# Gongzihang6/Pointcept-KeypointDetection

Measured on AMD Instinct MI355X. Metric: Mpoints/sec PTv3 fwd @100k pts/scene, 1024-pt window; keypoint offset L2 vs ref, higher is better.
Workload: dtype bf16; 1 GPU; OffsetKeypointPTv3 (PT-v3m1 fork config, 46.2M params) eval forward, 1 x 100000-point synthetic surface scene(s) per GPU, patch 1024, serialization + sparse conv + attention + head included; points_per_gpu=100000, parallelism=replicas x1 (scene-sharded, no collective), forwards_in_flight=1

## Files before the change

### include/ptv3_hip.h

```cpp
#ifndef PTV3_HIP_H
#define PTV3_HIP_H
#include <stddef.h>
#include <stdint.h>

#ifdef __cplusplus
extern "C" {
#endif

#define PTV3_F32 0
#define PTV3_BF16 1

#define PTV3_ORDER_Z 0
#define PTV3_ORDER_Z_TRANS 1
#define PTV3_ORDER_HILBERT 2
#define PTV3_ORDER_HILBERT_TRANS 3

#define PTV3_ACT_NONE 0
#define PTV3_ACT_GELU 1
#define PTV3_ACT_RELU 2

const char* ptv3_last_error(void);
int ptv3_version(void);

int ptv3_sfc_encode(const void* grid_coord, int coord_is_i64, const int64_t* batch, int64_t n,
                    int depth, const int* order_ids_host, int k, int64_t* code, void* stream);

size_t ptv3_argsort_workspace_bytes(int k, int64_t n);
int ptv3_argsort_i64(const int64_t* code, int k, int64_t n, int end_bit, int64_t* order,
                     int64_t* inverse, void* workspace, size_t workspace_bytes, void* stream);

int ptv3_argsort_i64_rows(const int64_t* code, int k, int64_t n, int end_bit, int64_t* order, int64_t* inverse,
                          int32_t* row_order, void* workspace, size_t workspace_bytes, void* stream);
int ptv3_argsort_scan_batch(void);

int ptv3_coord_max(const void* grid_coord, int coord_is_i64, int64_t n, int32_t* state, int32_t* out_max, void* stream);

int ptv3_pad_plan(const int64_t* offset, int b, int64_t n, int64_t n_pad, int patch, int64_t* pad,
                  int64_t* unpad, int32_t* cu_seqlens, void* stream);

int ptv3_window_maps(const int64_t* order, const int64_t* inverse, const int64_t* pad,
                     const int64_t* unpad, int64_t n, int64_t n_pad, int32_t* win_order,
                     int32_t* win_inverse, void* stream);

int ptv3_window_plan(const int64_t* order, const int64_t* inverse, const int64_t* offset, int b, int k,
                     int64_t n, int64_t n_pad, int patch, int32_t* win_order, int32_t* win_inverse,
                     int32_t* cu_seqlens, void* stream);

int ptv3_window_attn_fwd(const void* qkv, const int32_t* win_order, const int32_t* win_inverse,
                         void* out, int64_t n, int64_t n_pad, int c, int heads, int patch, float scale,
                         const float* rpe_bias, int dtype, void* stream);

int ptv3_window_attn_varlen_fwd(const void* qkv, const int32_t* win_order, const int32_t* win_inverse,
                                const int32_t* cu_seqlens, int num_windows, void* out, int64_t n, int64_t n_pad,
                                int c, int heads, int max_seqlen, float scale, double sum_len_sq, int dtype,
                                void* stream);

int ptv3_window_attn_rpe_fwd(const void* qkv, const int32_t* win_order, const int32_t* win_inverse, void* out,
                             int64_t n, int64_t n_pad, int c, int heads, int patch, float scale,
                             const int32_t* grid_coord, const float* rpe_table, int pos_bnd, int dtype,
                             void* stream);

int64_t ptv3_subm_table_slots(int64_t n);
int ptv3_subm_build_table(const int32_t* indices, int64_t n, void* table, int64_t slots, void* stream);
int ptv3_subm_neighbors(const int32_t* indices, int64_t n, const void* table, int64_t slots, int ksize,
                        int32_t* nbr, void* stream);

size_t ptv3_subm_block_table_bytes(int64_t n);
int ptv3_subm_build_block_table(const int32_t* indices, int64_t n, void* table, size_t bytes, void* stream);
int ptv3_subm_neighbors_blocks(const int32_t* indices, int64_t n, const void* table, size_t bytes, int ksize,
                               int32_t* nbr, void* stream);

int ptv3_subm_sites(const int64_t* batch, const void* grid_coord, int coord_is_i64, int64_t n, int32_t* indices,
                    int64_t* grid64, void* table, size_t bytes, void* stream);
int ptv3_subm_build_block_table_zeroed(const int32_t* indices, int64_t n, void* table, size_t bytes, void* stream);

size_t ptv3_gemm_workspace_bytes(int64_t m, int cin, int cout, int kvol, int dtype);
int ptv3_gemm_splits(int64_t m, int cin, int cout, int kvol, int dtype);
int ptv3_gemm(const void* x, const void* w, void* out, int64_t m, int cin, int cout, int kvol,
              const int32_t* nbr, const int32_t* row_order, const float* bias, const float* bn_scale,
              const float* bn_shift, int act, const void* res, const int32_t* res_index, void* out2,
              int dtype, void* workspace, size_t workspace_bytes, void* stream);

int ptv3_block_fusable(int c, int hidden, int dtype, int64_t m);
int ptv3_rows_linear_capable(int c, int cout, int dtype, int64_t m);
int ptv3_rows_linear(const void* x, const void* shortcut, const float* g0, const float* b0, const float* g1,
                     const float* b1, const void* w, const float* bias, int act, const void* res, void* f1, void* out,
                     int64_t m, int c, int cout, float eps, int dtype, void* stream);
int ptv3_block_head(const void* x, const float* slab, int splits, const float* conv_bias, const void* shortcut,
                    const float* g0, const float* b0, const float* g1, const float* b1, const void* wqkv,
                    const float* bqkv, void* f1, void* qkv, int64_t m, int c, float eps, int dtype, void* stream);
int ptv3_mlp2_fusable(int cin, int hidden, int cout, int dtype);
int ptv3_mlp2(const void* x, const void* w1, const float* b1, const float* s1, const float* t1, int act,
              const void* w2, const float* b2, void* out, int out_f32, int64_t m, int cin, int hidden, int cout,
              int dtype, void* stream);
int ptv3_block_tail(const void* attn, const void* f1, const void* wproj, const float* bproj, const float* g2,
                    const float* b2, const void* w1, const float* bias1, const void* w2, const float* bias2,
                    void* out, int64_t m, int c, int hidden, float eps, int dtype, void* stream);

int ptv3_rows_linear_ln_capable(int c, int cout, int dtype);
int ptv3_rows_linear_ln(const void* x, const void* w, const float* bias, const float* gamma, const float* beta,
                        void* out, int64_t m, int c, int cout, float eps, int act, int dtype, void* stream);
int ptv3_subm_conv_ln_capable(int c, int kvol, int dtype);
int ptv3_subm_conv_ln(const void* x, const void* w, const int32_t* nbr, const int32_t* row_order, const float* bias,
                      const float* gamma, const float* beta, void* out, int64_t m, int c, int kvol, float eps, int act,
                      int dtype, void* stream);

int ptv3_res_conv_capable(int64_t m, int ca, int cb, int cout, int kvol);
int ptv3_res_conv_row_tiles(int64_t m, int cout);
int ptv3_res_conv(const float* xa, const float* xb, const float* w, const int32_t* nbr, const int32_t* row_order,
                  const float* bn_scale, const float* bn_shift, const float* res, int act, float* out,
                  const float* w_proj, const float* proj_scale, const float* proj_shift, float* proj_out, int64_t m,
                  int ca, int cb, int cout, int kvol, void* stream);

int ptv3_layernorm(const void* x, const float* gamma, const float* beta, const void* res, void* y,
                   const float* gamma2, const float* beta2, void* y2, int64_t m, int c, float eps,
                   int dtype, void* stream);

int ptv3_layernorm_slabs(const float* slab, int splits, const float* slab_bias, const float* gamma, const float* beta,
                         const void* res, void* y, const float* gamma2, const float* beta2, void* y2, int64_t m, int c,
                         float eps, int dtype, void* stream);

int ptv3_affine_act(const void* x, const float* scale, const float* shift, int act, void* y, int64_t m,
                    int c, int dtype, void* stream);

int ptv3_cast(const void* x, int src_dtype, void* y, int dst_dtype, int64_t count, void* stream);

size_t ptv3_pool_workspace_bytes(int64_t n);
int ptv3_pool_segments(const int64_t* code0, const int64_t* order0, int64_t n, int shift_bits,
                       const int64_t* batch, int64_t* cluster, int32_t* seg_start, int32_t* n_out,
                       int64_t* pooled_offset, void* workspace, size_t workspace_bytes, void* stream);
int ptv3_pool_reduce(const void* feat, const float* coord, const int64_t* grid_coord,
                     const int64_t* batch, const int64_t* code, int k, const int64_t* order0,
                     const int32_t* seg_start, int64_t n, int64_t n_out, int c, int pooling_depth,
                     const float* bn_scale, const float* bn_shift, int act, const int* row_perm_host,
                     void* feat_out, float* coord_out, int64_t* grid_out, int64_t* batch_out,
                     int64_t* code_out, int dtype, void* stream);

typedef struct {
  int32_t dtype, in_channels , num_stages, num_orders;
  int32_t enc_depths[8], enc_channels[8], enc_heads[8], enc_patch[8];
  int32_t dec_depths[8], dec_channels[8], dec_heads[8], dec_patch[8];
  int32_t stride[8];
  int32_t enc_mode, enable_flash;
  int32_t head_hidden, head_out;
  float mlp_ratio, ln_eps, qk_scale ;
} ptv3_model_desc;

typedef struct {
  const void* grid_coord; int32_t coord_is_i64;
  const void* feat;
  const int64_t* batch;
  const int64_t* offset;
  const int64_t* offset_host;
  int32_t b; int64_t n;
  int32_t depth;
  const int32_t* order_ids_host;
  const int32_t* pool_perm_host;
  int64_t *code, *order, *inverse;
  void* out_feat;
  float* out_head;
  int64_t* stage_points_host;
  int32_t* depth_out;
  int64_t* batch_out;
  int32_t inputs_resident;
  int32_t overlap_calls;
  const void* raw_feat;
  int32_t raw_feat_channels;
  int32_t raw_feat_dtype;
  int64_t arena_n;
  int32_t arena_b;
  void* executor;
} ptv3_forward_io;

void* ptv3_executor_create(void);
int ptv3_executor_destroy(void* executor);

size_t ptv3_forward_workspace_bytes(const ptv3_model_desc* desc, int64_t n, int b);
int ptv3_forward(const ptv3_model_desc* desc, const void* const* params, int num_params,
                 const ptv3_forward_io* io, void* workspace, size_t workspace_bytes, void* stream);

size_t ptv3_gemm_tn_workspace_bytes(int64_t m, int cout, int cin, int kvol);
int ptv3_gemm_tn(const void* dy, const void* x, const int32_t* nbr, float* dw, float* dbias, int64_t m, int cout,
                 int cin, int kvol, int dtype, void* workspace, size_t workspace_bytes, void* stream);
size_t ptv3_col_reduce_workspace_bytes(int64_t m, int c);
int ptv3_col_reduce(const void* a, const void* b, const float* mu, const float* rs, float mu_scale, int mode, float* out,
                    int64_t m, int c, int dtype, void* workspace, size_t workspace_bytes, void* stream);
int ptv3_bn_finalize(const float* sum, const float* centred_sq, int64_t m, const float* weight, const float* bias,
                     float* running_mean, float* running_var, float momentum, float eps, float* mean, float* rstd,
                     float* scale, float* shift, int c, void* stream);
int ptv3_bn_bwd_coeffs(const float* sums, int64_t m, const float* weight, const float* rstd, const float* mean, float* ca,
                       float* cb, float* cc, int c, void* stream);
int ptv3_layernorm_bwd(const void* x, const void* dy, const void* add, const float* gamma, float eps, void* dx,
                       float* dgamma_dbeta, int64_t m, int c, int dtype, void* workspace,
                       size_t workspace_bytes, void* stream);
int ptv3_act_bwd(const void* dy, const void* x, const float* scale, const float* shift, int act, void* dx,
                 int64_t m, int c, int dtype, void* stream);
int ptv3_affine2(const void* dy, const void* x, const float* ca, const float* cb, const float* cc, void* dx,
                 int64_t m, int c, int dtype, void* stream);
int ptv3_pool_max_bwd(const void* feat, const void* dy, const int64_t* order0, const int32_t* seg_start,
                      int64_t n_out, int c, void* dfeat, int dtype, void* stream);
int ptv3_segment_sum(const void* dy, const int64_t* order0, const int32_t* seg_start, int64_t n_out, int c,
                     void* out, int dtype, void* stream);
size_t ptv3_window_attn_bwd_workspace_bytes(int64_t n, int64_t n_pad, int c, int heads, int dtype);
int ptv3_window_attn_bwd(const void* qkv, const void* out, const void* dout, const int32_t* win_order,
                         const int32_t* win_inverse, void* dqkv, int64_t n, int64_t n_pad, int c, int heads,
                         int patch, float scale, int dtype, void* workspace, size_t workspace_bytes,
                         void* stream);
int ptv3_window_attn_varlen_bwd(const void* qkv, const void* out, const void* dout, const int32_t* win_order,
                                const int32_t* win_inverse, const int32_t* cu_seqlens, int num_windows, void* dqkv,
                                int64_t n, int64_t n_pad, int c, int heads, int max_seqlen, float scale, int dtype,
                                void* workspace, size_t workspace_bytes, void* stream);
int ptv3_window_attn_train_fwd(const void* qkv, const int32_t* win_order, const int32_t* win_inverse,
                               const int32_t* cu_seqlens, int num_windows, void* out, float* lse, int64_t n,
                               int64_t n_pad, int c, int heads, int patch, float scale, double sum_len_sq, int dtype,
                               void* stream);
int ptv3_window_attn_train_bwd(const void* qkv, const void* out, const void* dout, const float* lse,
                               const int32_t* win_order, const int32_t* win_inverse, const int32_t* cu_seqlens,
                               int num_windows, void* dqkv, int64_t n, int64_t n_pad, int c, int heads, int patch,
                               float scale, int dtype, void* workspace, size_t workspace_bytes, void* stream);
int ptv3_window_attn_drop_fwd(const void* qkv, const int32_t* win_order, const int32_t* win_inverse,
                              const int32_t* cu_seqlens, int num_windows, void* out, int64_t n, int64_t n_pad, int c,
                              int heads, int patch, float scale, float p_drop, uint32_t seed, int dtype, void* stream);
int ptv3_window_attn_drop_bwd(const void* qkv, const void* out, const void* dout, const int32_t* win_order,
                              const int32_t* win_inverse, const int32_t* cu_seqlens, int num_windows, void* dqkv,
                              int64_t n, int64_t n_pad, int c, int heads, int patch, float scale, float p_drop,
                              uint32_t seed, int dtype, void* workspace, size_t workspace_bytes, void* stream);
size_t ptv3_window_attn_rpe_bwd_workspace_bytes(int64_t n, int64_t n_pad, int c, int heads, int patch, int pos_bnd,
                                                int dtype);
int ptv3_window_attn_rpe_bwd(const void* qkv, const void* out, const void* dout, const int32_t* win_order,
                             const int32_t* win_inverse, const int32_t* grid_coord, const float* rpe_table,
                             int pos_bnd, void* dqkv, float* dtable, int64_t n, int64_t n_pad, int c, int heads,
                             int patch, float scale, int dtype, void* workspace, size_t workspace_bytes, void* stream);
typedef struct ptv3_block_train {
  int64_t n, n_pad;
// ... 196 lines not shown
```

### pointcept-keypointdetection_amd/csrc/engine.hip

```cpp
#include <algorithm>
#include <chrono>
#include <mutex>
#include <stdio.h>
#include <stdlib.h>
#include <vector>
#include "common.h"
#include "window_attn.h"

namespace ptv3 {

struct Arena {
  char* base; size_t cap; size_t off; size_t peak; bool dry; bool failed;
  void* alloc(size_t bytes) {
    size_t a = (off + 255) / 256 * 256;
    off = a + bytes;
    if (off > peak) peak = off;
    if (dry) return (void*)(uintptr_t)256;
    if (off > cap) { failed = true; return nullptr; }
    return base + a;
  }
};

__global__ void make_indices_kernel(const int64_t* __restrict__ batch, const void* __restrict__ grid,
                                    int is_i64, int64_t n, int32_t* __restrict__ idx,
                                    int64_t* __restrict__ grid64, int32_t* __restrict__ row_order,
                                    const int64_t* __restrict__ order0) {
  int64_t i = (int64_t)blockIdx.x * blockDim.x + threadIdx.x;
  if (i >= n) return;
  int64_t x, y, z;
  if (is_i64) {
    const int64_t* g = (const int64_t*)grid;
    x = g[3 * i]; y = g[3 * i + 1]; z = g[3 * i + 2];
  } else {
    const int32_t* g = (const int32_t*)grid;
    x = g[3 * i]; y = g[3 * i + 1]; z = g[3 * i + 2];
  }
  idx[4 * i] = (int32_t)batch[i];
  idx[4 * i + 1] = (int32_t)x; idx[4 * i + 2] = (int32_t)y; idx[4 * i + 3] = (int32_t)z;
  if (grid64) { grid64[3 * i] = x; grid64[3 * i + 1] = y; grid64[3 * i + 2] = z; }
  if (row_order) row_order[i] = (int32_t)order0[i];
}

__global__ void i64_to_i32_kernel(const int64_t* __restrict__ src, int32_t* __restrict__ dst, int64_t n) {
  int64_t i = (int64_t)blockIdx.x * blockDim.x + threadIdx.x;
  if (i < n) dst[i] = (int32_t)src[i];
}

constexpr int CM_BATCH = 8;
template <typename CoordT>
__global__ void __launch_bounds__(256) coord_max_kernel(const CoordT* __restrict__ grid, int64_t n3, int* __restrict__ state,
                                                        int* __restrict__ out, const int64_t* __restrict__ offset, int b,
                                                        int64_t* __restrict__ offset_out) {
  __shared__ int s_wave[4];
  __shared__ int s_last;
  const int64_t base = (int64_t)blockIdx.x * (256 * CM_BATCH) + threadIdx.x;
  CoordT c[CM_BATCH];
#pragma unroll
  for (int u = 0; u < CM_BATCH; ++u) c[u] = grid[min(base + u * 256, n3 - 1)];
  int v = 0;
#pragma unroll
  for (int u = 0; u < CM_BATCH; ++u) v = max(v, (int)c[u]);
  for (int d = 32; d > 0; d >>= 1) v = max(v, __shfl_down(v, d, 64));
  if ((threadIdx.x & 63) == 0) s_wave[threadIdx.x >> 6] = v;
  __syncthreads();
  if (threadIdx.x == 0) {
    atomicMax(&state[0], max(max(s_wave[0], s_wave[1]), max(s_wave[2], s_wave[3])));
    __threadfence();
    const bool last = atomicAdd(&state[1], 1) == (int)gridDim.x - 1;
    if (last) {
      __threadfence();
      out[0] = atomicExch(&state[0], 0);
      atomicExch(&state[1], 0);
    }
    s_last = last;
  }
  __syncthreads();
  if (s_last)
    for (int i = threadIdx.x; i < b; i += 256) offset_out[i] = offset[i];
}
static void coord_max(const void* grid, int is_i64, int64_t n, int* state, int* out, const int64_t* offset, int b,
                      int64_t* offset_out, hipStream_t s) {
  const dim3 blocks((unsigned)cdiv(3 * n, 256 * CM_BATCH));
  if (is_i64)
    hipLaunchKernelGGL(coord_max_kernel<int64_t>, blocks, dim3(256), 0, s, (const int64_t*)grid, 3 * n, state, out, offset,
                       b, offset_out);
  else
    hipLaunchKernelGGL(coord_max_kernel<int32_t>, blocks, dim3(256), 0, s, (const int32_t*)grid, 3 * n, state, out, offset,
                       b, offset_out);
}

__global__ void batch_from_offset_kernel(const int64_t* __restrict__ offset, int b, int64_t n,
                                         int64_t* __restrict__ batch) {
  int64_t i = (int64_t)blockIdx.x * blockDim.x + threadIdx.x;
  if (i >= n) return;
  int lo = 0, hi = b;
  while (lo < hi) { int mid = (lo + hi) >> 1; if (offset[mid] > i) hi = mid; else lo = mid + 1; }
  batch[i] = lo;
}

struct Plan {
  int K = -1; int64_t n_pad = 0; int32_t* wo[8] = {nullptr}; int32_t* wi[8] = {nullptr};
  int32_t* cu = nullptr; int nwin = 0; double sum_len_sq = 0.0;
};

struct Level {
  int64_t n = 0; int depth = 0;
  std::vector<int64_t> off_host;
  const int64_t* offset = nullptr;
  const int64_t* grid = nullptr; const int64_t* batch = nullptr;
  int64_t *code = nullptr, *order = nullptr, *inverse = nullptr;
  int32_t* indices = nullptr; void* table = nullptr; size_t table_bytes = 0;
  int32_t* nbr3 = nullptr; int32_t* nbr5 = nullptr; int32_t* row_order = nullptr;
  Plan plan[2];
  int32_t* seg = nullptr;
  int64_t* cluster = nullptr;
  int32_t* cluster32 = nullptr;
  hipEvent_t ready = nullptr;
  void* feat = nullptr; void* conv_feat = nullptr; int channels = 0;
};

static inline double now_us() {
  return std::chrono::duration<double, std::micro>(std::chrono::steady_clock::now().time_since_epoch()).count();
}

struct DeviceStreams { hipStream_t geo = nullptr; hipStream_t feat[2] = {nullptr, nullptr}; };
static std::mutex g_pool_mutex;
static std::vector<DeviceStreams> g_device_streams;
static hipStream_t device_stream(int device, int which ) {
  std::lock_guard<std::mutex> guard(g_pool_mutex);
  if ((int)g_device_streams.size() <= device) g_device_streams.resize(device + 1);
  DeviceStreams& d = g_device_streams[device];
  hipStream_t& s = which == 0 ? d.geo : d.feat[which - 1];
  if (!s) {
    if (which == 0) {
      int least = 0, greatest = 0;
      (void)hipDeviceGetStreamPriorityRange(&least, &greatest);
      if (hipStreamCreateWithPriority(&s, hipStreamNonBlocking, greatest) != hipSuccess) s = nullptr;
    } else if (hipStreamCreateWithFlags(&s, hipStreamNonBlocking) != hipSuccess) {
      s = nullptr;
    }
  }
  return s;
}

struct Exec {
  int device = 0;
  hipStream_t geo = nullptr;
  hipStream_t feat[2] = {nullptr, nullptr};
  std::vector<hipEvent_t> events;
  unsigned call = 0;
  bool last_overlap = false;
  double sync_us = 0.0;
  std::mutex mu;
  void* pinned = nullptr; size_t pinned_cap = 0;
  int* cm_state = nullptr;
  int* coord_max_state() {
    if (!cm_state) {
      if (hipMalloc((void**)&cm_state, 256) != hipSuccess) { cm_state = nullptr; return nullptr; }
      if (hipMemset(cm_state, 0, 256) != hipSuccess) { (void)hipFree(cm_state); cm_state = nullptr; }
    }
    return cm_state;
  }
  void* pinned_at_least(size_t bytes) {
    if (pinned_cap < bytes) {
      if (pinned) (void)hipHostFree(pinned);
      pinned = nullptr; pinned_cap = 0;
      const size_t cap = std::max<size_t>(bytes, 4096);
      if (hipHostMalloc(&pinned, cap, hipHostMallocDefault) != hipSuccess) { pinned = nullptr; return nullptr; }
      pinned_cap = cap;
    }
    return pinned;
  }
  hipError_t timed_event_sync(hipEvent_t e) {
    double t = now_us();
    hipError_t r = hipEventSynchronize(e);
    sync_us += now_us() - t;
    return r;
  }
  hipError_t timed_sync(hipStream_t s) {
    double t = now_us();
    hipError_t e = hipStreamSynchronize(s);
    sync_us += now_us() - t;
    return e;
  }
  hipEvent_t event_at(size_t i) {
    while (events.size() <= i) {
      hipEvent_t e;
      (void)hipEventCreateWithFlags(&e, hipEventDisableTiming);
      events.push_back(e);
    }
    return events[i];
  }
  void release() {
    if (geo) { (void)hipStreamSynchronize(geo); geo = nullptr; }
    for (auto& f : feat) if (f) { (void)hipStreamSynchronize(f); f = nullptr; }
    for (hipEvent_t e : events) (void)hipEventDestroy(e);
    events.clear();
    if (pinned) { (void)hipHostFree(pinned); pinned = nullptr; pinned_cap = 0; }
    if (cm_state) { (void)hipFree(cm_state); cm_state = nullptr; }
  }
};
static std::mutex g_exec_mutex;
static std::vector<Exec*> g_default_exec;
static Exec* default_exec() {
  int dev = 0;
  (void)hipGetDevice(&dev);
  std::lock_guard<std::mutex> guard(g_exec_mutex);
  if ((int)g_default_exec.size() <= dev) g_default_exec.resize(dev + 1, nullptr);
  if (!g_default_exec[dev]) { g_default_exec[dev] = new Exec(); g_default_exec[dev]->device = dev; }
  return g_default_exec[dev];
}

template <typename S, typename D>
__global__ void pad_cast_kernel(const S* __restrict__ x, int cin, D* __restrict__ y, int cpad, int64_t n) {
  const int64_t i = (int64_t)blockIdx.x * blockDim.x + threadIdx.x;
  if (i >= n * cpad) return;
  const int c = (int)(i % cpad);
  y[i] = from_f32<D>(c < cin ? to_f32<S>(x[(i / cpad) * cin + c]) : 0.f);
}
static void pad_cast(const void* x, int sdt, int cin, void* y, int ddt, int cpad, int64_t n, hipStream_t s) {
  dim3 grid((unsigned)cdiv(n * cpad, 256)), block(256);
  if (sdt == PTV3_F32 && ddt == PTV3_F32)
    hipLaunchKernelGGL((pad_cast_kernel<float, float>), grid, block, 0, s, (const float*)x, cin, (float*)y, cpad, n);
  else if (sdt == PTV3_F32)
    hipLaunchKernelGGL((pad_cast_kernel<float, __bf16>), grid, block, 0, s, (const float*)x, cin, (__bf16*)y, cpad, n);
  else if (ddt == PTV3_F32)
    hipLaunchKernelGGL((pad_cast_kernel<__bf16, float>), grid, block, 0, s, (const __bf16*)x, cin, (float*)y, cpad, n);
  else
    hipLaunchKernelGGL((pad_cast_kernel<__bf16, __bf16>), grid, block, 0, s, (const __bf16*)x, cin, (__bf16*)y, cpad, n);
}

struct Run {
  Exec* X;
  const ptv3_model_desc* d; const void* const* params; int pi = 0;
  Arena* G; Arena* F;
  hipStream_t sg, sf;
  int es; bool dry; int rc = 0;
  const void* next() { return params ? params[pi++] : (pi++, nullptr); }
  bool ok() const { return rc == 0 && !G->failed && !F->failed; }
#define RUN(call) do { if (!dry && ok()) { int r__ = (call); if (r__) rc = r__; } } while (0)

  void gemm(const void* x, const void* w, void* out, int64_t m, int cin, int cout, int kvol, const int32_t* nbr,
            const int32_t* row_order, const float* bias, const float* bns, const float* bnt, int act,
            const void* res, const int32_t* res_index, void* out2) {
    size_t wsb = ptv3_gemm_workspace_bytes(m, cin, cout, kvol, d->dtype);
    size_t mark = F->off;
    void* ws = wsb ? F->alloc(wsb) : nullptr;
    RUN(ptv3_gemm(x, w, out, m, cin, cout, kvol, nbr, row_order, bias, bns, bnt, act, res, res_index, out2,
                  d->dtype, ws, wsb, sf));
    F->off = mark;
  }

  bool rows_path(int64_t n, int C, int hidden) const {
    static const int64_t min_rows = [] { const char* e = getenv("PTV3_ROWS_MIN"); return e ? atoll(e) : (int64_t)0; }();
    return n >= min_rows && ptv3_rows_linear_capable(C, 3 * C, d->dtype, n) && ptv3_rows_linear_capable(C, C, d->dtype, n) &&
           ptv3_rows_linear_capable(C, hidden, d->dtype, n);
  }

  int patch_K(const Level& L, int patch) const {
    if (d->enable_flash) return patch;
    int64_t mn = L.off_host[0];
    for (size_t i = 1; i < L.off_host.size(); ++i) mn = std::min(mn, L.off_host[i] - L.off_host[i - 1]);
    return (int)std::min<int64_t>(mn, patch);
  }

  void window_plan(Level& L, Plan& P, int K) {
    int64_t n_pad = 0, prev = 0;
    for (int64_t o : L.off_host) {
      int64_t cnt = o - prev;
      n_pad += cnt > K ? (cnt + K - 1) / K * K : cnt;
      prev = o;
    }
    P.K = K; P.n_pad = n_pad;
    bool ragged = false;
    P.nwin = 0; P.sum_len_sq = 0.0; prev = 0;
    for (int64_t o : L.off_host) {
      const int64_t cnt = o - prev;
      prev = o;
      P.nwin += (int)((cnt + K - 1) / K);
      if (cnt < K) { ragged = true; P.sum_len_sq += (double)cnt * cnt; }
      else P.sum_len_sq += (double)((cnt + K - 1) / K) * K * K;
    }
    const int k = d->num_orders;
    int32_t* wo = (int32_t*)G->alloc((size_t)k * n_pad * 4);
    int32_t* wi = (int32_t*)G->alloc((size_t)k * L.n * 4);
    P.cu = (ragged || (dry && d->enable_flash)) ? (int32_t*)G->alloc(((size_t)P.nwin + L.off_host.size() + 1) * 4) : nullptr;
    if (!ragged && !dry) P.cu = nullptr;
    RUN(ptv3_window_plan(L.order, L.inverse, L.offset, (int)L.off_host.size(), k, L.n, n_pad, K, wo, wi, P.cu, sg));
    for (int i = 0; i < k; ++i) { P.wo[i] = wo + (int64_t)i * n_pad; P.wi[i] = wi + (int64_t)i * L.n; }
  }

  hipEvent_t stem_ready = nullptr;
  void level0_sites(Level& L, const void* grid_in, int is_i64) {
    L.indices = (int32_t*)G->alloc((size_t)L.n * 16);
    L.row_order = (int32_t*)G->alloc((size_t)L.n * 4);
    int64_t* g64 = (int64_t*)G->alloc((size_t)L.n * 24);
    L.grid = g64;
    L.table_bytes = ptv3_subm_block_table_bytes(L.n);
    L.table = G->alloc(L.table_bytes);
    RUN(ptv3_subm_sites(L.batch, grid_in, is_i64, L.n, L.indices, g64, L.table, L.table_bytes, sg));
    RUN(ptv3_subm_build_block_table_zeroed(L.indices, L.n, L.table, L.table_bytes, sg));
    L.nbr5 = (int32_t*)G->alloc((size_t)L.n * 125 * 4);
    RUN(ptv3_subm_neighbors_blocks(L.indices, L.n, L.table, L.table_bytes, 5, L.nbr5, sg));
  }

  void level_tables(Level& L, int st) {
    L.nbr3 = (int32_t*)G->alloc((size_t)L.n * 27 * 4);
    RUN(ptv3_subm_neighbors_blocks(L.indices, L.n, L.table, L.table_bytes, 3, L.nbr3, sg));
    const int Ke = patch_K(L, d->enc_patch[st]);
    window_plan(L, L.plan[0], Ke);
    if (!d->enc_mode && st < d->num_stages - 1) {
      const int Kd = patch_K(L, d->dec_patch[st]);
      if (Kd == Ke) L.plan[1] = L.plan[0]; else window_plan(L, L.plan[1], Kd);
    }
  }

  void level_geometry(Level& L, int st, const void* grid_in, int is_i64) {
    L.indices = (int32_t*)G->alloc((size_t)L.n * 16);
    L.row_order = (int32_t*)G->alloc((size_t)L.n * 4);
    if (!dry && ok())
      hipLaunchKernelGGL(make_indices_kernel, dim3((unsigned)cdiv(L.n, 256)), dim3(256), 0, sg, L.batch, grid_in, is_i64,
                         L.n, L.indices, (int64_t*)nullptr, L.row_order, L.order);
    L.table_bytes = ptv3_subm_block_table_bytes(L.n);
    L.table = G->alloc(L.table_bytes);
    RUN(ptv3_subm_build_block_table(L.indices, L.n, L.table, L.table_bytes, sg));
    level_tables(L, st);
  }

  void attention(const Level& L, const Plan& P, const void* qkv, void* out, int C, int H, int oi, float scale) {
    WindowAttnCall a = window_attn_call(qkv, P.wo[oi], P.wi[oi], out, L.n, P.n_pad, C, H, P.K, scale, d->dtype, sf);
    a.cu_seqlens = P.cu; a.num_windows = P.nwin; a.sum_len_sq = P.sum_len_sq;
    RUN(window_attn_forward(a, {"window_attn", WA_RAGGED_OPTIONAL}));
  }

  void block(Level& L, const Plan& P, int C, int H, int oi) {
    const void* conv_w = next(); const float* conv_b = (const float*)next();
    const float* ln0_g = (const float*)next(); const float* ln0_b = (const float*)next();
    const float* n1_g = (const float*)next(); const float* n1_b = (const float*)next();
    const void* qkv_w = next(); const float* qkv_b = (const float*)next();
    const void* proj_w = next(); const float* proj_b = (const float*)next();
    const float* n2_g = (const float*)next(); const float* n2_b = (const float*)next();
    const void* fc1_w = next(); const float* fc1_b = (const float*)next();
    const void* fc2_w = next(); const float* fc2_b = (const float*)next();
    const int hidden = (int)(C * d->mlp_ratio);
    const size_t mark = F->off;
    const size_t row = (size_t)L.n * es;
    const float scale = d->qk_scale > 0.f ? d->qk_scale : 1.0f / sqrtf((float)(C / H));
    if (ptv3_block_fusable(C, hidden, d->dtype, L.n)) {
      void* f1 = F->alloc(row * C); void* qkv = F->alloc(row * 3 * C); void* t4 = F->alloc(row * C);
      const int splits = ptv3_gemm_splits(L.n, C, C, 27, d->dtype);
      if (splits > 1) {
        const size_t wsb = ptv3_gemm_workspace_bytes(L.n, C, C, 27, d->dtype);
        float* slab = (float*)F->alloc(wsb);
        RUN(ptv3_gemm(L.conv_feat, conv_w, nullptr, L.n, C, C, 27, L.nbr3, L.row_order, nullptr, nullptr, nullptr, 0,
                      nullptr, nullptr, nullptr, d->dtype, slab, wsb, sf));
        RUN(ptv3_block_head(nullptr, slab, splits, conv_b, L.feat, ln0_g, ln0_b, n1_g, n1_b, qkv_w, qkv_b, f1, qkv, L.n,
                            C, d->ln_eps, d->dtype, sf));
      } else {
        void* t2 = F->alloc(row * C);
        gemm(L.conv_feat, conv_w, t2, L.n, C, C, 27, L.nbr3, L.row_order, conv_b, nullptr, nullptr, 0, nullptr, nullptr, nullptr);
        RUN(ptv3_block_head(t2, nullptr, 0, nullptr, L.feat, ln0_g, ln0_b, n1_g, n1_b, qkv_w, qkv_b, f1, qkv, L.n, C,
                            d->ln_eps, d->dtype, sf));
      }
      attention(L, P, qkv, t4, C, H, oi, scale);
      RUN(ptv3_block_tail(t4, f1, proj_w, proj_b, n2_g, n2_b, fc1_w, fc1_b, fc2_w, fc2_b, L.feat, L.n, C, hidden,
                          d->ln_eps, d->dtype, sf));
    } else {
      void* t2 = F->alloc(row * C); void* f1 = F->alloc(row * C); void* t3 = F->alloc(row * C);
      void* qkv = F->alloc(row * 3 * C); void* t4 = F->alloc(row * C); void* f2 = F->alloc(row * C);
      void* t5 = F->alloc(row * C); void* t6 = F->alloc(row * hidden);
      const int splits = ptv3_gemm_splits(L.n, C, C, 27, d->dtype);
      const bool rows = rows_path(L.n, C, hidden);
      if (splits > 1) {
        const size_t wsb = ptv3_gemm_workspace_bytes(L.n, C, C, 27, d->dtype);
        float* slab = (float*)F->alloc(wsb);
        RUN(ptv3_gemm(L.conv_feat, conv_w, nullptr, L.n, C, C, 27, L.nbr3, L.row_order, nullptr, nullptr, nullptr, 0,
                      nullptr, nullptr, nullptr, d->dtype, slab, wsb, sf));
        RUN(ptv3_layernorm_slabs(slab, splits, conv_b, ln0_g, ln0_b, L.feat, f1, n1_g, n1_b, t3, L.n, C, d->ln_eps,
                                 d->dtype, sf));
        gemm(t3, qkv_w, qkv, L.n, C, 3 * C, 1, nullptr, nullptr, qkv_b, nullptr, nullptr, 0, nullptr, nullptr, nullptr);
      } else if (rows) {
        gemm(L.conv_feat, conv_w, t2, L.n, C, C, 27, L.nbr3, L.row_order, conv_b, nullptr, nullptr, 0, nullptr, nullptr, nullptr);
        RUN(ptv3_rows_linear(t2, L.feat, ln0_g, ln0_b, n1_g, n1_b, qkv_w, qkv_b, 0, nullptr, f1, qkv, L.n, C, 3 * C,
                             d->ln_eps, d->dtype, sf));
      } else {
        gemm(L.conv_feat, conv_w, t2, L.n, C, C, 27, L.nbr3, L.row_order, conv_b, nullptr, nullptr, 0, nullptr, nullptr, nullptr);
        RUN(ptv3_layernorm(t2, ln0_g, ln0_b, L.feat, f1, n1_g, n1_b, t3, L.n, C, d->ln_eps, d->dtype, sf));
        gemm(t3, qkv_w, qkv, L.n, C, 3 * C, 1, nullptr, nullptr, qkv_b, nullptr, nullptr, 0, nullptr, nullptr, nullptr);
      }
      attention(L, P, qkv, t4, C, H, oi, scale);
      if (rows) {
        RUN(ptv3_rows_linear(t4, nullptr, nullptr, nullptr, nullptr, nullptr, proj_w, proj_b, 0, f1, nullptr, f2, L.n, C, C,
                             d->ln_eps, d->dtype, sf));
        RUN(ptv3_rows_linear(f2, nullptr, nullptr, nullptr, n2_g, n2_b, fc1_w, fc1_b, PTV3_ACT_GELU, nullptr, nullptr, t6,
                             L.n, C, hidden, d->ln_eps, d->dtype, sf));
      } else {
        gemm(t4, proj_w, f2, L.n, C, C, 1, nullptr, nullptr, proj_b, nullptr, nullptr, 0, f1, nullptr, nullptr);
        RUN(ptv3_layernorm(f2, n2_g, n2_b, nullptr, t5, nullptr, nullptr, nullptr, L.n, C, d->ln_eps, d->dtype, sf));
        gemm(t5, fc1_w, t6, L.n, C, hidden, 1, nullptr, nullptr, fc1_b, nullptr, nullptr, PTV3_ACT_GELU, nullptr, nullptr, nullptr);
      }
      gemm(t6, fc2_w, L.feat, L.n, hidden, C, 1, nullptr, nullptr, fc2_b, nullptr, nullptr, 0, f2, nullptr, nullptr);
    }
    L.conv_feat = L.feat;
    F->off = mark;
  }
};

#define RUNR(call) do { if (!dry && R.ok()) { int r__ = (call); if (r__) R.rc = r__; } } while (0)

static int run_forward(Exec* X, const ptv3_model_desc* d, const void* const* params, const ptv3_forward_io* io, Arena& G,
                       Arena& F, hipStream_t sf, bool dry, int* param_count = nullptr) {
  Run R; R.X = X; R.d = d; R.params = params; R.G = &G; R.F = &F; R.sf = sf; R.dry = dry;
  R.es = d->dtype == PTV3_F32 ? 4 : 2;
  const int S = d->num_stages, k = d->num_orders, es = R.es;
  if (!dry) {
    if (!X->geo) {
      X->geo = device_stream(X->device, 0);
      if (!X->geo) {
        set_error("forward: cannot create the geometry stream");
        return PTV3_ERR_LAUNCH;
      }
    }
    if (!io->inputs_resident) {
      hipEvent_t e = X->event_at(0);
      (void)hipEventRecord(e, sf);
      (void)hipStreamWaitEvent(X->geo, e, 0);
    } else {
      (void)hipStreamWaitEvent(X->geo, X->event_at(20 + (X->call & 1)), 0);
    }
  }
  R.sg = dry ? nullptr : X->geo;
  hipStream_t sg = R.sg;
  std::vector<Level> lv(S);
  const int nbits = io->b > 1 ? 32 - __builtin_clz((unsigned)(io->b - 1)) : 0;

  Level& L0 = lv[0];
  L0.n = io->n; L0.batch = io->batch; L0.offset = io->offset;
  L0.code = io->code; L0.order = io->order; L0.inverse = io->inverse;
  L0.off_host.resize(io->b);
  int depth = io->depth;
  const int* hmax = nullptr; const int64_t* hoff = nullptr;
  hipEvent_t read_back = nullptr;
  if (dry) {
    for (int i = 0; i < io->b; ++i) L0.off_host[i] = io->offset_host ? io->offset_host[i] : io->n * (i + 1) / io->b;
    if (depth <= 0) depth = 16;
  } else {
    if (io->offset_host) std::copy(io->offset_host, io->offset_host + io->b, L0.off_host.begin());
    if (depth <= 0 || !io->offset_host) {
      char* pin = (char*)X->pinned_at_least(8 + (size_t)io->b * 8);
      if (!pin) { set_error("forward: cannot allocate the pinned read-back buffer"); return PTV3_ERR_LAUNCH; }
      if (!io->offset_host) hoff = (const int64_t*)(pin + 8);
      if (depth <= 0) {
        int* state = X->coord_max_state();
        if (!state) { set_error("forward: cannot allocate the coordinate-maximum state"); return PTV3_ERR_LAUNCH; }
        hmax = (const int*)pin;
        coord_max(io->grid_coord, io->coord_is_i64, io->n, state, (int*)pin, io->offset, hoff ? io->b : 0,
                  (int64_t*)(pin + 8), sg);
      } else {
        (void)hipMemcpyAsync(pin + 8, io->offset, (size_t)io->b * 8, hipMemcpyDeviceToHost, sg);
      }
      read_back = X->event_at(18);
      (void)hipEventRecord(read_back, sg);
    }
  }
  if (io->batch == nullptr) {
    int64_t* bt = io->batch_out ? io->batch_out : (int64_t*)G.alloc((size_t)io->n * 8);
    if (!dry && R.ok())
      hipLaunchKernelGGL(batch_from_offset_kernel, dim3((unsigned)cdiv(io->n, 256)), dim3(256), 0, sg, io->offset, io->b,
                         io->n, bt);
    L0.batch = bt;
  }
  R.level0_sites(L0, io->grid_coord, io->coord_is_i64);
  if (!dry) {
    if (read_back && X->timed_event_sync(read_back) != hipSuccess) {
      set_error("forward: input read-back failed");
      return PTV3_ERR_LAUNCH;
    }
    if (hoff) std::copy(hoff, hoff + io->b, L0.off_host.begin());
    if (hmax) { depth = 0; for (unsigned v = (unsigned)*hmax + 1; v; v >>= 1) ++depth; }
    PTV3_REQUIRE(depth >= 1 && depth <= 16, "forward: serialization depth %d outside [1,16] (structure.py:81)", depth);
    for (int i = 0; i < io->b; ++i)
      PTV3_REQUIRE(L0.off_host[i] > (i ? L0.off_host[i - 1] : 0), "forward: empty scene %d", i);
    PTV3_REQUIRE(L0.off_host[io->b - 1] == io->n, "forward: offset does not end at n");
  }
  L0.depth = depth;
  if (io->depth_out) *io->depth_out = depth;
  {
    RUNR(ptv3_sfc_encode(io->grid_coord, io->coord_is_i64, L0.batch, io->n, depth, io->order_ids_host, k, L0.code, sg));
    size_t wsb = ptv3_argsort_workspace_bytes(k, io->n);
    void* ws = G.alloc(wsb);
    RUNR(ptv3_argsort_i64_rows(L0.code, k, io->n, std::max(1, 3 * depth + nbits), L0.order, L0.inverse, L0.row_order, ws, wsb,
                               sg));
  }
  if (!dry && R.ok()) { R.stem_ready = X->event_at(19); (void)hipEventRecord(R.stem_ready, sg); }
  R.level_tables(L0, 0);
  if (io->stage_points_host) io->stage_points_host[0] = L0.n;
  if (!dry && R.ok()) { L0.ready = X->event_at(1); (void)hipEventRecord(L0.ready, sg); }

  auto wait_level = [&](Level& L) { if (!dry && R.ok()) (void)hipStreamWaitEvent(sf, L.ready, 0); };
  struct PoolParams { const void* w; const float *b, *bns, *bnt; };
  const void* stem_w = R.next(); const float* stem_s = (const float*)R.next(); const float* stem_t = (const float*)R.next();
  {
    if (!dry && R.ok()) (void)hipStreamWaitEvent(sf, R.stem_ready, 0);
    const int C0 = d->enc_channels[0];
    L0.feat = F.alloc((size_t)L0.n * C0 * es); L0.channels = C0;
    const void* feat_in = io->feat;
    if (io->raw_feat) {
      void* padded = F.alloc((size_t)L0.n * d->in_channels * es);
      if (!dry && R.ok())
        pad_cast(io->raw_feat, io->raw_feat_dtype, io->raw_feat_channels, padded, d->dtype, d->in_channels, L0.n, sf);
      feat_in = padded;
    }
    R.gemm(feat_in, stem_w, L0.feat, L0.n, d->in_channels, C0, 125, L0.nbr5, L0.row_order, nullptr, stem_s, stem_t,
           PTV3_ACT_GELU, nullptr, nullptr, nullptr);
    L0.conv_feat = L0.feat;
    wait_level(L0);
  }
  for (int st = 0; st < S; ++st) {
    Level& L = lv[st];
    if (st > 0) {
      Level& P = lv[st - 1];
      PoolParams pp;
      pp.w = R.next(); pp.b = (const float*)R.next(); pp.bns = (const float*)R.next(); pp.bnt = (const float*)R.next();
      const int C = d->enc_channels[st], Cp = d->enc_channels[st - 1];
      int pd = 0; { int v = d->stride[st - 1] - 1; while (v > 0) { ++pd; v >>= 1; } }
      if (pd > P.depth) pd = 0;
      P.cluster = (int64_t*)G.alloc((size_t)P.n * 8);
      P.seg = (int32_t*)G.alloc((size_t)(P.n + 1) * 4);
      int64_t* poff = (int64_t*)G.alloc((size_t)io->b * 8);
      int32_t* nout_dev = (int32_t*)G.alloc(256);
      size_t pwsb = ptv3_pool_workspace_bytes(P.n);
      void* pws = G.alloc(pwsb);
      RUNR(ptv3_pool_segments(P.code, P.order, P.n, 3 * pd, P.batch, P.cluster, P.seg, nout_dev, poff, pws, pwsb, sg));
      L.off_host.resize(io->b);
      if (dry) {
        L.off_host = P.off_host;
      } else if (R.ok()) {
        if (hipMemcpyAsync(L.off_host.data(), poff, (size_t)io->b * 8, hipMemcpyDeviceToHost, sg) != hipSuccess ||
            X->timed_sync(sg) != hipSuccess) { set_error("forward: offset read-back failed"); return PTV3_ERR_LAUNCH; }
      }
      if (!R.ok()) break;
      L.n = L.off_host[io->b - 1]; L.depth = P.depth - pd; L.offset = poff; L.channels = C;
      if (io->stage_points_host) io->stage_points_host[st] = L.n;
      const int* perm = io->pool_perm_host + (size_t)(st - 1) * k;
      int64_t* g = (int64_t*)G.alloc((size_t)L.n * 24);
      int64_t* bt = (int64_t*)G.alloc((size_t)L.n * 8);
      L.code = (int64_t*)G.alloc((size_t)k * L.n * 8);
      L.order = (int64_t*)G.alloc((size_t)k * L.n * 8);
      L.inverse = (int64_t*)G.alloc((size_t)k * L.n * 8);
      RUNR(ptv3_pool_reduce(nullptr, nullptr, P.grid, P.batch, P.code, k, P.order, P.seg, P.n, L.n, C, pd, nullptr,
                           nullptr, 0, perm, nullptr, nullptr, g, bt, L.code, d->dtype, sg));
      L.grid = g; L.batch = bt;
      {
        size_t wsb = ptv3_argsort_workspace_bytes(k, L.n);
        void* ws = G.alloc(wsb);
        RUNR(ptv3_argsort_i64(L.code, k, L.n, std::max(1, 3 * L.depth + nbits), L.order, L.inverse, ws, wsb, sg));
      }
      R.level_geometry(L, st, L.grid, 1);
      if (!d->enc_mode) {
        P.cluster32 = (int32_t*)G.alloc((size_t)P.n * 4);
        if (!dry && R.ok())
          hipLaunchKernelGGL(i64_to_i32_kernel, dim3((unsigned)cdiv(P.n, 256)), dim3(256), 0, sg, P.cluster, P.cluster32, P.n);
      }
      if (!dry && R.ok()) { L.ready = X->event_at(1 + st); (void)hipEventRecord(L.ready, sg); }
      wait_level(L);
      L.feat = F.alloc((size_t)L.n * C * es);
      const size_t mark = F.off;
      void* proj = F.alloc((size_t)P.n * C * es);
      R.gemm(P.feat, pp.w, proj, P.n, Cp, C, 1, nullptr, nullptr, pp.b, nullptr, nullptr, 0, nullptr, nullptr, nullptr);
      RUNR(ptv3_pool_reduce(proj, nullptr, nullptr, nullptr, nullptr, k, P.order, P.seg, P.n, L.n, C, pd, pp.bns, pp.bnt,
                           PTV3_ACT_GELU, nullptr, L.feat, nullptr, nullptr, nullptr, nullptr, d->dtype, sf));
      F.off = mark;
      L.conv_feat = L.feat;
    }
    for (int i = 0; i < d->enc_depths[st]; ++i)
      R.block(L, L.plan[0], d->enc_channels[st], d->enc_heads[st], i % k);
    if (!R.ok()) break;
  }
  if (!d->enc_mode && R.ok()) {
    for (int st = S - 2; st >= 0; --st) {
      Level& P = lv[st];
      Level& Ch = lv[st + 1];
      const int Cd = d->dec_channels[st];
      const int Cin = Ch.channels, Cskip = d->enc_channels[st];
      const void* w = R.next(); const float* b = (const float*)R.next();
      const float* bns = (const float*)R.next(); const float* bnt = (const float*)R.next();
      const void* ws_ = R.next(); const float* bs = (const float*)R.next();
      const float* bnss = (const float*)R.next(); const float* bnst = (const float*)R.next();
      void* skip = F.alloc((size_t)P.n * Cd * es);
      void* fused = (st == 0 && io->out_feat) ? io->out_feat : F.alloc((size_t)P.n * Cd * es);
      const size_t mark = F.off;
      void* up = F.alloc((size_t)Ch.n * Cd * es);
      R.gemm(Ch.feat, w, up, Ch.n, Cin, Cd, 1, nullptr, nullptr, b, bns, bnt, PTV3_ACT_GELU, nullptr, nullptr, nullptr);
      R.gemm(P.feat, ws_, skip, P.n, Cskip, Cd, 1, nullptr, nullptr, bs, bnss, bnst, PTV3_ACT_GELU, up, P.cluster32, fused);
      F.off = mark;
      P.feat = fused; P.conv_feat = skip; P.channels = Cd;
      for (int i = 0; i < d->dec_depths[st]; ++i)
        R.block(P, P.plan[1], Cd, d->dec_heads[st], i % k);
      if (!R.ok()) break;
    }
  }
  if (R.ok() && d->head_out > 0 && !d->enc_mode) {
    Level& L = lv[0];
    const void* w0 = R.next(); const float* b0 = (const float*)R.next();
    const float* bns = (const float*)R.next(); const float* bnt = (const float*)R.next();
    const void* w1 = R.next(); const float* b1 = (const float*)R.next();
    const size_t mark = F.off;
    if (ptv3_mlp2_fusable(L.channels, d->head_hidden, d->head_out, d->dtype)) {
      if (!dry && R.ok()) {
        int r = ptv3_mlp2(L.feat, w0, b0, bns, bnt, PTV3_ACT_RELU, w1, b1, io->out_head, 1, L.n, L.channels,
                          d->head_hidden, d->head_out, d->dtype, sf);
        if (r) R.rc = r;
      }
    } else {
    void* hid = F.alloc((size_t)L.n * d->head_hidden * es);
    R.gemm(L.feat, w0, hid, L.n, L.channels, d->head_hidden, 1, nullptr, nullptr, b0, bns, bnt, PTV3_ACT_RELU, nullptr,
           nullptr, nullptr);
    if (d->dtype == PTV3_F32) {
      R.gemm(hid, w1, io->out_head, L.n, d->head_hidden, d->head_out, 1, nullptr, nullptr, b1, nullptr, nullptr, 0,
             nullptr, nullptr, nullptr);
    } else {
      void* o = F.alloc((size_t)L.n * d->head_out * es);
      R.gemm(hid, w1, o, L.n, d->head_hidden, d->head_out, 1, nullptr, nullptr, b1, nullptr, nullptr, 0, nullptr,
             nullptr, nullptr);
      if (!dry && R.ok()) { int r = ptv3_cast(o, PTV3_BF16, io->out_head, PTV3_F32, L.n * d->head_out, sf); if (r) R.rc = r; }
    }
    }
    F.off = mark;
  }
  if (!dry && R.ok() && !d->enc_mode && io->out_feat && lv[0].feat != io->out_feat)
    (void)hipMemcpyAsync(io->out_feat, lv[0].feat, (size_t)lv[0].n * lv[0].channels * es, hipMemcpyDeviceToDevice, sf);
  if (!dry) (void)hipEventRecord(X->event_at(20 + (X->call & 1)), sf);
  if (param_count) *param_count = R.pi;
  if (G.failed || F.failed) { set_error("forward: workspace arena too small"); return PTV3_ERR_ARG; }
  if (R.rc) return R.rc;
  if (!dry) PTV3_LAUNCH_CHECK();
  return PTV3_OK;
}

static int check_desc(const ptv3_model_desc* d) {
  PTV3_REQUIRE(d->num_stages >= 1 && d->num_stages <= 8, "forward: num_stages %d", d->num_stages);
  PTV3_REQUIRE(d->num_orders >= 1 && d->num_orders <= 8, "forward: num_orders %d", d->num_orders);
  PTV3_REQUIRE(d->dtype == PTV3_F32 || d->dtype == PTV3_BF16, "forward: dtype");
  PTV3_REQUIRE(d->mlp_ratio > 0.f, "forward: mlp_ratio");
  return PTV3_OK;
}

static void plan_bytes(const ptv3_model_desc* desc, int64_t n, int b, size_t* geo, size_t* feat, int* count) {
  std::vector<int> ids(desc->num_orders, 0), perm((size_t)desc->num_stages * desc->num_orders, 0);
  ptv3_forward_io io{};
  io.n = n; io.b = b; io.depth = 0; io.order_ids_host = ids.data(); io.pool_perm_host = perm.data();
  io.coord_is_i64 = 1;
  Arena G{nullptr, 0, 0, 0, true, false}, F{nullptr, 0, 0, 0, true, false};
  run_forward(nullptr, desc, nullptr, &io, G, F, nullptr, true, count);
  *geo = (G.peak + (size_t)b * 16384 * 64 + (1 << 20) + 255) / 256 * 256;
  *feat = (F.peak + (1 << 20) + 255) / 256 * 256;
}

}

using namespace ptv3;

extern "C" int ptv3_coord_max(const void* grid_coord, int coord_is_i64, int64_t n, int32_t* state, int32_t* out_max,
                              void* stream) {
  PTV3_REQUIRE(n >= 1 && n < ((int64_t)1 << 31) && grid_coord && state && out_max, "coord_max: n=%lld or a null pointer",
               (long long)n);
  coord_max(grid_coord, coord_is_i64, n, state, out_max, nullptr, 0, nullptr, (hipStream_t)stream);
  PTV3_LAUNCH_CHECK();
  return PTV3_OK;
}

extern "C" size_t ptv3_forward_workspace_bytes(const ptv3_model_desc* desc, int64_t n, int b) {
  if (check_desc(desc)) return 0;
  size_t g, f;
  plan_bytes(desc, n, b, &g, &f, nullptr);
  return 2 * g + 2 * f + 512;
}

extern "C" void* ptv3_executor_create(void) {
  Exec* X = new Exec();
  (void)hipGetDevice(&X->device);
  return X;
}

extern "C" int ptv3_executor_destroy(void* executor) {
  Exec* X = (Exec*)executor;
  if (!X) return PTV3_OK;
  {
    std::lock_guard<std::mutex> guard(X->mu);
    X->release();
  }
  delete X;
  return PTV3_OK;
}

extern "C" int ptv3_forward(const ptv3_model_desc* desc, const void* const* params, int num_params,
                            const ptv3_forward_io* io, void* workspace, size_t workspace_bytes, void* stream) {
  Exec* X = io->executor ? (Exec*)io->executor : default_exec();
  std::lock_guard<std::mutex> guard(X->mu);
  int cur_dev = 0;
  (void)hipGetDevice(&cur_dev);
  PTV3_REQUIRE(cur_dev == X->device, "forward: executor belongs to device %d, the current device is %d", X->device, cur_dev);
  if (int r = check_desc(desc)) return r;
  PTV3_REQUIRE(io->n >= 1 && io->b >= 1, "forward: empty batch");
  PTV3_REQUIRE(io->depth <= 16, "forward: depth %d > 16", io->depth);
  PTV3_REQUIRE(io->code && io->order && io->inverse, "forward: level-0 serialization outputs are required");
  size_t g, f;
  int count = 0;
  plan_bytes(desc, io->n, io->b, &g, &f, &count);
  PTV3_REQUIRE(count == num_params, "forward: %d parameter pointers given, the model description needs %d",
               num_params, count);
  const bool overlap = io->overlap_calls != 0;
  PTV3_REQUIRE(!overlap || io->inputs_resident, "forward: overlap_calls needs inputs_resident");
  PTV3_REQUIRE(io->raw_feat == nullptr || (io->raw_feat_channels >= 1 && io->raw_feat_channels <= desc->in_channels &&
                                           (io->raw_feat_dtype == PTV3_F32 || io->raw_feat_dtype == PTV3_BF16)),
               "forward: bad raw_feat description");
  if (io->arena_n > 0) {
    PTV3_REQUIRE(io->arena_n >= io->n && io->arena_b >= io->b, "forward: arena capacity (%lld, %d) below this call (%lld, %d)",
                 (long long)io->arena_n, io->arena_b, (long long)io->n, io->b);
    size_t gc, fc;
    plan_bytes(desc, io->arena_n, io->arena_b, &gc, &fc, nullptr);
    PTV3_REQUIRE(gc >= g && fc >= f, "forward: arena capacity plan smaller than this call's plan");
    g = gc; f = fc;
  } else {
    PTV3_REQUIRE(!io->inputs_resident || !overlap, "forward: overlap_calls needs a fixed arena layout (arena_n / arena_b)");
  }
  const size_t need = 2 * g + (overlap ? 2 : 1) * f + 256;
  PTV3_REQUIRE(workspace_bytes >= need, "forward: workspace %zu bytes < %zu (ptv3_forward_workspace_bytes)",
               workspace_bytes, need);
// ... 38 lines not shown
```

### pointcept-keypointdetection_amd/csrc/gemm.hip

```cpp
#include <stdlib.h>
#include <algorithm>
#include <type_traits>
#include "common.h"
#include "profile.h"
#include "block_args.h"
#include "../../include/ptv3_hip.h"

namespace ptv3 {

constexpr int GM_THREADS = 256;
constexpr int GM_BM = 64;

struct GemmArgs {
  const void* x; const void* w; void* out; void* out2; const void* res;
  const int32_t* nbr; const int32_t* row_order; const int32_t* res_index;
  const float* bias; const float* bn_scale; const float* bn_shift;
  float* slab;
  int64_t m; int cin; int cout; int kvol; int act; int cin_shift; int steps_per_split;
  int64_t x_bytes;
  int ablate;
};

__device__ __forceinline__ float apply_act(float v, int act) {
  if (act == PTV3_ACT_GELU) return gelu_erf(v);
  if (act == PTV3_ACT_RELU) return fmaxf(v, 0.f);
  return v;
}

template <typename T>
__device__ __forceinline__ void epilogue_store(const GemmArgs& a, int64_t orow, int ch0, const float* accv) {
  typedef typename Vec4<T>::type V4;
  T* out = reinterpret_cast<T*>(a.out);
  T* out2 = reinterpret_cast<T*>(a.out2);
  const T* res = reinterpret_cast<const T*>(a.res);
  const bool vec_ok = (a.cout & 3) == 0;
  float v[4], v2[4];
#pragma unroll
  for (int r = 0; r < 4; ++r) {
    const int ch = ch0 + r;
    float t = accv[r];
    if (ch < a.cout) {
      if (a.bias) t += a.bias[ch];
      if (a.bn_scale) t = t * a.bn_scale[ch] + a.bn_shift[ch];
      t = apply_act(t, a.act);
    }
    v[r] = t;
    v2[r] = t;
  }
  if (a.res) {
    const int64_t rrow = a.res_index ? (int64_t)a.res_index[orow] : orow;
    if (vec_ok) {
      float rr[4];
      unpack4<T>(*reinterpret_cast<const V4*>(res + rrow * a.cout + ch0), rr);
#pragma unroll
      for (int r = 0; r < 4; ++r) v2[r] = v[r] + rr[r];
    } else {
#pragma unroll
      for (int r = 0; r < 4; ++r)
        if (ch0 + r < a.cout) v2[r] = v[r] + to_f32<T>(res[rrow * a.cout + ch0 + r]);
    }
  }
  if (vec_ok) {
    if (out2) {
      *reinterpret_cast<V4*>(out + orow * a.cout + ch0) = pack4<T>(v[0], v[1], v[2], v[3]);
      *reinterpret_cast<V4*>(out2 + orow * a.cout + ch0) = pack4<T>(v2[0], v2[1], v2[2], v2[3]);
    } else {
      *reinterpret_cast<V4*>(out + orow * a.cout + ch0) = pack4<T>(v2[0], v2[1], v2[2], v2[3]);
    }
  } else {
#pragma unroll
    for (int r = 0; r < 4; ++r)
      if (ch0 + r < a.cout) {
        if (out2) {
          out[orow * a.cout + ch0 + r] = from_f32<T>(v[r]);
          out2[orow * a.cout + ch0 + r] = from_f32<T>(v2[r]);
        } else {
          out[orow * a.cout + ch0 + r] = from_f32<T>(v2[r]);
        }
      }
  }
}

template <typename T> struct Chunk16;
template <> struct Chunk16<float> {
  static constexpr int N = 4;
  static __device__ __forceinline__ void load(const float* p, float* o) { f32x4 v = *reinterpret_cast<const f32x4*>(p); o[0] = v[0]; o[1] = v[1]; o[2] = v[2]; o[3] = v[3]; }
  static __device__ __forceinline__ void store(float* p, const float* o) { *reinterpret_cast<f32x4*>(p) = f32x4{o[0], o[1], o[2], o[3]}; }
};
template <> struct Chunk16<__bf16> {
  static constexpr int N = 8;
  static __device__ __forceinline__ void load(const __bf16* p, float* o) {
    const s16x8 v = *reinterpret_cast<const s16x8*>(p);
#pragma unroll
    for (int i = 0; i < 8; ++i) o[i] = bf16_to_f32(v[i]);
  }
  static __device__ __forceinline__ void store(__bf16* p, const float* o) {
    const s16x4 lo = pack4<__bf16>(o[0], o[1], o[2], o[3]), hi = pack4<__bf16>(o[4], o[5], o[6], o[7]);
    *reinterpret_cast<s16x8*>(p) = __builtin_shufflevector(lo, hi, 0, 1, 2, 3, 4, 5, 6, 7);
  }
};

struct EpiVec { f32x4 bias, scale, shift; };
__device__ __forceinline__ void park_epi(const GemmArgs& a, float* sEpi, int bn, int n0, int tid, int nthreads) {
  for (int t = tid; t < bn; t += nthreads) {
    const int ch = n0 + t;
    const bool in = ch < a.cout;
    sEpi[t] = (in && a.bias) ? a.bias[ch] : 0.f;
    sEpi[bn + t] = (in && a.bn_scale) ? a.bn_scale[ch] : 1.f;
    sEpi[2 * bn + t] = (in && a.bn_scale) ? a.bn_shift[ch] : 0.f;
  }
}
__device__ __forceinline__ EpiVec load_epi(const float* sEpi, int bn, int cl) {
  return EpiVec{*reinterpret_cast<const f32x4*>(sEpi + cl), *reinterpret_cast<const f32x4*>(sEpi + bn + cl),
                *reinterpret_cast<const f32x4*>(sEpi + 2 * bn + cl)};
}

template <typename T>
__device__ __forceinline__ void stage_values(const GemmArgs& a, T* sOut, int os, int rl, int cl, const EpiVec& e,
                                             f32x4 acc) {
  float v[4];
#pragma unroll
  for (int r = 0; r < 4; ++r) v[r] = apply_act((acc[r] + e.bias[r]) * e.scale[r] + e.shift[r], a.act);
  *reinterpret_cast<typename Vec4<T>::type*>(sOut + (size_t)rl * os + cl) = pack4<T>(v[0], v[1], v[2], v[3]);
}

template <typename T, int UB>
__device__ __forceinline__ void store_tile(const GemmArgs& a, const T* sOut, int os, int rows, int bn, int64_t row0,
                                           int n0, int tid, int nthreads) {
  constexpr int N = Chunk16<T>::N;
  typedef typename Frag<T>::type FR;
  const int cpr = bn / N;
  const int total = rows * cpr;
  T* out = reinterpret_cast<T*>(a.out);
  T* out2 = reinterpret_cast<T*>(a.out2);
  const T* res = reinterpret_cast<const T*>(a.res);
  for (int e0 = tid; e0 < total; e0 += nthreads * UB) {
    int64_t orow[UB];
    int col[UB], rl[UB];
    bool ok[UB];
#pragma unroll
    for (int u = 0; u < UB; ++u) {
      const int e = e0 + u * nthreads;
      rl[u] = e / cpr;
      col[u] = n0 + (e - rl[u] * cpr) * N;
      const int64_t prow = row0 + rl[u];
      ok[u] = e < total && prow < a.m && col[u] < a.cout;
      orow[u] = ok[u] ? (a.row_order ? (int64_t)a.row_order[prow] : prow) : 0;
    }
    FR rraw[UB];
    if (res) {
      int64_t rrow[UB];
#pragma unroll
      for (int u = 0; u < UB; ++u) rrow[u] = (ok[u] && a.res_index) ? (int64_t)a.res_index[orow[u]] : orow[u];
#pragma unroll
      for (int u = 0; u < UB; ++u)
        if (ok[u]) rraw[u] = *reinterpret_cast<const FR*>(res + rrow[u] * a.cout + col[u]);
    }
#pragma unroll
// ... 465 lines not shown
  const int wr = wave / WN, wc = wave % WN;
  const unsigned ntn = (a.cout + BN - 1) / BN;
  const unsigned logical = xcd_remap(blockIdx.x, gridDim.x);
  const int64_t row0 = (int64_t)(logical / ntn) * GC_BM;
  const int n0 = (int)(logical % ntn) * BN;
  const int ktot = a.kvol * a.cin;
  const int step_lo = a.slab ? (int)blockIdx.y * a.steps_per_split : 0;
  const int nsteps = a.slab ? min(ktot / BK - step_lo, a.steps_per_split) : ktot / BK;

  {
#pragma unroll
    for (int half = tid; half < 2 * GC_BM; half += NTH) {
      const int pr = half >> 1, d0 = (half & 1) * 14;
      const int64_t r = row0 + pr;
      const bool in = r < a.m;
      const int64_t orow = in ? (a.row_order ? (int64_t)a.row_order[r] : r) : 0;
      int32_t v[14];
#pragma unroll
      for (int u = 0; u < 14; ++u) {
        const int d = d0 + u;
        v[u] = a.nbr[orow * a.kvol + (d < a.kvol ? d : 0)];
      }
#pragma unroll
      for (int u = 0; u < 14; ++u)
        if (d0 + u < a.kvol) sNbr[pr * a.kvol + d0 + u] = in ? v[u] : -1;
    }
  }
  if (!a.slab) park_epi(a, sEpi, BN, n0, tid, NTH);

  const __amdgpu_buffer_rsrc_t xrs =
      __builtin_amdgcn_make_buffer_rsrc(const_cast<void*>(a.x), 0, (int)a.x_bytes, 0x00020000);
  const __amdgpu_buffer_rsrc_t wrs = __builtin_amdgcn_make_buffer_rsrc(
      const_cast<void*>(a.w), 0, (int)((int64_t)a.cout * ktot * (int)sizeof(T)), 0x00020000);
  auto swz = [](int r) { return KB == 128 ? ((r >> 1) & 7) : ((0 - (r >> 2)) & 3); };
  constexpr int LPR = KB / 16;
  const int rr = lane / LPR, cch = lane % LPR;
  int xnb[XQ];
  unsigned xcol[XQ];
  unsigned woff[WQ];
#pragma unroll
  for (int i = 0; i < XQ; ++i) {
    const int r = RPI * (wave + NW * i) + rr;
    xnb[i] = r * a.kvol;
    xcol[i] = (unsigned)((cch ^ swz(r)) * 16);
  }
#pragma unroll
  for (int i = 0; i < WQ; ++i) {
    const int r = RPI * (wave + NW * i) + rr;
    const int o = n0 + r;
    woff[i] = o < a.cout ? (unsigned)(((int64_t)o * ktot) * (int)sizeof(T)) + (unsigned)((cch ^ swz(r)) * 16) : 0xFFFFFFF0u;
  }
  const unsigned row_bytes = (unsigned)(a.cin * (int)sizeof(T));
  auto issue = [&](int step) {
    char* buf = stg + (step % NSTG) * STG;
    const int k0 = (step_lo + step) * BK;
    const int d = a.cin_shift >= 0 ? (k0 >> a.cin_shift) : (k0 / a.cin);
    const unsigned kb = (unsigned)((k0 - d * a.cin) * (int)sizeof(T));
#pragma unroll
    for (int i = 0; i < XQ; ++i) {
      const int src = sNbr[xnb[i] + d];
      const unsigned off = src >= 0 ? (unsigned)src * row_bytes + kb + xcol[i] : 0xFFFFFFF0u;
      __builtin_amdgcn_raw_ptr_buffer_load_lds(xrs, PTV3_LDS_PTR(buf + (wave + NW * i) * 1024), 16, off, 0, 0, 0);
    }
    const unsigned kw = (unsigned)(k0 * (int)sizeof(T));
#pragma unroll
    for (int i = 0; i < WQ; ++i) {
      const unsigned off = woff[i] == 0xFFFFFFF0u ? woff[i] : woff[i] + kw;
      __builtin_amdgcn_raw_ptr_buffer_load_lds(wrs, PTV3_LDS_PTR(buf + GC_BM * KB + (wave + NW * i) * 1024), 16, off, 0, 0, 0);
    }
  };

  f32x4 acc[MI][NJ];
#pragma unroll
  for (int m = 0; m < MI; ++m)
#pragma unroll
    for (int j = 0; j < NJ; ++j) acc[m][j] = f32x4{0.f, 0.f, 0.f, 0.f};

  auto frag = [&](const char* img, int r, int ks) -> FR {
    return *reinterpret_cast<const FR*>(img + r * KB + 16 * ((4 * ks + g) ^ swz(r)));
  };
  asm volatile("s_waitcnt lgkmcnt(0)" ::: "memory");
  __builtin_amdgcn_s_barrier();
  asm volatile("" ::: "memory");
#pragma unroll
  for (int i = 0; i < AH; ++i)
    if (i < nsteps) issue(i);
  for (int step = 0; step < nsteps; ++step) {
    const int rem = nsteps - 1 - step;
    if (!(a.ablate & 4)) {
      if (rem >= AH - 1) gc_wait_vm<(AH - 1) * DPS>();
      else if (AH >= 3 && rem == 1) gc_wait_vm<DPS>();
      else gc_wait_vm<0>();
      asm volatile("s_waitcnt lgkmcnt(0)" ::: "memory");
      __builtin_amdgcn_s_barrier();
      asm volatile("" ::: "memory");
    }
    if (step + AH < nsteps && !(a.ablate & 2)) issue(step + AH);
    if (a.ablate & 1) continue;
    const char* bx = stg + (step % NSTG) * STG;
    const char* bw = bx + GC_BM * KB;
    FR xf[2][4], wf[2][NJ];
    auto load_group = [&](int n, FR (&x4)[4], FR (&w4)[NJ]) {
      const int ks = n / (MI / 4), h = n % (MI / 4);
      if (h == 0) {
#pragma unroll
        for (int j = 0; j < NJ; ++j) w4[j] = frag(bw, (NJ * wc + j) * 16 + li, ks);
      }
#pragma unroll
      for (int m = 0; m < 4; ++m) x4[m] = frag(bx, (MI * wr + 4 * h + m) * 16 + li, ks);
    };
    load_group(0, xf[0], wf[0]);
    __builtin_amdgcn_sched_group_barrier(0x100, 4 + NJ, 0);
    static_for<0, NGRP>([&](auto nc) {
      constexpr int n = decltype(nc)::value;
      constexpr int ks = n / (MI / 4), h = n % (MI / 4);
      if constexpr (n + 1 < NGRP) load_group(n + 1, xf[(n + 1) & 1], wf[((n + 1) / (MI / 4)) & 1]);
#pragma unroll
      for (int m = 0; m < 4; ++m)
#pragma unroll
        for (int j = 0; j < NJ; ++j) acc[4 * h + m][j] = F::mma(wf[ks & 1][j], xf[n & 1][m], acc[4 * h + m][j]);
      constexpr int MPG = 4 * NJ * (F::E == 8 ? 1 : 4);
      __builtin_amdgcn_sched_group_barrier(0x008, 1, 0);
      if constexpr (n + 1 < NGRP) __builtin_amdgcn_sched_group_barrier(0x100, ((n + 1) % (MI / 4) == 0) ? 4 + NJ : 4, 0);
      __builtin_amdgcn_sched_group_barrier(0x008, MPG - 1, 0);
    });
  }
  if (a.slab) {
#pragma unroll
    for (int m = 0; m < MI; ++m) {
      const int64_t prow = row0 + (MI * wr + m) * 16 + li;
      if (prow >= a.m) continue;
      const int64_t orow = a.row_order ? (int64_t)a.row_order[prow] : prow;
      float* dst = a.slab + ((int64_t)blockIdx.y * a.m + orow) * a.cout + n0 + 4 * g;
#pragma unroll
      for (int j = 0; j < NJ; ++j) {
        const int ch = (NJ * wc + j) * 16;
        if (n0 + ch + 4 * g < a.cout) *reinterpret_cast<f32x4*>(dst + ch) = acc[m][j];
      }
    }
    return;
  }
  __syncthreads();
  constexpr int OS = BN + 16 / (int)sizeof(T);
  T* sOut = reinterpret_cast<T*>(gc_smem);
#pragma unroll
  for (int j = 0; j < NJ; ++j) {
    const EpiVec ev = load_epi(sEpi, BN, (NJ * wc + j) * 16 + 4 * g);
#pragma unroll
    for (int m = 0; m < MI; ++m)
      stage_values<T>(a, sOut, OS, (MI * wr + m) * 16 + li, (NJ * wc + j) * 16 + 4 * g, ev, acc[m][j]);
  }
  __syncthreads();
  store_tile<T, 8>(a, sOut, OS, GC_BM, BN, row0, n0, tid, NTH);
}

static bool use_conv_tile(int64_t m, int cin, int cout, int kvol, int dtype, int64_t x_bytes, int* bn_out, int splits) {
  const char* env = getenv("PTV3_CONV_TILE");
  const int mode = env ? atoi(env) : 1;
  const int bk = dtype == PTV3_F32 ? 32 : 64, gran = dtype == PTV3_F32 ? 4 : 8;
  const char* e64 = getenv("PTV3_CONV_TILE_64");
  const bool narrow = cout == 64 && dtype == PTV3_BF16 && e64 && atoi(e64) != 0;
  if (mode == 0 || x_bytes <= 0 || kvol > GB_MAX_KVOL || kvol < 2 || cin % bk != 0 || cout % gran != 0 || (cout < 128 && !narrow))
    return false;
  if (narrow) {
    *bn_out = 64;
    return splits > 1 || mode == 2 || cdiv(m, GC_BM) >= 160;
  }
  if (splits > 1) {
    const char* se = getenv("PTV3_CONV_TILE_SPLIT");
    *bn_out = 128;
    return cout % 8 == 0 && (se ? atoi(se) != 0 : dtype == PTV3_BF16);
  }
  const int bn = (dtype == PTV3_BF16 && cout >= 256) ? 256 : 128;
  *bn_out = bn;
  if (mode == 2) return true;
  const int64_t tiles = cdiv(m, GC_BM) * cdiv(cout, bn);
  const int64_t rounds = cdiv(tiles, 256);
  return tiles >= 160 && 4 * tiles >= 3 * rounds * 256 && (int64_t)kvol * cin >= 1024;
}

static bool use_big_tile(int64_t m, int cin, int cout, int kvol, int dtype, int* bn_out) {
  const char* env = getenv("PTV3_GEMM_BIG");
  const int mode = env ? atoi(env) : 1;
  if (mode == 0 || kvol > GB_MAX_KVOL || cout < (mode == 2 ? 64 : 128)) return false;
  const int bn = cout >= 128 ? 128 : 64;
  *bn_out = bn;
  const int64_t tiles = cdiv(m, GB_BM) * cdiv(cout, bn);
  const int64_t ktot = (int64_t)kvol * cin;
  if (mode == 2) return true;
  return tiles >= 256 && ktot >= 1024;
}

template <typename T>
__global__ void __launch_bounds__(256) splitk_reduce_kernel(GemmArgs a, int splits) {
  const int c4 = (a.cout + 3) / 4;
  int64_t t = (int64_t)blockIdx.x * blockDim.x + threadIdx.x;
  if (t >= a.m * c4) return;
  const int64_t row = t / c4;
  const int ch0 = (int)(t - row * c4) * 4;
  float v[4] = {0.f, 0.f, 0.f, 0.f};
  const bool vec_ok = (a.cout & 3) == 0;
  for (int z = 0; z < splits; ++z) {
    const float* src = a.slab + ((int64_t)z * a.m + row) * a.cout + ch0;
    if (vec_ok) {
      f32x4 p = *reinterpret_cast<const f32x4*>(src);
      v[0] += p[0]; v[1] += p[1]; v[2] += p[2]; v[3] += p[3];
    } else {
#pragma unroll
      for (int r = 0; r < 4; ++r)
        if (ch0 + r < a.cout) v[r] += src[r];
    }
  }
  epilogue_store<T>(a, row, ch0, v);
}

static int bk_of(int dtype) { return dtype == PTV3_F32 ? 32 : 64; }

static int choose_nt(int cout) {
  static const int opts[] = {2, 4, 6, 8, 12, 16};
  static const bool tuning = getenv("PTV3_GEMM_TUNE") != nullptr;
  if (tuning) {
    if (const char* e = getenv("PTV3_GEMM_NT")) {
      int v = atoi(e);
      for (int nt : opts) if (nt == v) return v;
    }
  }
  return cout <= 32 ? 2 : 4;
}

static int choose_splits(int64_t m, int cin, int cout, int kvol, int dtype, int* steps_per_split) {
  const int bk = bk_of(dtype);
  const int64_t ktot = (int64_t)kvol * cin;
  const int nsteps = (int)((ktot + bk - 1) / bk);
  const int bn = 16 * choose_nt(cout);
  const int64_t base = cdiv(m, GM_BM) * cdiv(cout, bn);
  int splits = 1;
  if (nsteps >= 16 && base < 512) {
    int64_t want = 1536 / base;
    if (want > nsteps / 4) want = nsteps / 4;
    if (want >= 4) splits = (int)want;
  }
  int sps = (nsteps + splits - 1) / splits;
  splits = (nsteps + sps - 1) / sps;
  *steps_per_split = sps;
  return splits;
}

}

using namespace ptv3;

extern "C" int ptv3_gemm_splits(int64_t m, int cin, int cout, int kvol, int dtype) {
  int sps;
  return choose_splits(m, cin, cout, kvol, dtype, &sps);
}

extern "C" size_t ptv3_gemm_workspace_bytes(int64_t m, int cin, int cout, int kvol, int dtype) {
  int sps;
  int splits = choose_splits(m, cin, cout, kvol, dtype, &sps);
  return splits > 1 ? (size_t)splits * m * cout * sizeof(float) : 0;
}

extern "C" int ptv3_gemm(const void* x, const void* w, void* out, int64_t m, int cin, int cout, int kvol,
                         const int32_t* nbr, const int32_t* row_order, const float* bias,
                         const float* bn_scale, const float* bn_shift, int act, const void* res,
                         const int32_t* res_index, void* out2, int dtype, void* workspace,
                         size_t workspace_bytes, void* stream) {
  PTV3_REQUIRE(dtype == PTV3_F32 || dtype == PTV3_BF16, "gemm: bad dtype %d", dtype);
  const int gran = dtype == PTV3_F32 ? 4 : 8;
  PTV3_REQUIRE(cin > 0 && cin % gran == 0, "gemm: cin=%d must be a positive multiple of %d for this dtype", cin, gran);
  PTV3_REQUIRE(cout > 0, "gemm: cout=%d", cout);
  PTV3_REQUIRE(kvol >= 1 && (kvol == 1 || nbr != nullptr), "gemm: kvol=%d needs a neighbour table", kvol);
  PTV3_REQUIRE((bn_scale == nullptr) == (bn_shift == nullptr), "gemm: bn_scale/bn_shift must come together");
  PTV3_REQUIRE(out2 == nullptr || res != nullptr, "gemm: out2 without res");
  if (m == 0) return PTV3_OK;
  int sps;
  int splits = choose_splits(m, cin, cout, kvol, dtype, &sps);
  {
    const char* ct = getenv("PTV3_CONV_TILE");
    const char* bg = getenv("PTV3_GEMM_BIG");
    const char* sk = getenv("PTV3_GEMM_SPLITK");
    if (out != nullptr && ((ct && atoi(ct) == 2 && nbr) || (bg && atoi(bg) == 2) || (sk && atoi(sk) == 0))) { splits = 1; sps = 0; }
  }
  int big_bn = 0;
  const bool big = splits <= 1 && out != nullptr && use_big_tile(m, cin, cout, kvol, dtype, &big_bn);
  if (splits > 1 && (workspace == nullptr || workspace_bytes < (size_t)splits * m * cout * sizeof(float))) {
    splits = 1;
    sps = 0;
  }
  PTV3_REQUIRE(out != nullptr || splits > 1, "gemm: out == NULL needs a split-K shape and its workspace");
  int cin_shift = -1;
  if ((cin & (cin - 1)) == 0) { cin_shift = 0; while ((1 << cin_shift) < cin) ++cin_shift; }
  const int esz0 = dtype == PTV3_F32 ? 4 : 2;
  const char* buf_env = getenv("PTV3_GEMM_BUF");
  const bool buf_on = !(buf_env && atoi(buf_env) == 0);
  const int64_t xb = m * cin * esz0, wb = (int64_t)cout * kvol * cin * esz0, lim = ((int64_t)1 << 31) - 4096;
  const int64_t x_bytes = (nbr && buf_on && xb < lim && wb < lim) ? xb : 0;
  GemmArgs a{x, w, out, out2, res, nbr, row_order, res_index, bias, bn_scale, bn_shift,
             splits > 1 ? (float*)workspace : nullptr, m, cin, cout, kvol, act, cin_shift, sps, x_bytes, 0};
  if (const char* e = getenv("PTV3_CONV_ABLATE")) a.ablate = atoi(e);
  hipStream_t s = (hipStream_t)stream;
  int nt = choose_nt(cout);
  if (nbr && nt != 2) nt = 4;
  const int bn = 16 * nt;
  const int esz = dtype == PTV3_F32 ? 4 : 2;
  const int prof = prof_begin(s, nbr ? PROF_SUBM_CONV : PROF_LINEAR, 2.0 * m * kvol * cin * cout,
                              ((double)m * cin * (nbr ? 1 : kvol) + (double)cout * kvol * cin +
                               (double)m * cout * (1 + (res != nullptr) + (out2 != nullptr))) * esz,
                              nbr, m * kvol, 2.0 * cin * cout);
  auto reduce_slabs = [&]() {
    GemmArgs r = a;
    r.row_order = nullptr;
    const int64_t work = m * ((cout + 3) / 4);
    if (dtype == PTV3_F32)
      hipLaunchKernelGGL(splitk_reduce_kernel<float>, dim3((unsigned)cdiv(work, 256)), dim3(256), 0, s, r, splits);
    else
      hipLaunchKernelGGL(splitk_reduce_kernel<__bf16>, dim3((unsigned)cdiv(work, 256)), dim3(256), 0, s, r, splits);
  };
  int ct_bn = 0;
  const bool ctile = nbr != nullptr && (out != nullptr || splits > 1) && use_conv_tile(m, cin, cout, kvol, dtype, x_bytes, &ct_bn, splits);
  if (ctile) {
    prof_kernel(prof, PK_CONV_TILE);
    const char* st_env = getenv("PTV3_CONV_STAGES");
    const bool four = st_env && atoi(st_env) == 4 && splits <= 1;
    const size_t lds_ops = (size_t)(GC_BM + ct_bn) * 256 + (size_t)GC_BM * GB_MAX_KVOL * 4;
    const size_t lds_out = (size_t)GC_BM * (ct_bn * esz + 16);
    const size_t lds = std::max(lds_ops, lds_out) + (size_t)3 * ct_bn * sizeof(float);
    PTV3_REQUIRE(lds <= 160 * 1024, "conv tile: %zu bytes of LDS", lds);
    dim3 cgrid((unsigned)(cdiv(m, GC_BM) * cdiv(cout, ct_bn)), (unsigned)std::max(splits, 1));
#define GC_LAUNCH(T, BN_, KB_, NS_)                                                                              \
    do {                                                                                                         \
      ensure_dynamic_lds(reinterpret_cast<const void*>(&conv_tile_kernel<T, BN_, KB_, NS_>), 160 * 1024);        \
      hipLaunchKernelGGL((conv_tile_kernel<T, BN_, KB_, NS_>), cgrid, gc_threads, lds, s, a);              \
    } while (0)
#define GC_PICK(T, BN_) do { if (four) GC_LAUNCH(T, BN_, 64, 4); else GC_LAUNCH(T, BN_, 128, 2); } while (0)
    const dim3 gc_threads(ct_bn == 64 ? GC_THREADS / 2 : GC_THREADS);
    if (dtype == PTV3_F32) GC_PICK(float, 128);
    else if (ct_bn == 256) GC_PICK(__bf16, 256);
    else if (ct_bn == 64) GC_PICK(__bf16, 64);
    else GC_PICK(__bf16, 128);
#undef GC_PICK
#undef GC_LAUNCH
    prof_end(prof, s);
    if (splits > 1 && out != nullptr) reduce_slabs();
    PTV3_LAUNCH_CHECK();
    return PTV3_OK;
  }
  prof_kernel(prof, big ? (nbr ? PK_GEMM_BIG_CONV : PK_GEMM_BIG_DENSE)
                        : nt == 2 ? (nbr ? PK_GEMM32_CONV : PK_GEMM32_DENSE) : (nbr ? PK_GEMM64_CONV : PK_GEMM64_DENSE));
  if (big) {
    const size_t lds_out = (size_t)GB_BM * (big_bn * esz + 16);
    const size_t lds = std::max((size_t)2 * (GB_BM + big_bn) * 128 + (nbr ? (size_t)GB_BM * kvol * 4 : 0), lds_out);
    static_assert(2 * (GB_BM + 128) * 128 + GB_BM * GB_MAX_KVOL * 4 + GB_MAX_STEPS + 32 + 3 * 128 * 4 <= 80 * 1024,
                  "gemm_big_kernel: two workgroups per CU need <= 80 KB of LDS each");
    dim3 bgrid((unsigned)(cdiv(m, GB_BM) * cdiv(cout, big_bn)));
#define GB_LAUNCH(T, WM_, WN_, BN_, G_, B_)                                                                      \
    do {                                                                                                         \
      ensure_dynamic_lds(reinterpret_cast<const void*>(&gemm_big_kernel<T, WM_, WN_, BN_, G_, B_>), 96 * 1024);  \
      hipLaunchKernelGGL((gemm_big_kernel<T, WM_, WN_, BN_, G_, B_>), bgrid, dim3(GB_THREADS), lds, s, a);       \
    } while (0)
#define GB_PICK(T)                                                                                               \
    do {                                                                                                         \
      if (nbr && x_bytes) { if (big_bn == 128) GB_LAUNCH(T, 2, 2, 128, true, true); else GB_LAUNCH(T, 4, 1, 64, true, true); } \
      else if (nbr) { if (big_bn == 128) GB_LAUNCH(T, 2, 2, 128, true, false); else GB_LAUNCH(T, 4, 1, 64, true, false); }     \
      else { if (big_bn == 128) GB_LAUNCH(T, 2, 2, 128, false, false); else GB_LAUNCH(T, 4, 1, 64, false, false); }            \
    } while (0)
    if (dtype == PTV3_F32) GB_PICK(float); else GB_PICK(__bf16);
#undef GB_PICK
#undef GB_LAUNCH
    prof_end(prof, s);
    PTV3_LAUNCH_CHECK();
    return PTV3_OK;
  }
  dim3 grid((unsigned)cdiv(m, GM_BM), (unsigned)cdiv(cout, bn), (unsigned)splits);
#define GM_LAUNCH(T, G)                                                                                \
  switch (nt) {                                                                                        \
    case 2: hipLaunchKernelGGL((gemm_kernel<T, 2, G>), grid, dim3(GM_THREADS), 0, s, a); break;        \
    case 4: hipLaunchKernelGGL((gemm_kernel<T, 4, G>), grid, dim3(GM_THREADS), 0, s, a); break;        \
    case 6: hipLaunchKernelGGL((gemm_kernel<T, 6, G>), grid, dim3(GM_THREADS), 0, s, a); break;        \
    case 8: hipLaunchKernelGGL((gemm_kernel<T, 8, G>), grid, dim3(GM_THREADS), 0, s, a); break;        \
    case 12: hipLaunchKernelGGL((gemm_kernel<T, 12, G>), grid, dim3(GM_THREADS), 0, s, a); break;      \
    default: hipLaunchKernelGGL((gemm_kernel<T, 16, G>), grid, dim3(GM_THREADS), 0, s, a); break;      \
  }
  const char* pd_env = getenv("PTV3_GEMM_PD");
  const char* pdl_env = getenv("PTV3_GEMM_PD_LARGE");
  int pd = 1;
  if (nt == 4) {
    const bool small = (int64_t)grid.x * grid.y * grid.z <= 1024;
    pd = pd_env ? atoi(pd_env) : (small ? 4 : (pdl_env ? atoi(pdl_env) : 1));
    if (pd != 2 && pd != 4) pd = 1;
  }
#define GM_PD(T, G)                                                                                            \
  do {                                                                                                         \
    if (pd == 4) hipLaunchKernelGGL((gemm_kernel<T, 4, G, 4>), grid, dim3(GM_THREADS), 0, s, a);               \
    else if (pd == 2) hipLaunchKernelGGL((gemm_kernel<T, 4, G, 2>), grid, dim3(GM_THREADS), 0, s, a);          \
    else hipLaunchKernelGGL((gemm_kernel<T, 4, G, 1>), grid, dim3(GM_THREADS), 0, s, a);                       \
  } while (0)
  if (nbr) {
    if (dtype == PTV3_F32) {
      if (nt == 2) hipLaunchKernelGGL((gemm_kernel<float, 2, true>), grid, dim3(GM_THREADS), 0, s, a);
      else GM_PD(float, true);
    } else {
      if (nt == 2) hipLaunchKernelGGL((gemm_kernel<__bf16, 2, true>), grid, dim3(GM_THREADS), 0, s, a);
      else GM_PD(__bf16, true);
    }
  } else if (nt == 4) {
    if (dtype == PTV3_F32) GM_PD(float, false); else GM_PD(__bf16, false);
  } else if (dtype == PTV3_F32) { GM_LAUNCH(float, false) } else { GM_LAUNCH(__bf16, false) }
#undef GM_PD
#undef GM_LAUNCH
  prof_end(prof, s);
  if (splits > 1 && out != nullptr) reduce_slabs();
  PTV3_LAUNCH_CHECK();
  return PTV3_OK;
}
```

### pointcept-keypointdetection_amd/csrc/profile.h

```cpp
#pragma once
#include <hip/hip_runtime.h>
#include <stdint.h>

namespace ptv3 {
enum { PROF_LINEAR = 0, PROF_SUBM_CONV = 1, PROF_WINDOW_ATTN = 2, PROF_BACKWARD = 3, PROF_FAMILIES = 4 };
enum {
  PK_GEMM64_DENSE = 0, PK_GEMM64_CONV, PK_GEMM32_DENSE, PK_GEMM32_CONV, PK_GEMM_BIG_DENSE, PK_GEMM_BIG_CONV,
  PK_BLOCK_HEAD, PK_BLOCK_TAIL, PK_BLOCK_HEAD_COOP, PK_BLOCK_TAIL_COOP, PK_MLP2, PK_ATTN_FULL, PK_ATTN_TILED,
  PK_BLOCK_HEAD_WIDE, PK_BLOCK_TAIL_WIDE, PK_CONV_TILE, PK_GEMM_TN, PK_ATTN_BWD_DQ, PK_ATTN_BWD_DKV, PK_SWIN_ATTN, PK_ROWS_LINEAR, PK_SWIN_ATTN_MFMA, PK_KERNELS
};
void prof_kernel(int rec, int kernel);
bool prof_on();
int prof_begin(hipStream_t s, int family, double flops, double bytes, const int32_t* nbr, int64_t nbr_count,
               double flops_per_valid);
void prof_end(int rec, hipStream_t s);
}
```

### pointcept-keypointdetection_amd/csrc/profile.hip

```cpp
#include <vector>
#include "common.h"
#include "profile.h"
#include "../../include/ptv3_hip.h"

namespace ptv3 {

struct ProfRec { int family; double flops, bytes, per_valid; hipEvent_t e0, e1; int slot; int kernel; };
static const char* const g_kernel_names[PK_KERNELS] = {
    "gemm_kernel<64ch> dense", "gemm_kernel<64ch> gather (sparse conv)", "gemm_kernel<32ch> dense",
    "gemm_kernel<32ch> gather (sparse conv)", "gemm_big_kernel dense", "gemm_big_kernel gather (sparse conv)",
    "block_head_kernel", "block_tail_kernel", "block_head_coop_kernel", "block_tail_coop_kernel", "mlp2_kernel",
    "window_attn_full_kernel", "window_attn_kernel", "block_head_wide_kernel", "block_tail_wide_kernel",
    "conv_tile_kernel (sparse conv)", "gemm_tn_kernel", "attn_bwd_dq_kernel", "attn_bwd_dkv_kernel",
    "swin_attn_kernel", "rows_linear_kernel", "swin_attn_mfma_kernel"};
static bool g_on = false;
static double g_hint_flops = -1.0;
static std::vector<ProfRec> g_recs;
static std::vector<hipEvent_t> g_pool;
static unsigned long long* g_slots = nullptr;
static int g_nslots = 0;
constexpr int MAX_SLOTS = 1 << 16;

__global__ void count_valid_kernel(const int32_t* __restrict__ nbr, int64_t n, unsigned long long* out) {
  int64_t i = (int64_t)blockIdx.x * blockDim.x + threadIdx.x;
  unsigned long long c = 0;
  for (; i < n; i += (int64_t)gridDim.x * blockDim.x) c += nbr[i] >= 0;
  for (int d = 32; d > 0; d >>= 1) c += __shfl_down(c, d, 64);
  if ((threadIdx.x & 63) == 0 && c) atomicAdd(out, c);
}

bool prof_on() { return g_on; }

static hipEvent_t get_event() {
  if (!g_pool.empty()) { hipEvent_t e = g_pool.back(); g_pool.pop_back(); return e; }
  hipEvent_t e;
  (void)hipEventCreate(&e);
  return e;
}

int prof_begin(hipStream_t s, int family, double flops, double bytes, const int32_t* nbr, int64_t nbr_count,
               double flops_per_valid) {
  if (!g_on) return -1;
  static const int default_kernel[PROF_FAMILIES] = {PK_GEMM64_DENSE, PK_GEMM64_CONV, PK_ATTN_FULL, PK_GEMM_TN};
  if (g_hint_flops >= 0.0) { flops = g_hint_flops; g_hint_flops = -1.0; }
  ProfRec r{family, flops, bytes, flops_per_valid, get_event(), get_event(), -1, default_kernel[family]};
  if (nbr && g_slots && g_nslots < MAX_SLOTS) {
    r.slot = g_nslots++;
    hipLaunchKernelGGL(count_valid_kernel, dim3(512), dim3(256), 0, s, nbr, nbr_count, g_slots + r.slot);
  }
  (void)hipEventRecord(r.e0, s);
  g_recs.push_back(r);
  return (int)g_recs.size() - 1;
}

void prof_end(int rec, hipStream_t s) {
  if (rec >= 0) (void)hipEventRecord(g_recs[rec].e1, s);
}

void prof_kernel(int rec, int kernel) {
  if (rec >= 0 && kernel >= 0 && kernel < PK_KERNELS) g_recs[rec].kernel = kernel;
}

}

using namespace ptv3;

extern "C" int ptv3_profile_enable(int on) {
  if (on && !g_slots) {
    if (hipMalloc(&g_slots, (size_t)MAX_SLOTS * 8) != hipSuccess) { set_error("profile: hipMalloc failed"); return PTV3_ERR_LAUNCH; }
  }
  if (on) {
    (void)hipMemset(g_slots, 0, (size_t)MAX_SLOTS * 8);
    g_nslots = 0;
    for (auto& r : g_recs) { g_pool.push_back(r.e0); g_pool.push_back(r.e1); }
    g_recs.clear();
  }
  g_on = on != 0;
  return PTV3_OK;
}

extern "C" int ptv3_profile_hint_flops(double flops) {
  g_hint_flops = flops;
  return PTV3_OK;
}

extern "C" int ptv3_profile_kernel_count(void) { return PK_KERNELS; }
extern "C" const char* ptv3_profile_kernel_name(int kernel) {
  return kernel >= 0 && kernel < PK_KERNELS ? g_kernel_names[kernel] : "";
}

static int collect(int by_kernel, int n, double* ms, double* flops, double* bytes, int64_t* launches) {
  if (hipDeviceSynchronize() != hipSuccess) { set_error("profile: synchronize failed"); return PTV3_ERR_LAUNCH; }
  std::vector<unsigned long long> slots(g_nslots > 0 ? g_nslots : 1);
  if (g_nslots > 0) (void)hipMemcpy(slots.data(), g_slots, (size_t)g_nslots * 8, hipMemcpyDeviceToHost);
  for (int f = 0; f < n; ++f) { ms[f] = flops[f] = bytes[f] = 0.0; launches[f] = 0; }
  for (auto& r : g_recs) {
    float t = 0.f;
    (void)hipEventElapsedTime(&t, r.e0, r.e1);
    const int k = by_kernel ? r.kernel : r.family;
    ms[k] += t;
    flops[k] += r.slot >= 0 ? r.per_valid * (double)slots[r.slot] : r.flops;
    bytes[k] += r.bytes;
    launches[k] += 1;
  }
  return PTV3_OK;
}

extern "C" int ptv3_profile_collect_kernels(double* ms, double* flops, double* bytes, int64_t* launches) {
  return collect(1, PK_KERNELS, ms, flops, bytes, launches);
}

extern "C" int ptv3_profile_collect(double* ms, double* flops, double* bytes, int64_t* launches) {
  if (int rc = collect(0, PROF_FAMILIES, ms, flops, bytes, launches)) return rc;
  for (auto& r : g_recs) { g_pool.push_back(r.e0); g_pool.push_back(r.e1); }
  g_recs.clear();
  if (g_slots) (void)hipMemset(g_slots, 0, (size_t)MAX_SLOTS * 8);
  g_nslots = 0;
  return PTV3_OK;
}
```

### pointcept-keypointdetection_amd/csrc/sparse.hip

```cpp
#include <stdlib.h>
#include "common.h"
#include "hashtable.h"
#include "../../include/ptv3_hip.h"

namespace ptv3 {

__global__ void ht_insert_kernel(const int32_t* __restrict__ idx, int64_t n, unsigned long long* keys,
                                 int32_t* vals, uint64_t mask) {
  int64_t i = (int64_t)blockIdx.x * blockDim.x + threadIdx.x;
  if (i >= n) return;
  uint64_t key = site_key(idx[4 * i], idx[4 * i + 1], idx[4 * i + 2], idx[4 * i + 3]);
  uint64_t slot = mix64(key) & mask;
  for (uint64_t probe = 0; probe <= mask; ++probe) {
    unsigned long long prev = atomicCAS(&keys[slot], (unsigned long long)HT_EMPTY, (unsigned long long)key);
    if (prev == HT_EMPTY || prev == key) {
      atomicMin(&vals[slot], (int32_t)i);
      return;
    }
    slot = (slot + 1) & mask;
  }
}

__global__ void ht_neighbors_kernel(const int32_t* __restrict__ idx, int64_t n,
                                    const unsigned long long* __restrict__ keys,
                                    const int32_t* __restrict__ vals, uint64_t mask, int ksize, int kvol,
                                    int32_t* __restrict__ nbr) {
  int64_t t = (int64_t)blockIdx.x * blockDim.x + threadIdx.x;
  if (t >= n * kvol) return;
  int64_t i = t / kvol;
  int d = (int)(t - i * kvol);
  int c = d % ksize, b_ = (d / ksize) % ksize, a = d / (ksize * ksize);
  int half = ksize / 2;
  int x = idx[4 * i + 1] + a - half, y = idx[4 * i + 2] + b_ - half, z = idx[4 * i + 3] + c - half;
  int32_t found = -1;
  if (d == kvol / 2) {
    found = (int32_t)i;
  } else if (x >= 0 && y >= 0 && z >= 0 && x < 65536 && y < 65536 && z < 65536) {
    uint64_t key = site_key(idx[4 * i], x, y, z);
    uint64_t slot = mix64(key) & mask;
    for (uint64_t probe = 0; probe <= mask; ++probe) {
      unsigned long long kq = keys[slot];
      if (kq == key) { found = vals[slot]; break; }
      if (kq == HT_EMPTY) break;
      slot = (slot + 1) & mask;
    }
  }
  nbr[t] = found;
}

__global__ void ht_neighbors_half_kernel(const int32_t* __restrict__ idx, int64_t n,
                                         const unsigned long long* __restrict__ keys, const int32_t* __restrict__ vals,
                                         uint64_t mask, int ksize, int kvol, int slots_log2,
                                         int32_t* __restrict__ nbr) {
  const int hv = kvol / 2 + 1;
  const int64_t i = (int64_t)blockIdx.x * (256 >> slots_log2) + (threadIdx.x >> slots_log2);
  const int d = threadIdx.x & ((1 << slots_log2) - 1);
  if (i >= n || d >= hv) return;
  if (d == kvol / 2) { nbr[i * kvol + d] = (int32_t)i; return; }
  int c = d % ksize, b_ = (d / ksize) % ksize, a = d / (ksize * ksize);
  int half = ksize / 2;
  int x = idx[4 * i + 1] + a - half, y = idx[4 * i + 2] + b_ - half, z = idx[4 * i + 3] + c - half;
  if (!(x >= 0 && y >= 0 && z >= 0 && x < 65536 && y < 65536 && z < 65536)) return;
  uint64_t key = site_key(idx[4 * i], x, y, z);
  uint64_t slot = mix64(key) & mask;
  for (uint64_t probe = 0; probe <= mask; ++probe) {
    unsigned long long kq = keys[slot];
    if (kq == key) {
      const int32_t j = vals[slot];
      nbr[i * kvol + d] = j;
      nbr[(int64_t)j * kvol + (kvol - 1 - d)] = (int32_t)i;
      return;
    }
    if (kq == HT_EMPTY) return;
    slot = (slot + 1) & mask;
  }
}

struct BlockTable {
  BlockSlot* slots; uint32_t* payload; int32_t* counter; int32_t* site_slot; uint64_t smask; size_t zero_bytes;
};
static inline size_t bt_payload_bytes(int64_t n) { return ((size_t)n * 4 + 15) & ~(size_t)15; }
static inline BlockTable bt_layout(void* table, int64_t n) {
  const int64_t S = ptv3_subm_table_slots(n);
  char* p = (char*)table;
  BlockTable t;
  t.slots = (BlockSlot*)p;
  t.payload = (uint32_t*)(p + (size_t)S * sizeof(BlockSlot));
  t.counter = (int32_t*)((char*)t.payload + bt_payload_bytes(n));
  t.site_slot = (int32_t*)((char*)t.counter + 16);
  t.smask = (uint64_t)(S - 1);
  t.zero_bytes = (size_t)S * sizeof(BlockSlot) + bt_payload_bytes(n) + 16;
  return t;
}

__global__ void bt_sites_kernel(const int64_t* __restrict__ batch, const void* __restrict__ grid, int is_i64, int64_t n,
                                int32_t* __restrict__ idx, int64_t* __restrict__ grid64, uint4* __restrict__ zero,
                                int64_t zero16) {
  const int64_t i = (int64_t)blockIdx.x * blockDim.x + threadIdx.x;
  for (int64_t j = i; j < zero16; j += (int64_t)gridDim.x * blockDim.x) zero[j] = uint4{0u, 0u, 0u, 0u};
  if (i >= n) return;
  int64_t x, y, z;
  if (is_i64) {
    const int64_t* g = (const int64_t*)grid;
    x = g[3 * i]; y = g[3 * i + 1]; z = g[3 * i + 2];
  } else {
    const int32_t* g = (const int32_t*)grid;
    x = g[3 * i]; y = g[3 * i + 1]; z = g[3 * i + 2];
  }
  reinterpret_cast<int4*>(idx)[i] = int4{(int32_t)batch[i], (int32_t)x, (int32_t)y, (int32_t)z};
  if (grid64) { grid64[3 * i] = x; grid64[3 * i + 1] = y; grid64[3 * i + 2] = z; }
}

__global__ void bt_claim_kernel(const int32_t* __restrict__ idx, int64_t n, BlockSlot* slots, uint64_t smask,
                                int32_t* __restrict__ site_slot) {
  const int64_t i = (int64_t)blockIdx.x * blockDim.x + threadIdx.x;
  if (i >= n) return;
  const int4 s = reinterpret_cast<const int4*>(idx)[i];
  const uint64_t key = block_key(s.x, s.y >> 2, s.z >> 2, s.w >> 2);
  uint64_t slot = mix64(key) & smask;
  int32_t mine = -1;
  for (uint64_t probe = 0; probe <= smask; ++probe) {
    const unsigned long long prev = atomicCAS(&slots[slot].key, 0ull, (unsigned long long)key);
    if (prev == 0 || prev == key) {
      atomicOr(&slots[slot].mask, 1ull << block_bit(s.y, s.z, s.w));
      mine = (int32_t)slot;
      break;
    }
    slot = (slot + 1) & smask;
  }
  site_slot[i] = mine;
}

__global__ __launch_bounds__(256) void bt_base_kernel(BlockSlot* slots, int32_t* counter) {
  __shared__ int s_wave[4];
  __shared__ int s_start;
  const int64_t s0 = (int64_t)blockIdx.x * 1024 + threadIdx.x;
  const int lane = threadIdx.x & 63, wave = threadIdx.x >> 6;
  int cnt[4], mine = 0;
#pragma unroll
  for (int j = 0; j < 4; ++j) { cnt[j] = __popcll(slots[s0 + j * 256].mask); mine += cnt[j]; }
  int incl = mine;
#pragma unroll
  for (int o = 1; o < 64; o <<= 1) {
    const int up = __shfl_up(incl, o, 64);
    if (lane >= o) incl += up;
  }
  if (lane == 63) s_wave[wave] = incl;
  __syncthreads();
  if (threadIdx.x == 0) {
    const int total = s_wave[0] + s_wave[1] + s_wave[2] + s_wave[3];
    s_start = total ? atomicAdd(counter, total) : 0;
  }
  __syncthreads();
  int at = s_start + incl - mine;
  for (int w = 0; w < wave; ++w) at += s_wave[w];
#pragma unroll
  for (int j = 0; j < 4; ++j) {
    if (cnt[j]) slots[s0 + j * 256].base = at;
    at += cnt[j];
  }
}

__global__ void bt_payload_kernel(const int32_t* __restrict__ idx, int64_t n, const BlockSlot* __restrict__ slots,
                                  const int32_t* __restrict__ site_slot, uint32_t* payload) {
  const int64_t i = (int64_t)blockIdx.x * blockDim.x + threadIdx.x;
  if (i >= n) return;
  const int32_t slot = site_slot[i];
  if (slot < 0) return;
  const int4 s = reinterpret_cast<const int4*>(idx)[i];
  const unsigned long long m = slots[slot].mask;
  const int bit = block_bit(s.y, s.z, s.w);
  const int at = slots[slot].base + __popcll(m & ((1ull << bit) - 1));
  atomicMax(&payload[at], ~(uint32_t)i);
}

template <int K, int SITES>
__global__ __launch_bounds__(256) void bt_neighbors_kernel(const int32_t* __restrict__ idx, int64_t n,
                                                           const BlockSlot* __restrict__ slots, uint64_t smask,
                                                           const uint32_t* __restrict__ payload,
                                                           int32_t* __restrict__ nbr) {
  constexpr int KVOL = K * K * K, H = K / 2, NB = K <= 5 ? 2 : 3, NC = NB * NB * NB;
  constexpr int ITER = (SITES * KVOL + 255) / 256;
  __shared__ int4 s_site[SITES];
  __shared__ unsigned long long s_mask[SITES * NC];
  __shared__ int32_t s_base[SITES * NC];
  const int64_t i0 = (int64_t)blockIdx.x * SITES;
  for (int c = threadIdx.x; c < SITES * NC; c += 256) {
    const int s = c / NC, cc = c - s * NC;
    unsigned long long m = 0;
    int32_t base = 0;
    if (i0 + s < n) {
      const int4 p = reinterpret_cast<const int4*>(idx)[i0 + s];
      if (cc == 0) s_site[s] = p;
      const int cx = cc / (NB * NB), cy = (cc / NB) % NB, cz = cc % NB;
      const int bx0 = (p.y - H) >> 2, by0 = (p.z - H) >> 2, bz0 = (p.w - H) >> 2;
      const int bx = bx0 + cx, by = by0 + cy, bz = bz0 + cz;
      if (bx >= 0 && by >= 0 && bz >= 0 && bx <= ((p.y + H) >> 2) && by <= ((p.z + H) >> 2) &&
          bz <= ((p.w + H) >> 2) && bx < 16384 && by < 16384 && bz < 16384) {
        const int64_t slot = bt_find(slots, smask, p.x, bx, by, bz);
        if (slot >= 0) { m = slots[slot].mask; base = slots[slot].base; }
      }
    }
    s_mask[c] = m;
    s_base[c] = base;
  }
  __syncthreads();
  int32_t v[ITER];
#pragma unroll
  for (int it = 0; it < ITER; ++it) {
    const int t = threadIdx.x + it * 256;
    const int s = t / KVOL, d = t - s * KVOL;
    v[it] = -1;
    if (t < SITES * KVOL && i0 + s < n) {
      const int4 p = s_site[s];
      const int x = p.y + d / (K * K) - H, y = p.z + (d / K) % K - H, z = p.w + d % K - H;
      if (d == KVOL / 2) {
        v[it] = (int32_t)(i0 + s);
      } else if (x >= 0 && y >= 0 && z >= 0 && x < 65536 && y < 65536 && z < 65536) {
        const int c = s * NC + (((x >> 2) - ((p.y - H) >> 2)) * NB + ((y >> 2) - ((p.z - H) >> 2))) * NB +
                      ((z >> 2) - ((p.w - H) >> 2));
        const unsigned long long m = s_mask[c];
        const int bit = block_bit(x, y, z);
        if ((m >> bit) & 1) v[it] = (int32_t)~payload[s_base[c] + __popcll(m & ((1ull << bit) - 1))];
      }
    }
  }
#pragma unroll
  for (int it = 0; it < ITER; ++it) {
    const int t = threadIdx.x + it * 256;
    if (t < SITES * KVOL && i0 + t / KVOL < n) nbr[i0 * KVOL + t] = v[it];
  }
}

}

using namespace ptv3;

extern "C" int64_t ptv3_subm_table_slots(int64_t n) {
  int64_t s = 1024;
  while (s < 2 * n) s <<= 1;
  return s;
}

extern "C" int ptv3_subm_build_table(const int32_t* indices, int64_t n, void* table, int64_t slots,
                                     void* stream) {
  PTV3_REQUIRE(slots >= 2 * n && (slots & (slots - 1)) == 0, "subm_build_table: slots must be a power of two >= 2n");
  hipStream_t s = (hipStream_t)stream;
  unsigned long long* keys = (unsigned long long*)table;
  int32_t* vals = (int32_t*)((char*)table + slots * 8);
  if (hipMemsetAsync(keys, 0xFF, (size_t)slots * 8, s) != hipSuccess) {
    set_error("subm_build_table: memset failed");
    return PTV3_ERR_LAUNCH;
  }
  if (hipMemsetAsync(vals, 0x7F, (size_t)slots * 4, s) != hipSuccess) {
    set_error("subm_build_table: memset failed");
    return PTV3_ERR_LAUNCH;
  }
  if (n == 0) return PTV3_OK;
  hipLaunchKernelGGL(ht_insert_kernel, dim3((unsigned)cdiv(n, 256)), dim3(256), 0, s, indices, n, keys, vals,
                     (uint64_t)(slots - 1));
  PTV3_LAUNCH_CHECK();
  return PTV3_OK;
}

extern "C" int ptv3_subm_neighbors(const int32_t* indices, int64_t n, const void* table, int64_t slots,
                                   int ksize, int32_t* nbr, void* stream) {
  PTV3_REQUIRE(ksize >= 1 && ksize <= 7 && (ksize & 1), "subm_neighbors: ksize %d must be odd and <= 7", ksize);
  if (n == 0) return PTV3_OK;
  const int kvol = ksize * ksize * ksize;
  const unsigned long long* keys = (const unsigned long long*)table;
  const int32_t* vals = (const int32_t*)((const char*)table + slots * 8);
  const char* sym = getenv("PTV3_NBR_SYMMETRIC");
  if (sym && atoi(sym) == 0) {
    hipLaunchKernelGGL(ht_neighbors_kernel, dim3((unsigned)cdiv(n * kvol, 256)), dim3(256), 0,
                       (hipStream_t)stream, indices, n, keys, vals, (uint64_t)(slots - 1), ksize, kvol, nbr);
  } else {
    if (hipMemsetAsync(nbr, 0xFF, (size_t)n * kvol * sizeof(int32_t), (hipStream_t)stream) != hipSuccess) {
      set_error("subm_neighbors: memset failed");
      return PTV3_ERR_LAUNCH;
    }
    int sl = 0;
    while ((1 << sl) < kvol / 2 + 1) ++sl;
    hipLaunchKernelGGL(ht_neighbors_half_kernel, dim3((unsigned)cdiv(n, 256 >> sl)), dim3(256), 0,
                       (hipStream_t)stream, indices, n, keys, vals, (uint64_t)(slots - 1), ksize, kvol, sl, nbr);
  }
  PTV3_LAUNCH_CHECK();
  return PTV3_OK;
}

extern "C" size_t ptv3_subm_block_table_bytes(int64_t n) {
  if (n < 0) n = 0;
  return (size_t)ptv3_subm_table_slots(n) * sizeof(BlockSlot) + 2 * bt_payload_bytes(n) + 16;
}

extern "C" int ptv3_subm_sites(const int64_t* batch, const void* grid_coord, int coord_is_i64, int64_t n,
                               int32_t* indices, int64_t* grid64, void* table, size_t bytes, void* stream) {
  PTV3_REQUIRE(n >= 0 && n < ((int64_t)1 << 31), "subm_sites: n=%lld out of range", (long long)n);
  PTV3_REQUIRE(table && bytes >= ptv3_subm_block_table_bytes(n) && ((uintptr_t)table & 15) == 0,
               "subm_sites: table must be 16-byte aligned and hold ptv3_subm_block_table_bytes(n) bytes");
  PTV3_REQUIRE(n == 0 || (batch && grid_coord && indices), "subm_sites: batch, grid_coord and indices are required");
  PTV3_REQUIRE(((uintptr_t)indices & 15) == 0, "subm_sites: indices must be 16-byte aligned");
  const BlockTable t = bt_layout(table, n);
  hipLaunchKernelGGL(bt_sites_kernel, dim3((unsigned)cdiv(n > 0 ? n : 1, 256)), dim3(256), 0, (hipStream_t)stream, batch,
                     grid_coord, coord_is_i64, n, indices, grid64, (uint4*)table, (int64_t)(t.zero_bytes / 16));
  PTV3_LAUNCH_CHECK();
  return PTV3_OK;
}

static int build_block_table(const int32_t* indices, int64_t n, void* table, size_t bytes, bool zeroed, void* stream) {
  PTV3_REQUIRE(n >= 0 && n < ((int64_t)1 << 31), "subm_build_block_table: n=%lld out of range", (long long)n);
  PTV3_REQUIRE(table && bytes >= ptv3_subm_block_table_bytes(n) && ((uintptr_t)table & 15) == 0,
               "subm_build_block_table: table must be 16-byte aligned and hold ptv3_subm_block_table_bytes(n) bytes");
  PTV3_REQUIRE(n == 0 || indices, "subm_build_block_table: indices are required");
  hipStream_t s = (hipStream_t)stream;
  const BlockTable t = bt_layout(table, n);
  if (!zeroed && hipMemsetAsync(table, 0, t.zero_bytes, s) != hipSuccess) {
    set_error("subm_build_block_table: memset failed");
    return PTV3_ERR_LAUNCH;
  }
  if (n == 0) return PTV3_OK;
  const dim3 sites((unsigned)cdiv(n, 256)), block(256);
  hipLaunchKernelGGL(bt_claim_kernel, sites, block, 0, s, indices, n, t.slots, t.smask, t.site_slot);
  hipLaunchKernelGGL(bt_base_kernel, dim3((unsigned)((t.smask + 1) / 1024)), block, 0, s, t.slots, t.counter);
  hipLaunchKernelGGL(bt_payload_kernel, sites, block, 0, s, indices, n, t.slots, t.site_slot, t.payload);
  PTV3_LAUNCH_CHECK();
  return PTV3_OK;
}

extern "C" int ptv3_subm_build_block_table(const int32_t* indices, int64_t n, void* table, size_t bytes,
                                           void* stream) {
  return build_block_table(indices, n, table, bytes, false, stream);
}

extern "C" int ptv3_subm_build_block_table_zeroed(const int32_t* indices, int64_t n, void* table, size_t bytes,
                                                  void* stream) {
  return build_block_table(indices, n, table, bytes, true, stream);
}

template <int K, int SITES>
static void bt_neighbors_launch(const int32_t* indices, int64_t n, const BlockTable& t, int32_t* nbr, hipStream_t s) {
  hipLaunchKernelGGL((bt_neighbors_kernel<K, SITES>), dim3((unsigned)cdiv(n, SITES)), dim3(256), 0, s, indices, n,
                     t.slots, t.smask, t.payload, nbr);
}

extern "C" int ptv3_subm_neighbors_blocks(const int32_t* indices, int64_t n, const void* table, size_t bytes,
                                          int ksize, int32_t* nbr, void* stream) {
  PTV3_REQUIRE(ksize >= 1 && ksize <= 7 && (ksize & 1), "subm_neighbors_blocks: ksize %d must be odd and <= 7", ksize);
  PTV3_REQUIRE(n >= 0 && n < ((int64_t)1 << 31), "subm_neighbors_blocks: n=%lld out of range", (long long)n);
  PTV3_REQUIRE(table && bytes >= ptv3_subm_block_table_bytes(n) && ((uintptr_t)table & 15) == 0,
               "subm_neighbors_blocks: table must be the one ptv3_subm_build_block_table built for these n sites");
  if (n == 0) return PTV3_OK;
  PTV3_REQUIRE(indices && nbr, "subm_neighbors_blocks: indices and nbr are required");
  const BlockTable t = bt_layout(const_cast<void*>(table), n);
  hipStream_t s = (hipStream_t)stream;
  switch (ksize) {
    case 1: bt_neighbors_launch<1, 256>(indices, n, t, nbr, s); break;
    case 3: bt_neighbors_launch<3, 16>(indices, n, t, nbr, s); break;
    case 5: bt_neighbors_launch<5, 16>(indices, n, t, nbr, s); break;
    default: bt_neighbors_launch<7, 4>(indices, n, t, nbr, s); break;
  }
  PTV3_LAUNCH_CHECK();
  return PTV3_OK;
}
```

### pointcept-keypointdetection_amd/ptv3_hip/lib.py

```python
import ctypes
import os
from ctypes import c_char_p, c_double, c_float, c_int, c_int64, c_size_t, c_uint32, c_void_p

PTV3_F32, PTV3_BF16 = 0, 1
ACT_NONE, ACT_GELU, ACT_RELU = 0, 1, 2
ORDER_IDS = {"z": 0, "z-trans": 1, "hilbert": 2, "hilbert-trans": 3}

_HERE = os.path.dirname(os.path.abspath(__file__))


def library_path():
    return os.environ.get("PTV3_HIP_LIB", os.path.join(os.path.dirname(_HERE), "lib", "libptv3_hip.so"))


P = c_void_p


class BlockTrain(ctypes.Structure):
    _fields_ = ([("n", c_int64), ("n_pad", c_int64)] +
                [(k, ctypes.c_int32) for k in ("c", "hidden", "heads", "patch", "kvol", "num_windows", "dtype", "reserved")] +
                [("scale", c_float), ("eps", c_float), ("keep1", c_float), ("keep2", c_float), ("sum_len_sq", c_double)] +
                [(k, P) for k in ("nbr", "row_order", "win_order", "win_inverse", "cu_seqlens", "feat", "conv_feat",
                                  "w_conv", "w_lin", "w_qkv", "w_proj", "w_fc1", "w_fc2",
                                  "wt_conv", "wt_lin", "wt_qkv", "wt_proj", "wt_fc1", "wt_fc2",
                                  "b_conv", "b_lin", "b_qkv", "b_proj", "b_fc1", "b_fc2", "g0", "b0", "g1", "b1", "g2", "b2",
                                  "mask1", "mask2",
                                  "c1", "c2", "f1", "t3", "qkv", "a", "f2", "t5", "h0", "h", "out",
                                  "dout", "dfeat", "dconv_feat",
                                  "dw_conv", "dw_lin", "dw_qkv", "dw_proj", "dw_fc1", "dw_fc2",
                                  "db_conv", "db_lin", "db_qkv", "db_proj", "db_fc1", "db_fc2",
                                  "dln0", "dln1", "dln2", "workspace")] +
                [("workspace_bytes", c_size_t), ("attn_lse", P)])


SIGNATURES = {
    "ptv3_last_error": (c_char_p, []),
    "ptv3_version": (c_int, []),
    "ptv3_sfc_encode": (c_int, [P, c_int, P, c_int64, c_int, P, c_int, P, P]),
    "ptv3_argsort_workspace_bytes": (c_size_t, [c_int, c_int64]),
    "ptv3_argsort_i64": (c_int, [P, c_int, c_int64, c_int, P, P, P, c_size_t, P]),
    "ptv3_argsort_i64_rows": (c_int, [P, c_int, c_int64, c_int, P, P, P, P, c_size_t, P]),
    "ptv3_argsort_scan_batch": (c_int, []),
    "ptv3_coord_max": (c_int, [P, c_int, c_int64, P, P, P]),
    "ptv3_subm_sites": (c_int, [P, P, c_int, c_int64, P, P, P, c_size_t, P]),
    "ptv3_subm_build_block_table_zeroed": (c_int, [P, c_int64, P, c_size_t, P]),
    "ptv3_pad_plan": (c_int, [P, c_int, c_int64, c_int64, c_int, P, P, P, P]),
    "ptv3_window_maps": (c_int, [P, P, P, P, c_int64, c_int64, P, P, P]),
    "ptv3_window_plan": (c_int, [P, P, P, c_int, c_int, c_int64, c_int64, c_int, P, P, P, P]),
    "ptv3_window_attn_fwd": (c_int, [P, P, P, P, c_int64, c_int64, c_int, c_int, c_int, c_float, P, c_int, P]),
    "ptv3_window_attn_varlen_fwd": (c_int, [P, P, P, P, c_int, P, c_int64, c_int64, c_int, c_int, c_int, c_float,
                                            c_double, c_int, P]),
    "ptv3_window_attn_rpe_fwd": (c_int, [P, P, P, P, c_int64, c_int64, c_int, c_int, c_int, c_float, P, P, c_int,
                                         c_int, P]),
    "ptv3_subm_table_slots": (c_int64, [c_int64]),
    "ptv3_subm_build_table": (c_int, [P, c_int64, P, c_int64, P]),
    "ptv3_subm_neighbors": (c_int, [P, c_int64, P, c_int64, c_int, P, P]),
    "ptv3_subm_block_table_bytes": (c_size_t, [c_int64]),
    "ptv3_subm_build_block_table": (c_int, [P, c_int64, P, c_size_t, P]),
    "ptv3_subm_neighbors_blocks": (c_int, [P, c_int64, P, c_size_t, c_int, P, P]),
    "ptv3_gemm_workspace_bytes": (c_size_t, [c_int64, c_int, c_int, c_int, c_int]),
    "ptv3_gemm": (c_int, [P, P, P, c_int64, c_int, c_int, c_int, P, P, P, P, P, c_int, P, P, P, c_int, P, c_size_t,
                          P]),
    "ptv3_gemm_splits": (c_int, [c_int64, c_int, c_int, c_int, c_int]),
    "ptv3_block_fusable": (c_int, [c_int, c_int, c_int, c_int64]),
    "ptv3_rows_linear_capable": (c_int, [c_int, c_int, c_int, c_int64]),
    "ptv3_rows_linear": (c_int, [P, P, P, P, P, P, P, P, c_int, P, P, P, c_int64, c_int, c_int, c_float, c_int, P]),
    "ptv3_block_head": (c_int, [P, P, c_int, P, P, P, P, P, P, P, P, P, P, c_int64, c_int, c_float, c_int, P]),
    "ptv3_block_tail": (c_int, [P, P, P, P, P, P, P, P, P, P, P, c_int64, c_int, c_int, c_float, c_int, P]),
    "ptv3_rows_linear_ln_capable": (c_int, [c_int, c_int, c_int]),
    "ptv3_rows_linear_ln": (c_int, [P, P, P, P, P, P, c_int64, c_int, c_int, c_float, c_int, c_int, P]),
    "ptv3_subm_conv_ln_capable": (c_int, [c_int, c_int, c_int]),
    "ptv3_subm_conv_ln": (c_int, [P, P, P, P, P, P, P, P, c_int64, c_int, c_int, c_float, c_int, c_int, P]),
    "ptv3_res_conv_capable": (c_int, [c_int64, c_int, c_int, c_int, c_int]),
    "ptv3_res_conv_row_tiles": (c_int, [c_int64, c_int]),
    "ptv3_res_conv": (c_int, [P, P, P, P, P, P, P, P, c_int, P, P, P, P, P, c_int64, c_int, c_int, c_int, c_int, P]),
    "ptv3_mlp2_fusable": (c_int, [c_int, c_int, c_int, c_int]),
    "ptv3_mlp2": (c_int, [P, P, P, P, P, c_int, P, P, P, c_int, c_int64, c_int, c_int, c_int, c_int, P]),
    "ptv3_layernorm": (c_int, [P, P, P, P, P, P, P, P, c_int64, c_int, c_float, c_int, P]),
    "ptv3_layernorm_slabs": (c_int, [P, c_int, P, P, P, P, P, P, P, P, c_int64, c_int, c_float, c_int, P]),
    "ptv3_affine_act": (c_int, [P, P, P, c_int, P, c_int64, c_int, c_int, P]),
    "ptv3_cast": (c_int, [P, c_int, P, c_int, c_int64, P]),
    "ptv3_pool_workspace_bytes": (c_size_t, [c_int64]),
    "ptv3_pool_segments": (c_int, [P, P, c_int64, c_int, P, P, P, P, P, P, c_size_t, P]),
    "ptv3_pool_reduce": (c_int, [P, P, P, P, P, c_int, P, P, c_int64, c_int64, c_int, c_int, P, P, c_int, P, P, P,
                                 P, P, P, c_int, P]),
    "ptv3_forward_workspace_bytes": (c_size_t, [P, c_int64, c_int]),
    "ptv3_forward": (c_int, [P, P, c_int, P, P, c_size_t, P]),
    "ptv3_executor_create": (c_void_p, []),
    "ptv3_executor_destroy": (c_int, [P]),
    "ptv3_block_train_workspace_bytes": (c_size_t, [P, c_int]),
    "ptv3_block_train_fwd": (c_int, [P, P]),
    "ptv3_block_train_bwd": (c_int, [P, P]),
    "ptv3_gemm_tn_workspace_bytes": (c_size_t, [c_int64, c_int, c_int, c_int]),
    "ptv3_gemm_tn": (c_int, [P, P, P, P, P, c_int64, c_int, c_int, c_int, c_int, P, c_size_t, P]),
    "ptv3_col_reduce_workspace_bytes": (c_size_t, [c_int64, c_int]),
    "ptv3_col_reduce": (c_int, [P, P, P, P, c_float, c_int, P, c_int64, c_int, c_int, P, c_size_t, P]),
    "ptv3_bn_finalize": (c_int, [P, P, c_int64, P, P, P, P, c_float, c_float, P, P, P, P, c_int, P]),
    "ptv3_bn_bwd_coeffs": (c_int, [P, c_int64, P, P, P, P, P, P, c_int, P]),
    "ptv3_layernorm_bwd": (c_int, [P, P, P, P, c_float, P, P, c_int64, c_int, c_int, P, c_size_t, P]),
    "ptv3_act_bwd": (c_int, [P, P, P, P, c_int, P, c_int64, c_int, c_int, P]),
    "ptv3_affine2": (c_int, [P, P, P, P, P, P, c_int64, c_int, c_int, P]),
    "ptv3_pool_max_bwd": (c_int, [P, P, P, P, c_int64, c_int, P, c_int, P]),
    "ptv3_segment_sum": (c_int, [P, P, P, c_int64, c_int, P, c_int, P]),
    "ptv3_window_attn_bwd_workspace_bytes": (c_size_t, [c_int64, c_int64, c_int, c_int, c_int]),
    "ptv3_window_attn_bwd": (c_int, [P, P, P, P, P, P, c_int64, c_int64, c_int, c_int, c_int, c_float, c_int, P,
                                     c_size_t, P]),
    "ptv3_window_attn_varlen_bwd": (c_int, [P, P, P, P, P, P, c_int, P, c_int64, c_int64, c_int, c_int, c_int, c_float,
                                            c_int, P, c_size_t, P]),
    "ptv3_window_attn_train_fwd": (c_int, [P, P, P, P, c_int, P, P, c_int64, c_int64, c_int, c_int, c_int, c_float,
                                           c_double, c_int, P]),
    "ptv3_window_attn_train_bwd": (c_int, [P, P, P, P, P, P, P, c_int, P, c_int64, c_int64, c_int, c_int, c_int, c_float,
                                           c_int, P, c_size_t, P]),
    "ptv3_window_attn_drop_fwd": (c_int, [P, P, P, P, c_int, P, c_int64, c_int64, c_int, c_int, c_int, c_float, c_float,
                                          c_uint32, c_int, P]),
    "ptv3_window_attn_drop_bwd": (c_int, [P, P, P, P, P, P, c_int, P, c_int64, c_int64, c_int, c_int, c_int, c_float,
                                          c_float, c_uint32, c_int, P, c_size_t, P]),
    "ptv3_window_attn_rpe_bwd_workspace_bytes": (c_size_t, [c_int64, c_int64, c_int, c_int, c_int, c_int, c_int]),
    "ptv3_window_attn_rpe_bwd": (c_int, [P, P, P, P, P, P, P, c_int, P, P, c_int64, c_int64, c_int, c_int, c_int,
                                         c_float, c_int, P, c_size_t, P]),
    "ptv3_adamw_entry_bytes": (c_size_t, []),
    "ptv3_adamw_chunk": (c_int, []),
    "ptv3_adamw_fill_entry": (c_int, [P, P, P, P, P, c_int64, c_int, c_int]),
    "ptv3_adamw_fill_shadow": (c_int, [P, P, P, c_int, c_int, c_int, c_int]),
    "ptv3_adamw_fill_step_lag": (c_int, [P, c_int64]),
    "ptv3_adamw_step": (c_int, [P, c_int, c_int, P, P, c_int, c_float, c_float, c_float, c_int64, c_float, P, P, c_int,
                                c_int, P]),
    "ptv3_adamw_shadow_tiles": (c_int, [c_int, c_int, c_int]),
    "ptv3_adamw_fill_first_tile": (c_int, [P, c_int]),
    "ptv3_grad_sqnorm": (c_int, [P, c_int, c_int, P, P, P, P, P]),
    "ptv3_grid_hash": (c_int, [P, c_int64, c_double, c_int, P, P, P, P]),
    "ptv3_keypoint_aggregate": (c_int, [P, P, P, c_int, c_int, P, P, c_int, c_float, P, P, P]),
    "ptv3_scene_mean_workspace_bytes": (c_size_t, [c_int64, c_int, c_int]),
    "ptv3_scene_mean": (c_int, [P, P, c_int64, c_int, c_int, c_int, P, P, c_size_t, P]),
    "ptv3_scene_mean_head": (c_int, [P, P, c_int64, c_int, c_int, c_int, P, P, P, P, c_int, P, P, P, P, c_int, P, P,
                                     c_size_t, P]),
    "ptv3_scene_mean_bwd": (c_int, [P, P, c_int64, c_int, c_int, P, c_int, P]),
    "ptv3_scene_median_workspace_bytes": (c_size_t, [c_int, c_int]),
    "ptv3_scene_median": (c_int, [P, P, P, c_int64, c_int, c_int, P, P, c_size_t, P]),
    "ptv3_vote_loss_workspace_bytes": (c_size_t, [c_int64, c_int, c_int]),
    "ptv3_vote_loss": (c_int, [P, P, P, c_int, P, P, c_int, c_int64, c_int, c_int, c_float, P, P, P, c_size_t, P]),
    "ptv3_vote_loss_bwd": (c_int, [P, P, P, P, c_int, P, P, c_int64, c_int, c_int, c_float, P, P]),
    "ptv3_profile_enable": (c_int, [c_int]),
    "ptv3_profile_collect": (c_int, [P, P, P, P]),
    "ptv3_profile_hint_flops": (c_int, [ctypes.c_double]),
    "ptv3_profile_kernel_count": (c_int, []),
    "ptv3_profile_kernel_name": (c_char_p, [c_int]),
    "ptv3_profile_collect_kernels": (c_int, [P, P, P, P]),
    "ptv3_swin_window_keys": (c_int, [P, c_int64, c_int, c_int, c_int, P, P, P]),
    "ptv3_swin_attn_fwd": (c_int, [P, P, P, P, P, P, P, c_int, P, P, c_int, P, P, c_int64, c_int, c_int, c_int, c_int, P]),
    "ptv3_swin_attn_bwd": (c_int, [P, P, P, P, P, P, P, P, c_int, P, P, c_int, P, P, P, P, P, P, P, c_int64, c_int, c_int,
                                   c_int, c_int, P]),
    "ptv3_knn_query": (c_int, [c_int, c_int, P, P, P, P, c_int, P, P, P]),
    "ptv3_knn_query_cells": (c_int, [c_int, c_int, P, P, P, P, c_int64, P, P, P, c_float, P, P, P]),
    "ptv3_grouping_forward": (c_int, [c_int, c_int, c_int, P, P, P, P]),
    "ptv3_grouping_backward": (c_int, [c_int, c_int, c_int, P, P, P, P]),
    "ptv3_interpolation_forward": (c_int, [c_int, c_int, c_int, P, P, P, P, P]),
    "ptv3_interpolation_backward": (c_int, [c_int, c_int, c_int, P, P, P, P, P]),
    "ptv3_farthest_point_sampling": (c_int, [c_int, c_int, P, P, P, P, P, P]),
    "ptv3_vector_attn_fwd": (c_int, [P, P, P, P, P, c_int64, c_int, c_int, P, P, P, P, P, P, P, P, P, P, P, P, P, P]),
    "ptv3_down2_keys": (c_int, [P, c_int64, c_int, c_int, c_int, c_int64, P, P, P]),
    "ptv3_down2_children": (c_int, [P, P, P, P, P, P, P, c_int64, c_int64, P, P, P, P, P, P]),
    "ptv3_down2_conv": (c_int, [P, P, P, c_int64, c_int64, c_int, c_int, P, P, c_int, P, P]),
    "ptv3_up2_conv": (c_int, [P, P, P, P, P, c_int64, c_int64, c_int, c_int, P, P, c_int, P, P]),
    "ptv3_cluster_keys": (c_int, [P, c_int64, P, c_int, P, P]),
    "ptv3_cluster_center": (c_int, [P, c_int64, P, P, P, c_int64, c_int, P, P]),
    "ptv3_cluster_softmax_sum": (c_int, [P, c_int64, P, c_int64, P, P, P, P, c_int64, c_int, P, P]),
    "ptv3_cluster_mix": (c_int, [P, c_int64, P, P, c_int, P, c_int64, c_int64, c_int, P, c_int64, c_int, P]),
    "ptv3_add_act": (c_int, [P, P, c_int, P, c_int64, P]),
    "ptv3_gva_fwd": (c_int, [P, P, P, P, P, c_int64, c_int, c_int, c_int, P, P, P, P, P, P, P, P, P, P, P, P]),
    "ptv3_grid_keys": (c_int, [P, c_int64, P, c_int, c_float, P, P, P, P, P]),
    "ptv3_segment_mean3": (c_int, [P, P, P, c_int64, P, P]),
    "ptv3_strat_cell_keys": (c_int, [P, c_int64, P, c_int, P, c_float, c_int, P, P, P, P]),
    "ptv3_strat_key_count": (c_int, [P, P, P, P, P, P, P, P, P, P, c_int64, P, P]),
    "ptv3_strat_key_fill": (c_int, [P, P, P, P, P, P, P, P, P, P, P, c_int64, c_int64, P, P, P, P]),
    "ptv3_strat_rel_index": (c_int, [P, P, P, c_int64, c_float, c_float, c_int, P, P]),
    "ptv3_strat_attn_capable": (c_int, [c_int, c_int, c_int]),
    "ptv3_strat_attn_fwd": (c_int, [P, P, P, c_int64, P, P, P, P, P, P, P, P, c_int64, c_int, c_int, c_int, c_float,
                                    c_float, c_float, P, P]),
    "ptv3_ball_query": (c_int, [P, P, c_int, c_int64, c_float, c_int, P, P]),
    "ptv3_octree_keys": (c_int, [P, P, c_int, c_int64, c_float, c_int, P, P, P]),
    "ptv3_octree_attn_capable": (c_int, [c_int, c_int, c_int, c_int]),
    "ptv3_octree_attn_fwd": (c_int, [P, P, P, P, P, c_int64, c_int, c_int, c_int, c_int, c_int, c_float, P]),
    "ptv3_octree_dwconv": (c_int, [P, P, P, P, P, P, c_int64, c_int, P]),
    "ptv3_lovasz_scan_tile": (c_int, []),
    "ptv3_lovasz_workspace_bytes": (c_size_t, [c_int64, c_int]),
    "ptv3_lovasz_fwd": (c_int, [P, P, c_int64, c_int, c_int64, c_float, P, P, P, P, P, c_size_t, P]),
    "ptv3_lovasz_bwd": (c_int, [P, P, P, P, P, c_int64, c_int, c_int64, c_float, P, P]),
    "ptv3_focal_workspace_bytes": (c_size_t, [c_int64, c_int]),
    "ptv3_focal_fwd": (c_int, [P, P, P, c_int64, c_int, c_int64, c_float, c_float, c_int, P, P, P, c_size_t, P]),
    "ptv3_focal_bwd": (c_int, [P, P, P, P, P, c_int64, c_int, c_int64, c_float, c_float, c_int, P, P]),
}


class _Lib:

    def __init__(self):
        self._dll = None

    def load(self):
        if self._dll is None:
            path = library_path()
            if not os.path.exists(path):
                raise ImportError(
                    f"libptv3_hip.so not found at {path}: build it with `make -C pointcept-keypointdetection_amd` "
                    "(or __graft_entry__.build()); there is no CPU fallback for the PTv3 HIP path")
            dll = ctypes.CDLL(path)
            for name, (res, args) in SIGNATURES.items():
                fn = getattr(dll, name)
                fn.restype, fn.argtypes = res, args
            self._dll = dll
        return self._dll

    def __getattr__(self, name):
        return getattr(self.load(), name)

    def check(self, rc, what):
# ... 6 lines not shown
```

### pointcept-keypointdetection_amd/ptv3_hip/ops.py

```python
import ctypes
from types import SimpleNamespace

import torch

from .lib import lib, PTV3_F32, PTV3_BF16, ACT_NONE, ACT_GELU, ACT_RELU, ORDER_IDS

_DT = {torch.float32: PTV3_F32, torch.bfloat16: PTV3_BF16}

_raw_stream = torch._C._cuda_getCurrentRawStream if hasattr(torch._C, "_cuda_getCurrentRawStream") else None


def _stream():
    if _raw_stream is not None:
        return _raw_stream(torch.cuda.current_device())
    return torch.cuda.current_stream().cuda_stream


def _p(t):
    return None if t is None else t.data_ptr()


def _chk(t, name, dtype=None, dim=None):
    if t is None:
        return
# ... 172 lines not shown
    return window_attention_varlen(qkv, win_order, win_inverse, cu_seqlens, heads, patch, scale, sum_len_sq)


def window_attention_train(qkv, win_order, win_inverse, heads, patch, scale, cu_seqlens=None, sum_len_sq=0.0):
    n, c, n_pad, nwin = _attn_check("window_attention_train", qkv, win_order, win_inverse, heads, patch, cu_seqlens)
    out = torch.empty((n, c), dtype=qkv.dtype, device=qkv.device)
    lse = torch.empty((n_pad, int(heads)), dtype=torch.float32, device=qkv.device)
    lib.check(lib.ptv3_window_attn_train_fwd(_p(qkv), _p(win_order), _p(win_inverse), _p(cu_seqlens), nwin, _p(out),
                                             _p(lse), n, n_pad, c, int(heads), int(patch), float(scale),
                                             float(sum_len_sq), _dt(qkv), _stream()), "ptv3_window_attn_train_fwd")
    return out, lse


def window_attention_train_bwd(qkv, out, dout, lse, win_order, win_inverse, heads, patch, scale, cu_seqlens=None):
    n, c, n_pad, nwin = _attn_check("window_attention_train_bwd", qkv, win_order, win_inverse, heads, patch, cu_seqlens,
                                    out, dout, lse)
    dqkv = torch.empty_like(qkv)
    nb = lib.ptv3_window_attn_bwd_workspace_bytes(n, n_pad, c, int(heads), _dt(qkv))
    ws = _ws(nb, qkv.device)
    lib.check(lib.ptv3_window_attn_train_bwd(_p(qkv), _p(out), _p(dout), _p(lse), _p(win_order), _p(win_inverse),
                                             _p(cu_seqlens), nwin, _p(dqkv), n, n_pad, c, int(heads), int(patch),
                                             float(scale), _dt(qkv), _p(ws), nb, _stream()), "ptv3_window_attn_train_bwd")
    return dqkv


def window_attention_drop(qkv, win_order, win_inverse, heads, patch, scale, p_drop, seed, cu_seqlens=None):
    n, c, n_pad, nwin = _attn_check("window_attention_drop", qkv, win_order, win_inverse, heads, patch, cu_seqlens)
    out = torch.empty((n, c), dtype=qkv.dtype, device=qkv.device)
    lib.check(lib.ptv3_window_attn_drop_fwd(_p(qkv), _p(win_order), _p(win_inverse), _p(cu_seqlens), nwin, _p(out), n,
                                            n_pad, c, int(heads), int(patch), float(scale), float(p_drop),
                                            int(seed) & 0xFFFFFFFF, _dt(qkv), _stream()), "ptv3_window_attn_drop_fwd")
    return out


def window_attention_drop_bwd(qkv, out, dout, win_order, win_inverse, heads, patch, scale, p_drop, seed, cu_seqlens=None):
    n, c, n_pad, nwin = _attn_check("window_attention_drop_bwd", qkv, win_order, win_inverse, heads, patch, cu_seqlens,
                                    out, dout)
    dqkv = torch.empty_like(qkv)
    nb = lib.ptv3_window_attn_bwd_workspace_bytes(n, n_pad, c, int(heads), _dt(qkv))
    ws = _ws(nb, qkv.device)
    lib.check(lib.ptv3_window_attn_drop_bwd(_p(qkv), _p(out), _p(dout), _p(win_order), _p(win_inverse), _p(cu_seqlens),
                                            nwin, _p(dqkv), n, n_pad, c, int(heads), int(patch), float(scale),
                                            float(p_drop), int(seed) & 0xFFFFFFFF, _dt(qkv), _p(ws), nb, _stream()),
              "ptv3_window_attn_drop_bwd")
    return dqkv


def drop_keep_mask(slot, head, key, heads, seed, p_drop):
    import numpy as np
    idv = ((np.asarray(slot, np.uint64) * np.uint64(heads) + np.asarray(head, np.uint64)) << np.uint64(14)) | np.asarray(key, np.uint64)
    lo = (idv & np.uint64(0xFFFFFFFF)).astype(np.uint64)
    hi = (idv >> np.uint64(32)).astype(np.uint64)
    m32 = np.uint64(0xFFFFFFFF)
    x = ((lo * np.uint64(0x9E3779B1)) & m32) ^ ((hi * np.uint64(0x85EBCA77)) & m32) ^ np.uint64(int(seed) & 0xFFFFFFFF)
    x ^= x >> np.uint64(16)
    x = (x * np.uint64(0x7FEB352D)) & m32
    x ^= x >> np.uint64(15)
    x = (x * np.uint64(0x846CA68B)) & m32
    x ^= x >> np.uint64(16)
    thr = np.uint64(min(4294967295, int(float(np.float32(p_drop)) * 4294967296.0)))
    return x >= thr


def window_attention_rpe(qkv, win_order, win_inverse, heads, patch, scale, grid_coord, rpe_table, pos_bnd):
    n, c, n_pad, _ = _attn_check("window_attention_rpe", qkv, win_order, win_inverse, heads, patch,
                                 grid_coord=grid_coord, rpe_table=rpe_table, pos_bnd=pos_bnd)
    out = torch.empty((n, c), dtype=qkv.dtype, device=qkv.device)
    rc = lib.ptv3_window_attn_rpe_fwd(_p(qkv), _p(win_order), _p(win_inverse), _p(out), n, n_pad, c, int(heads),
                                      int(patch), float(scale), _p(grid_coord), _p(rpe_table), int(pos_bnd), _dt(qkv),
                                      _stream())
    if rc == 3:
        return None
    lib.check(rc, "ptv3_window_attn_rpe_fwd")
    return out


def subm_neighbors(indices, ksize, table=None):
    _chk(indices, "indices", torch.int32, 2)
    n = indices.shape[0]
    if table is None:
        slots = lib.ptv3_subm_table_slots(n)
        table = torch.empty(slots * 12, dtype=torch.uint8, device=indices.device)
        lib.check(lib.ptv3_subm_build_table(_p(indices), n, _p(table), slots, _stream()), "ptv3_subm_build_table")
    slots = table.numel() // 12
    nbr = torch.empty((n, ksize ** 3), dtype=torch.int32, device=indices.device)
    lib.check(lib.ptv3_subm_neighbors(_p(indices), n, _p(table), slots, int(ksize), _p(nbr), _stream()),
              "ptv3_subm_neighbors")
    return nbr, table


def subm_neighbors_blocks(indices, ksize, table=None):
    _chk(indices, "indices", torch.int32, 2)
    n = indices.shape[0]
    if table is None:
        table = torch.empty(lib.ptv3_subm_block_table_bytes(n), dtype=torch.uint8, device=indices.device)
        lib.check(lib.ptv3_subm_build_block_table(_p(indices), n, _p(table), table.numel(), _stream()),
                  "ptv3_subm_build_block_table")
    nbr = torch.empty((n, ksize ** 3), dtype=torch.int32, device=indices.device)
    lib.check(lib.ptv3_subm_neighbors_blocks(_p(indices), n, _p(table), table.numel(), int(ksize), _p(nbr), _stream()),
              "ptv3_subm_neighbors_blocks")
    return nbr, table


def subm_sites_table(batch, grid_coord):
    _chk(batch, "batch", torch.int64, 1)
    _chk(grid_coord, "grid_coord", (torch.int32, torch.int64), 2)
    n = grid_coord.shape[0]
    indices = torch.empty((n, 4), dtype=torch.int32, device=batch.device)
    grid64 = torch.empty((n, 3), dtype=torch.int64, device=batch.device)
    table = torch.empty(lib.ptv3_subm_block_table_bytes(n), dtype=torch.uint8, device=batch.device)
    lib.check(lib.ptv3_subm_sites(_p(batch), _p(grid_coord), int(grid_coord.dtype == torch.int64), n, _p(indices),
                                  _p(grid64), _p(table), table.numel(), _stream()), "ptv3_subm_sites")
    lib.check(lib.ptv3_subm_build_block_table_zeroed(_p(indices), n, _p(table), table.numel(), _stream()),
              "ptv3_subm_build_block_table_zeroed")
    return indices, grid64, table


def gemm(x, w, bias=None, nbr=None, kvol=1, row_order=None, bn_scale=None, bn_shift=None, act=ACT_NONE,
         res=None, res_index=None, dual=False, m=None):
    _chk(x, "x", (torch.float32, torch.bfloat16), 2)
    _chk(w, "w", x.dtype)
    for t, nm in ((bias, "bias"), (bn_scale, "bn_scale"), (bn_shift, "bn_shift")):
        _chk(t, nm, torch.float32, 1)
    _chk(nbr, "nbr", torch.int32, 2)
    _chk(row_order, "row_order", torch.int32, 1)
    _chk(res, "res", x.dtype, 2)
    _chk(res_index, "res_index", torch.int32, 1)
    cin = x.shape[1]
    cout = w.shape[0]
    if w.numel() != cout * kvol * cin:
        raise RuntimeError(f"gemm: weight has {w.numel()} elements, expected {cout}x{kvol}x{cin}")
    if m is None:
        m = nbr.shape[0] if nbr is not None else x.shape[0]
    if nbr is not None and (nbr.shape[0] != m or nbr.shape[1] != kvol):
        raise RuntimeError("gemm: neighbour table shape mismatch")
    for t in (bias, bn_scale, bn_shift):
        if t is not None and t.numel() != cout:
            raise RuntimeError("gemm: epilogue vector length != cout")
    if res is not None:
        if res.shape[1] != cout or (res_index is None and res.shape[0] != m):
            raise RuntimeError("gemm: residual shape mismatch")
        if res_index is not None and res_index.shape[0] != m:
            raise RuntimeError("gemm: res_index length != m")
    if row_order is not None and row_order.shape[0] != m:
        raise RuntimeError("gemm: row_order length != m")
    out = torch.empty((m, cout), dtype=x.dtype, device=x.device)
    out2 = torch.empty_like(out) if dual else None
    dt = _dt(x)
    ws_bytes = lib.ptv3_gemm_workspace_bytes(m, cin, cout, int(kvol), dt)
    ws = torch.empty(ws_bytes, dtype=torch.uint8, device=x.device) if ws_bytes else None
    lib.check(lib.ptv3_gemm(_p(x), _p(w), _p(out), m, cin, cout, int(kvol), _p(nbr), _p(row_order), _p(bias),
                            _p(bn_scale), _p(bn_shift), int(act), _p(res), _p(res_index), _p(out2), dt, _p(ws),
                            ws_bytes, _stream()), "ptv3_gemm")
    return (out, out2) if dual else out


def gemm_splits(m, cin, cout, kvol, dtype):
    return int(lib.ptv3_gemm_splits(int(m), int(cin), int(cout), int(kvol), _DT[dtype]))


def block_fusable(c, hidden, dtype, m=0):
    return int(lib.ptv3_block_fusable(int(c), int(hidden), _DT[dtype], int(m)))


def chain_permute(w, dtype):
    if dtype == torch.float32:
        return w
    k = w.shape[1]
    assert k % 32 == 0
    base = [(4 * g + e) if e < 4 else (16 + 4 * g + e - 4) for g in range(4) for e in range(8)]
    perm = torch.tensor([32 * q + b for q in range(k // 32) for b in base], device=w.device)
    return w.index_select(1, perm).contiguous()


def conv_slabs(x, w, nbr, kvol, row_order=None):
    m, cin, cout = nbr.shape[0], x.shape[1], w.shape[0]
    dt = _dt(x)
    splits = lib.ptv3_gemm_splits(m, cin, cout, int(kvol), dt)
    if splits <= 1:
        return None
    ws_bytes = lib.ptv3_gemm_workspace_bytes(m, cin, cout, int(kvol), dt)
    ws = torch.empty(ws_bytes, dtype=torch.uint8, device=x.device)
    lib.check(lib.ptv3_gemm(_p(x), _p(w), None, m, cin, cout, int(kvol), _p(nbr), _p(row_order), None, None, None, 0,
                            None, None, None, dt, _p(ws), ws_bytes, _stream()), "ptv3_gemm(slabs)")
    return ws, splits


def rows_linear_rows():
    import os
    return int(os.environ.get("PTV3_ROWS_MIN", "0"))


def rows_linear_capable(c, cout, dtype, m):
    return bool(lib.ptv3_rows_linear_capable(int(c), int(cout), _DT[dtype], int(m)))


def rows_linear(x, w, bias, act=ACT_NONE, res=None, ln=None, ln0=None, shortcut=None, eps=1e-5):
    _chk(x, "x", (torch.float32, torch.bfloat16), 2)
    _chk(w, "w", x.dtype, 2)
    m, c = x.shape
    cout = w.shape[0]
    out = torch.empty((m, cout), dtype=x.dtype, device=x.device)
    f1 = torch.empty_like(x) if ln0 is not None else None
    g0, b0 = ln0 if ln0 is not None else (None, None)
    g1, b1 = ln if ln is not None else (None, None)
    lib.check(lib.ptv3_rows_linear(_p(x), _p(shortcut), _p(g0), _p(b0), _p(g1), _p(b1), _p(w), _p(bias), int(act), _p(res),
                                   _p(f1), _p(out), m, c, cout, float(eps), _dt(x), _stream()), "ptv3_rows_linear")
    return (f1, out) if ln0 is not None else out


def rows_linear_ln_capable(c, cout, dtype):
    return dtype in _DT and bool(lib.ptv3_rows_linear_ln_capable(int(c), int(cout), _DT[dtype]))


def subm_conv_ln_capable(c, kvol, dtype):
    return dtype in _DT and bool(lib.ptv3_subm_conv_ln_capable(int(c), int(kvol), _DT[dtype]))


def _chk_ln(name, cout, bias, gamma, beta):
    for t, nm in ((bias, "bias"), (gamma, "gamma"), (beta, "beta")):
        _chk(t, f"{name}: {nm}", torch.float32, 1)
        if t is not None and t.numel() != cout:
            raise RuntimeError(f"{name}: {nm} has {t.numel()} entries, expected {cout}")


def rows_linear_ln(x, w, bias, gamma, beta, eps=1e-5, act=ACT_RELU, out=None):
    _chk(x, "x", (torch.float32, torch.bfloat16), 2)
    _chk(w, "w", x.dtype, 2)
    m, c = x.shape
    cout = w.shape[0]
    if w.shape[1] != c:
        raise RuntimeError(f"rows_linear_ln: weight {tuple(w.shape)} does not match x {tuple(x.shape)}")
    _chk_ln("rows_linear_ln", cout, bias, gamma, beta)
    if out is None:
        out = torch.empty((m, cout), dtype=x.dtype, device=x.device)
    _chk(out, "out", x.dtype, 2)
    if tuple(out.shape) != (m, cout):
        raise RuntimeError("rows_linear_ln: out shape mismatch")
    lib.check(lib.ptv3_rows_linear_ln(_p(x), _p(w), _p(bias), _p(gamma), _p(beta), _p(out), m, c, cout, float(eps),
                                      int(act), _dt(x), _stream()), "ptv3_rows_linear_ln")
    return out


def subm_conv_ln(x, w, nbr, bias, gamma, beta, eps=1e-5, act=ACT_RELU, row_order=None, out=None):
    _chk(x, "x", (torch.float32, torch.bfloat16), 2)
    _chk(w, "w", x.dtype)
    _chk(nbr, "nbr", torch.int32, 2)
    _chk(row_order, "row_order", torch.int32, 1)
    m, c = x.shape
    kvol = nbr.shape[1]
    if nbr.shape[0] != m:
        raise RuntimeError("subm_conv_ln: neighbour table has another row count than x")
    if w.numel() != c * kvol * c:
        raise RuntimeError(f"subm_conv_ln: weight has {w.numel()} elements, expected {c}x{kvol}x{c}")
    if row_order is not None and row_order.shape[0] != m:
        raise RuntimeError("subm_conv_ln: row_order length != m")
    _chk_ln("subm_conv_ln", c, bias, gamma, beta)
    if out is None:
        out = torch.empty((m, c), dtype=x.dtype, device=x.device)
    _chk(out, "out", x.dtype, 2)
    if tuple(out.shape) != (m, c):
        raise RuntimeError("subm_conv_ln: out shape mismatch")
    lib.check(lib.ptv3_subm_conv_ln(_p(x), _p(w), _p(nbr), _p(row_order), _p(bias), _p(gamma), _p(beta), _p(out), m, c,
                                    int(kvol), float(eps), int(act), _dt(x), _stream()), "ptv3_subm_conv_ln")
    return out


def block_head(x, slab, splits, conv_bias, shortcut, g0, b0, g1, b1, wqkv, bqkv, eps):
    _chk(shortcut, "shortcut", (torch.float32, torch.bfloat16), 2)
    m, c = shortcut.shape
    f1 = torch.empty_like(shortcut)
    qkv = torch.empty((m, 3 * c), dtype=shortcut.dtype, device=shortcut.device)
    lib.check(lib.ptv3_block_head(_p(x), _p(slab), int(splits), _p(conv_bias), _p(shortcut), _p(g0), _p(b0), _p(g1),
                                  _p(b1), _p(wqkv), _p(bqkv), _p(f1), _p(qkv), m, c, float(eps), _dt(shortcut),
                                  _stream()), "ptv3_block_head")
    return f1, qkv


def block_tail(attn, f1, wproj, bproj, g2, b2, w1, bias1, w2, bias2, eps):
    _chk(attn, "attn", (torch.float32, torch.bfloat16), 2)
    _chk(f1, "f1", attn.dtype, 2)
    m, c = attn.shape
    out = torch.empty_like(attn)
    lib.check(lib.ptv3_block_tail(_p(attn), _p(f1), _p(wproj), _p(bproj), _p(g2), _p(b2), _p(w1), _p(bias1), _p(w2),
                                  _p(bias2), _p(out), m, c, int(w1.shape[0]), float(eps), _dt(attn), _stream()),
              "ptv3_block_tail")
    return out


def mlp2_fusable(cin, hidden, cout, dtype):
    return bool(lib.ptv3_mlp2_fusable(int(cin), int(hidden), int(cout), _DT[dtype]))


def mlp2_weight2(w2, dtype):
    w = w2.detach().to(dtype)
    rows = 16 if w.shape[0] <= 16 else 32 if w.shape[0] <= 32 else 64
    pad = rows - w.shape[0]
    if pad:
        w = torch.nn.functional.pad(w, (0, 0, 0, pad))
    return chain_permute(w.contiguous(), dtype)


def mlp2(x, w1, b1, s1, t1, act, w2p, b2, cout, out_f32=True):
    _chk(x, "x", (torch.float32, torch.bfloat16), 2)
    _chk(w1, "w1", x.dtype, 2)
    _chk(w2p, "w2p", x.dtype, 2)
# ... 1403 lines not shown
```

Before: 40.05 Mpoints/s.

## Add halo-tiled submanifold conv with precomputed per-tile unique-neighbour plan

```diff
diff --git a/include/ptv3_hip.h b/include/ptv3_hip.h
--- a/include/ptv3_hip.h
+++ b/include/ptv3_hip.h
@@ -80,6 +80,16 @@
               const int32_t* nbr, const int32_t* row_order, const float* bias, const float* bn_scale,
               const float* bn_shift, int act, const void* res, const int32_t* res_index, void* out2,
               int dtype, void* workspace, size_t workspace_bytes, void* stream);
+
+size_t ptv3_halo_plan_bytes(int64_t m);
+int ptv3_halo_plan_shape(int* tile_sites, int* cap_rows);
+int ptv3_halo_plan_build(const int32_t* nbr, const int32_t* row_order, int64_t m, void* plan, size_t bytes,
+                         void* stream);
+int ptv3_conv_halo_policy(int64_t m, int cin, int cout, int kvol, int dtype);
+int ptv3_conv_halo(const void* x, const void* w, void* out, int64_t m, int c, const int32_t* nbr,
+                   const int32_t* row_order, const void* plan, size_t plan_bytes, const float* bias,
+                   const float* bn_scale, const float* bn_shift, int act, const void* res, const int32_t* res_index,
+                   void* out2, int dtype, void* stream);
 
 int ptv3_block_fusable(int c, int hidden, int dtype, int64_t m);
 int ptv3_rows_linear_capable(int c, int cout, int dtype, int64_t m);
diff --git a/pointcept-keypointdetection_amd/csrc/engine.hip b/pointcept-keypointdetection_amd/csrc/engine.hip
--- a/pointcept-keypointdetection_amd/csrc/engine.hip
+++ b/pointcept-keypointdetection_amd/csrc/engine.hip
@@ -111,6 +111,7 @@
   int64_t *code = nullptr, *order = nullptr, *inverse = nullptr;
   int32_t* indices = nullptr; void* table = nullptr; size_t table_bytes = 0;
   int32_t* nbr3 = nullptr; int32_t* nbr5 = nullptr; int32_t* row_order = nullptr;
+  void* halo = nullptr; size_t halo_bytes = 0; hipEvent_t halo_ready = nullptr; bool halo_waited = false;
   Plan plan[2];
   int32_t* seg = nullptr;
   int64_t* cluster = nullptr;
@@ -251,6 +252,27 @@
     F->off = mark;
   }
 
+  void halo_plan(Level& L, int st) {
+    const bool dec_here = !d->enc_mode && st < d->num_stages - 1;
+    if (!ptv3_conv_halo_policy(L.n, d->enc_channels[st], d->enc_channels[st], 27, d->dtype) &&
+        !(dec_here && ptv3_conv_halo_policy(L.n, d->dec_channels[st], d->dec_channels[st], 27, d->dtype)))
+      return;
+    L.halo_bytes = ptv3_halo_plan_bytes(L.n);
+    L.halo = G->alloc(L.halo_bytes);
+    RUN(ptv3_halo_plan_build(L.nbr3, L.row_order, L.n, L.halo, L.halo_bytes, sg));
+    if (!dry && ok()) { L.halo_ready = X->event_at(40 + st); (void)hipEventRecord(L.halo_ready, sg); }
+  }
+
+  void conv3(Level& L, const void* w, void* out, int C, const float* bias, bool first_block) {
+    if (L.halo && !first_block && ptv3_conv_halo_policy(L.n, C, C, 27, d->dtype)) {
+      if (!dry && ok() && !L.halo_waited) { (void)hipStreamWaitEvent(sf, L.halo_ready, 0); L.halo_waited = true; }
+      RUN(ptv3_conv_halo(L.conv_feat, w, out, L.n, C, L.nbr3, L.row_order, L.halo, L.halo_bytes, bias, nullptr, nullptr, 0,
+                         nullptr, nullptr, nullptr, d->dtype, sf));
+      return;
+    }
+    gemm(L.conv_feat, w, out, L.n, C, C, 27, L.nbr3, L.row_order, bias, nullptr, nullptr, 0, nullptr, nullptr, nullptr);
+  }
+
   bool rows_path(int64_t n, int C, int hidden) const {
     static const int64_t min_rows = [] { const char* e = getenv("PTV3_ROWS_MIN"); return e ? atoll(e) : (int64_t)0; }();
     return n >= min_rows && ptv3_rows_linear_capable(C, 3 * C, d->dtype, n) && ptv3_rows_linear_capable(C, C, d->dtype, n) &&
@@ -333,7 +355,7 @@
     RUN(window_attn_forward(a, {"window_attn", WA_RAGGED_OPTIONAL}));
   }
 
-  void block(Level& L, const Plan& P, int C, int H, int oi) {
+  void block(Level& L, const Plan& P, int C, int H, int oi, bool first = false) {
     const void* conv_w = next(); const float* conv_b = (const float*)next();
     const float* ln0_g = (const float*)next(); const float* ln0_b = (const float*)next();
     const float* n1_g = (const float*)next(); const float* n1_b = (const float*)next();
@@ -358,7 +380,7 @@
                             C, d->ln_eps, d->dtype, sf));
       } else {
         void* t2 = F->alloc(row * C);
-        gemm(L.conv_feat, conv_w, t2, L.n, C, C, 27, L.nbr3, L.row_order, conv_b, nullptr, nullptr, 0, nullptr, nullptr, nullptr);
+        conv3(L, conv_w, t2, C, conv_b, first);
         RUN(ptv3_block_head(t2, nullptr, 0, nullptr, L.feat, ln0_g, ln0_b, n1_g, n1_b, qkv_w, qkv_b, f1, qkv, L.n, C,
                             d->ln_eps, d->dtype, sf));
       }
@@ -380,11 +402,11 @@
                                  d->dtype, sf));
         gemm(t3, qkv_w, qkv, L.n, C, 3 * C, 1, nullptr, nullptr, qkv_b, nullptr, nullptr, 0, nullptr, nullptr, nullptr);
       } else if (rows) {
-        gemm(L.conv_feat, conv_w, t2, L.n, C, C, 27, L.nbr3, L.row_order, conv_b, nullptr, nullptr, 0, nullptr, nullptr, nullptr);
+        conv3(L, conv_w, t2, C, conv_b, first);
         RUN(ptv3_rows_linear(t2, L.feat, ln0_g, ln0_b, n1_g, n1_b, qkv_w, qkv_b, 0, nullptr, f1, qkv, L.n, C, 3 * C,
                              d->ln_eps, d->dtype, sf));
       } else {
-        gemm(L.conv_feat, conv_w, t2, L.n, C, C, 27, L.nbr3, L.row_order, conv_b, nullptr, nullptr, 0, nullptr, nullptr, nullptr);
+        conv3(L, conv_w, t2, C, conv_b, first);
         RUN(ptv3_layernorm(t2, ln0_g, ln0_b, L.feat, f1, n1_g, n1_b, t3, L.n, C, d->ln_eps, d->dtype, sf));
         gemm(t3, qkv_w, qkv, L.n, C, 3 * C, 1, nullptr, nullptr, qkv_b, nullptr, nullptr, 0, nullptr, nullptr, nullptr);
       }
@@ -496,6 +518,7 @@
   R.level_tables(L0, 0);
   if (io->stage_points_host) io->stage_points_host[0] = L0.n;
   if (!dry && R.ok()) { L0.ready = X->event_at(1); (void)hipEventRecord(L0.ready, sg); }
+  R.halo_plan(L0, 0);
 
   auto wait_level = [&](Level& L) { if (!dry && R.ok()) (void)hipStreamWaitEvent(sf, L.ready, 0); };
   struct PoolParams { const void* w; const float *b, *bns, *bnt; };
@@ -563,6 +586,7 @@
           hipLaunchKernelGGL(i64_to_i32_kernel, dim3((unsigned)cdiv(P.n, 256)), dim3(256), 0, sg, P.cluster, P.cluster32, P.n);
       }
       if (!dry && R.ok()) { L.ready = X->event_at(1 + st); (void)hipEventRecord(L.ready, sg); }
+      R.halo_plan(L, st);
       wait_level(L);
       L.feat = F.alloc((size_t)L.n * C * es);
       const size_t mark = F.off;
@@ -574,7 +598,7 @@
       L.conv_feat = L.feat;
     }
     for (int i = 0; i < d->enc_depths[st]; ++i)
-      R.block(L, L.plan[0], d->enc_channels[st], d->enc_heads[st], i % k);
+      R.block(L, L.plan[0], d->enc_channels[st], d->enc_heads[st], i % k, i == 0);
     if (!R.ok()) break;
   }
   if (!d->enc_mode && R.ok()) {
diff --git a/pointcept-keypointdetection_amd/csrc/gemm.hip b/pointcept-keypointdetection_amd/csrc/gemm.hip
--- a/pointcept-keypointdetection_amd/csrc/gemm.hip
+++ b/pointcept-keypointdetection_amd/csrc/gemm.hip
@@ -4,6 +4,7 @@
 #include "common.h"
 #include "profile.h"
 #include "block_args.h"
+#include "halo_plan.h"
 #include "../../include/ptv3_hip.h"
 
 namespace ptv3 {
@@ -775,6 +776,266 @@
   }
   __syncthreads();
   store_tile<T, 8>(a, sOut, OS, GC_BM, BN, row0, n0, tid, NTH);
+}
+
+static int choose_splits(int64_t m, int cin, int cout, int kvol, int dtype, int* steps_per_split);
+constexpr int64_t HALO_MIN_ROWS = 40000;
+
+struct HaloArgs { const int32_t* count; const int32_t* rows; const uint16_t* slots; };
+
+template <typename T, int C>
+struct HaloShape {
+  static constexpr int RB = C * (int)sizeof(T);
+  static constexpr int TPS = RB == 64 ? 2 : 1;
+  static constexpr int NSTG = (HALO_TAPS + TPS - 1) / TPS;
+  static constexpr int HALO = (HALO_CAP + 1) * RB;
+  static constexpr int WBUF = TPS * C * RB;
+  static constexpr int SLOT = HALO_T * HALO_TAPS * 2;
+  static constexpr int EPI = 3 * C * 4;
+  static constexpr int LDS = HALO + 2 * WBUF + SLOT + EPI;
+  static_assert(HALO >= HALO_T * (RB + 16), "the staged output tile overlays the halo");
+  static_assert(LDS <= 160 * 1024, "conv_halo_kernel: LDS");
+};
+
+template <typename T, int C>
+__global__ void __launch_bounds__(256) conv_halo_kernel(GemmArgs a, HaloArgs h) {
+  typedef Frag<T> F;
+  typedef typename F::type FR;
+  typedef HaloShape<T, C> S;
+  constexpr int E = F::E;
+  constexpr int RB = S::RB, CPR = RB / 16;
+  constexpr int KQ = C / F::KC;
+  constexpr int MI = 2, NJ = C / 16;
+  constexpr int TPS = S::TPS, NSTG = S::NSTG;
+  constexpr int WCH = C * CPR;
+  constexpr int W_LOADS = TPS * WCH / 256;
+  constexpr int RING = 3;
+  constexpr int RPP = 256 / CPR;
+  constexpr int G_LOADS = HALO_T / RPP;
+  constexpr int NP = (HALO_CAP + RPP - 1) / RPP;
+  constexpr int FB = NP > 14 ? 14 : NP;
+  constexpr int NB = (NP + FB - 1) / FB;
+  static_assert(HALO_T * RB + HALO_T * HALO_TAPS * 4 <= (HALO_CAP + 1) * RB, "slow path: rows 0..127 + the table fit the halo image");
+  static_assert(TPS * WCH % 256 == 0, "a weight stage is a whole number of chunks per thread");
+  extern __shared__ __attribute__((aligned(16))) char hc_smem[];
+  char* sHalo = hc_smem;
+  char* sW = sHalo + S::HALO;
+  unsigned short* sSlot = reinterpret_cast<unsigned short*>(sW + 2 * S::WBUF);
+  float* sEpi = reinterpret_cast<float*>(sW + 2 * S::WBUF + S::SLOT);
+
+  const T* __restrict__ x = reinterpret_cast<const T*>(a.x);
+  const T* __restrict__ w = reinterpret_cast<const T*>(a.w);
+  const int tid = threadIdx.x, lane = tid & 63, wave = tid >> 6;
+  const int li = lane & 15, g = lane >> 4;
+  const int64_t tile = xcd_remap(blockIdx.x, gridDim.x), row0 = tile * HALO_T;
+  int id[NP];
+#pragma unroll
+  for (int u = 0; u < NP; ++u) id[u] = h.rows[tile * HALO_CAP + min(tid / CPR + RPP * u, HALO_CAP - 1)];
+  const int cnt = h.count[tile];
+  const bool fast = cnt <= HALO_CAP;
+  auto swz = [](int r) { return CPR == 4 ? ((0 - (r >> 2)) & 3) : CPR == 8 ? ((r >> 1) & 7) : (r & 15); };
+  auto chunk_at = [&](char* img, int r, int c) { return reinterpret_cast<FR*>(img + r * RB + 16 * (c ^ swz(r))); };
+  auto frag_at = [&](const char* img, int r, int q) {
+    return *reinterpret_cast<const FR*>(img + r * RB + 16 * ((4 * q + g) ^ swz(r)));
+  };
+
+  park_epi(a, sEpi, C, 0, tid, 256);
+  int w_t[W_LOADS], w_o[W_LOADS], w_c[W_LOADS];
+#pragma unroll
+  for (int u = 0; u < W_LOADS; ++u) {
+    const int e = tid + 256 * u;
+    w_t[u] = e / WCH;
+    w_o[u] = (e % WCH) / CPR;
+    w_c[u] = e % CPR;
+  }
+  auto issue_w = [&](int stage, FR (&rw)[W_LOADS]) {
+#pragma unroll
+    for (int u = 0; u < W_LOADS; ++u) {
+      const int d = min(stage * TPS + w_t[u], HALO_TAPS - 1);
+      rw[u] = *reinterpret_cast<const FR*>(w + ((int64_t)w_o[u] * HALO_TAPS + d) * C + E * w_c[u]);
+    }
+  };
+  auto stash_w = [&](int buf, const FR (&rw)[W_LOADS]) {
+#pragma unroll
+    for (int u = 0; u < W_LOADS; ++u) *chunk_at(sW + buf * S::WBUF + w_t[u] * (C * RB), w_o[u], w_c[u]) = rw[u];
+  };
+
+  f32x4 acc[MI][NJ];
+#pragma unroll
+  for (int m = 0; m < MI; ++m)
+#pragma unroll
+    for (int j = 0; j < NJ; ++j) acc[m][j] = f32x4{0.f, 0.f, 0.f, 0.f};
+
+  if (tid < CPR) *reinterpret_cast<FR*>(sHalo + HALO_CAP * RB + 16 * tid) = F::zero();
+  if (fast) {
+    FR rw[RING][W_LOADS];
+    issue_w(0, rw[0]);
+    issue_w(1, rw[1]);
+    issue_w(2, rw[2]);
+    {
+      const s16x8* src = reinterpret_cast<const s16x8*>(h.slots + tile * (HALO_T * HALO_TAPS));
+      constexpr int NCH = S::SLOT / 16;
+      s16x8 v[2];
+#pragma unroll
+      for (int u = 0; u < 2; ++u) v[u] = src[min(tid + 256 * u, NCH - 1)];
+#pragma unroll
+      for (int u = 0; u < 2; ++u) {
+#pragma unroll
+        for (int i = 0; i < 8; ++i)
+          if ((unsigned short)v[u][i] == (unsigned short)HALO_ABSENT) v[u][i] = (short)HALO_CAP;
+        if (tid + 256 * u < NCH) reinterpret_cast<s16x8*>(sSlot)[tid + 256 * u] = v[u];
+      }
+    }
+    const int fr = tid / CPR, fc = tid % CPR;
+    static_for<0, NB>([&](auto bc) {
+      constexpr int b = decltype(bc)::value;
+      if (b * FB * RPP < cnt) {
+        FR v[FB];
+#pragma unroll
+        for (int u = 0; u < FB; ++u) {
+          const int r = fr + RPP * (b * FB + u);
+          const int src = (b * FB + u < NP && r < cnt) ? id[b * FB + u < NP ? b * FB + u : 0] : 0;
+          v[u] = *reinterpret_cast<const FR*>(x + (int64_t)src * C + E * fc);
+        }
+#pragma unroll
+        for (int u = 0; u < FB; ++u) {
+          const int r = fr + RPP * (b * FB + u);
+          if (r < cnt) *chunk_at(sHalo, r, fc) = v[u];
+        }
+      }
+    });
+    stash_w(0, rw[0]);
+    issue_w(3, rw[0]);
+    __syncthreads();
+    const unsigned short* my_slots = sSlot + (32 * wave + li) * HALO_TAPS;
+    int sl[2][TPS][MI];
+    FR xf[2][TPS][KQ][MI];
+    auto read_slots = [&](int stage, int (&o)[TPS][MI]) {
+#pragma unroll
+      for (int t = 0; t < TPS; ++t)
+#pragma unroll
+        for (int m = 0; m < MI; ++m) o[t][m] = my_slots[16 * m * HALO_TAPS + min(stage * TPS + t, HALO_TAPS - 1)];
+    };
+    auto read_x = [&](const int (&sv)[TPS][MI], FR (&o)[TPS][KQ][MI]) {
+#pragma unroll
+      for (int t = 0; t < TPS; ++t)
+#pragma unroll
+        for (int q = 0; q < KQ; ++q)
+#pragma unroll
+          for (int m = 0; m < MI; ++m) o[t][q][m] = frag_at(sHalo, sv[t][m], q);
+    };
+    read_slots(0, sl[0]);
+    read_x(sl[0], xf[0]);
+    read_slots(1, sl[1]);
+    static_for<0, NSTG>([&](auto sc) {
+      constexpr int s = decltype(sc)::value;
+      if constexpr (s + 1 < NSTG) stash_w((s + 1) & 1, rw[(s + 1) % RING]);
+      if constexpr (s + 4 < NSTG) issue_w(s + 4, rw[(s + 1) % RING]);
+      const char* bw = sW + (s & 1) * S::WBUF;
+      FR wf[TPS][KQ][NJ];
+#pragma unroll
+      for (int t = 0; t < TPS; ++t)
+#pragma unroll
+        for (int q = 0; q < KQ; ++q)
+#pragma unroll
+          for (int j = 0; j < NJ; ++j) wf[t][q][j] = frag_at(bw + t * (C * RB), 16 * j + li, q);
+      if constexpr (s + 1 < NSTG) read_x(sl[(s + 1) & 1], xf[(s + 1) & 1]);
+      if constexpr (s + 2 < NSTG) read_slots(s + 2, sl[s & 1]);
+#pragma unroll
+      for (int t = 0; t < TPS; ++t) {
+        if (s * TPS + t >= HALO_TAPS) continue;
+#pragma unroll
+        for (int q = 0; q < KQ; ++q)
+#pragma unroll
+          for (int m = 0; m < MI; ++m)
+#pragma unroll
+            for (int j = 0; j < NJ; ++j)
+              acc[m][j] = F::mma(wf[t][q][j], xf[s & 1][t][q][m], acc[m][j]);
+      }
+      __syncthreads();
+    });
+  } else {
+    int32_t* sNbr = reinterpret_cast<int32_t*>(sHalo + HALO_T * RB);
+    {
+      constexpr int PER = (HALO_T * HALO_TAPS + 255) / 256;
+      int64_t orow[PER];
+#pragma unroll
+      for (int u = 0; u < PER; ++u) {
+        const int64_t r = row0 + (tid + 256 * u) / HALO_TAPS;
+        const int64_t rs = r < a.m ? r : 0;
+        orow[u] = a.row_order ? (int64_t)a.row_order[rs] : rs;
+      }
+      int32_t nv[PER];
+#pragma unroll
+      for (int u = 0; u < PER; ++u) nv[u] = a.nbr[orow[u] * HALO_TAPS + (tid + 256 * u) % HALO_TAPS];
+#pragma unroll
+      for (int u = 0; u < PER; ++u) {
+        const int e = tid + 256 * u;
+        if (e < HALO_T * HALO_TAPS) sNbr[e] = row0 + e / HALO_TAPS < a.m ? nv[u] : -1;
+      }
+    }
+    __syncthreads();
+    const int gr = tid / CPR, gc = tid % CPR;
+    FR rw[W_LOADS];
+    int32_t nb[G_LOADS];
+    FR v[G_LOADS];
+    auto fetch = [&](int d) {
+#pragma unroll
+      for (int u = 0; u < G_LOADS; ++u) nb[u] = sNbr[(gr + RPP * u) * HALO_TAPS + d];
+#pragma unroll
+      for (int u = 0; u < G_LOADS; ++u) v[u] = *reinterpret_cast<const FR*>(x + (int64_t)(nb[u] >= 0 ? nb[u] : 0) * C + E * gc);
+    };
+    issue_w(0, rw);
+    fetch(0);
+    for (int d = 0; d < HALO_TAPS; ++d) {
+      const int t = d % TPS;
+      __syncthreads();
+#pragma unroll
+      for (int u = 0; u < G_LOADS; ++u) *chunk_at(sHalo, gr + RPP * u, gc) = nb[u] >= 0 ? v[u] : F::zero();
+      if (t == 0) stash_w(0, rw);
+      __syncthreads();
+      if (d + 1 < HALO_TAPS) {
+        fetch(d + 1);
+        if ((d + 1) % TPS == 0) issue_w((d + 1) / TPS, rw);
+      }
+      const char* bw = sW + t * (C * RB);
+#pragma unroll
+      for (int q = 0; q < KQ; ++q) {
+        FR xs[MI], ws[NJ];
+#pragma unroll
+        for (int m = 0; m < MI; ++m) xs[m] = frag_at(sHalo, 32 * wave + 16 * m + li, q);
+#pragma unroll
+        for (int j = 0; j < NJ; ++j) ws[j] = frag_at(bw, 16 * j + li, q);
+#pragma unroll
+        for (int m = 0; m < MI; ++m)
+#pragma unroll
+          for (int j = 0; j < NJ; ++j) acc[m][j] = F::mma(ws[j], xs[m], acc[m][j]);
+      }
+    }
+    __syncthreads();
+  }
+
+  constexpr int OS = C + 16 / (int)sizeof(T);
+  T* sOut = reinterpret_cast<T*>(hc_smem);
+#pragma unroll
+  for (int j = 0; j < NJ; ++j) {
+    const EpiVec ev = load_epi(sEpi, C, 16 * j + 4 * g);
+#pragma unroll
+    for (int m = 0; m < MI; ++m) stage_values<T>(a, sOut, OS, 32 * wave + 16 * m + li, 16 * j + 4 * g, ev, acc[m][j]);
+  }
+  __syncthreads();
+  store_tile<T, HALO_T * C / Chunk16<T>::N / 256>(a, sOut, OS, HALO_T, C, row0, 0, tid, 256);
+}
+
+static bool use_conv_halo(int64_t m, int cin, int cout, int kvol, int dtype) {
+  const char* env = getenv("PTV3_CONV_HALO");
+  const int mode = env ? atoi(env) : 1;
+  if (mode == 0 || kvol != HALO_TAPS || cin != cout || (cin != 32 && cin != 64)) return false;
+  if (dtype != PTV3_F32 && dtype != PTV3_BF16) return false;
+  if (mode == 2) return true;
+  int sps;
+  if (choose_splits(m, cin, cout, kvol, dtype, &sps) > 1) return false;
+  return dtype == PTV3_BF16 && m >= HALO_MIN_ROWS;
 }
 
 static bool use_conv_tile(int64_t m, int cin, int cout, int kvol, int dtype, int64_t x_bytes, int* bn_out, int splits) {
@@ -1037,3 +1298,46 @@
   PTV3_LAUNCH_CHECK();
   return PTV3_OK;
 }
+
+extern "C" int ptv3_conv_halo_policy(int64_t m, int cin, int cout, int kvol, int dtype) {
+  return use_conv_halo(m, cin, cout, kvol, dtype) ? 1 : 0;
+}
+
+extern "C" int ptv3_conv_halo(const void* x, const void* w, void* out, int64_t m, int c, const int32_t* nbr,
+                              const int32_t* row_order, const void* plan, size_t plan_bytes, const float* bias,
+                              const float* bn_scale, const float* bn_shift, int act, const void* res,
+                              const int32_t* res_index, void* out2, int dtype, void* stream) {
+  PTV3_REQUIRE(dtype == PTV3_F32 || dtype == PTV3_BF16, "conv_halo: bad dtype %d", dtype);
+  PTV3_REQUIRE(c == 32 || c == 64, "conv_halo: cin = cout = %d must be 32 or 64", c);
+  PTV3_REQUIRE(m >= 0 && m < ((int64_t)1 << 31), "conv_halo: m=%lld out of range", (long long)m);
+  PTV3_REQUIRE((bn_scale == nullptr) == (bn_shift == nullptr), "conv_halo: bn_scale/bn_shift must come together");
+  PTV3_REQUIRE(out2 == nullptr || res != nullptr, "conv_halo: out2 without res");
+  if (m == 0) return PTV3_OK;
+  PTV3_REQUIRE(x && w && out && nbr, "conv_halo: x, w, out and the 27-tap neighbour table are required");
+  PTV3_REQUIRE(plan && plan_bytes >= halo_plan_bytes(m) && ((uintptr_t)plan & 15) == 0,
+               "conv_halo: plan must be the one ptv3_halo_plan_build wrote for these m rows");
+  const HaloPlan p = halo_layout(const_cast<void*>(plan), m);
+  GemmArgs a{x, w, out, out2, res, nbr, row_order, res_index, bias, bn_scale, bn_shift, nullptr,
+             m, c, c, HALO_TAPS, act, c == 32 ? 5 : 6, 0, 0, 0};
+  const HaloArgs h{p.count, p.rows, p.slots};
+  hipStream_t s = (hipStream_t)stream;
+  const int esz = dtype == PTV3_F32 ? 4 : 2;
+  const int prof = prof_begin(s, PROF_SUBM_CONV, 2.0 * m * HALO_TAPS * c * c,
+                              ((double)m * c + (double)HALO_TAPS * c * c +
+                               (double)m * c * (1 + (res != nullptr) + (out2 != nullptr))) * esz,
+                              nbr, m * HALO_TAPS, 2.0 * c * c);
+  prof_kernel(prof, PK_CONV_HALO);
+  const dim3 grid((unsigned)p.tiles);
+#define HC_LAUNCH(T, C_)                                                                                      \
+  do {                                                                                                        \
+    const int lds = HaloShape<T, C_>::LDS;                                                                    \
+    ensure_dynamic_lds(reinterpret_cast<const void*>(&conv_halo_kernel<T, C_>), lds);                         \
+    hipLaunchKernelGGL((conv_halo_kernel<T, C_>), grid, dim3(256), lds, s, a, h);                             \
+  } while (0)
+  if (dtype == PTV3_F32) { if (c == 32) HC_LAUNCH(float, 32); else HC_LAUNCH(float, 64); }
+  else { if (c == 32) HC_LAUNCH(__bf16, 32); else HC_LAUNCH(__bf16, 64); }
+#undef HC_LAUNCH
+  prof_end(prof, s);
+  PTV3_LAUNCH_CHECK();
+  return PTV3_OK;
+}
diff --git a/pointcept-keypointdetection_amd/csrc/halo_plan.h b/pointcept-keypointdetection_amd/csrc/halo_plan.h
--- /dev/null
+++ b/pointcept-keypointdetection_amd/csrc/halo_plan.h
@@ -0,0 +1,30 @@
+#pragma once
+#include <stddef.h>
+#include <stdint.h>
+
+namespace ptv3 {
+
+constexpr int HALO_T = 128;
+constexpr int HALO_CAP = 432;
+constexpr int HALO_TAPS = 27;
+constexpr unsigned HALO_ABSENT = 0xFFFFu;
+
+struct HaloPlan { int32_t* count; int32_t* rows; uint16_t* slots; int64_t tiles; };
+
+static inline int64_t halo_tiles(int64_t m) { return (m + HALO_T - 1) / HALO_T; }
+static inline size_t halo_count_bytes(int64_t tiles) { return ((size_t)tiles * 4 + 15) & ~(size_t)15; }
+static inline size_t halo_plan_bytes(int64_t m) {
+  const int64_t t = halo_tiles(m < 0 ? 0 : m);
+  return halo_count_bytes(t) + (size_t)t * HALO_CAP * 4 + (size_t)t * HALO_T * HALO_TAPS * 2;
+}
+static inline HaloPlan halo_layout(void* plan, int64_t m) {
+  HaloPlan p;
+  p.tiles = halo_tiles(m);
+  char* b = (char*)plan;
+  p.count = (int32_t*)b;
+  p.rows = (int32_t*)(b + halo_count_bytes(p.tiles));
+  p.slots = (uint16_t*)(b + halo_count_bytes(p.tiles) + (size_t)p.tiles * HALO_CAP * 4);
+  return p;
+}
+
+}
diff --git a/pointcept-keypointdetection_amd/csrc/profile.h b/pointcept-keypointdetection_amd/csrc/profile.h
--- a/pointcept-keypointdetection_amd/csrc/profile.h
+++ b/pointcept-keypointdetection_amd/csrc/profile.h
@@ -7,7 +7,7 @@
 enum {
   PK_GEMM64_DENSE = 0, PK_GEMM64_CONV, PK_GEMM32_DENSE, PK_GEMM32_CONV, PK_GEMM_BIG_DENSE, PK_GEMM_BIG_CONV,
   PK_BLOCK_HEAD, PK_BLOCK_TAIL, PK_BLOCK_HEAD_COOP, PK_BLOCK_TAIL_COOP, PK_MLP2, PK_ATTN_FULL, PK_ATTN_TILED,
-  PK_BLOCK_HEAD_WIDE, PK_BLOCK_TAIL_WIDE, PK_CONV_TILE, PK_GEMM_TN, PK_ATTN_BWD_DQ, PK_ATTN_BWD_DKV, PK_SWIN_ATTN, PK_ROWS_LINEAR, PK_SWIN_ATTN_MFMA, PK_KERNELS
+  PK_BLOCK_HEAD_WIDE, PK_BLOCK_TAIL_WIDE, PK_CONV_TILE, PK_GEMM_TN, PK_ATTN_BWD_DQ, PK_ATTN_BWD_DKV, PK_SWIN_ATTN, PK_ROWS_LINEAR, PK_SWIN_ATTN_MFMA, PK_CONV_HALO, PK_KERNELS
 };
 void prof_kernel(int rec, int kernel);
 bool prof_on();
diff --git a/pointcept-keypointdetection_amd/csrc/profile.hip b/pointcept-keypointdetection_amd/csrc/profile.hip
--- a/pointcept-keypointdetection_amd/csrc/profile.hip
+++ b/pointcept-keypointdetection_amd/csrc/profile.hip
@@ -12,7 +12,7 @@
     "block_head_kernel", "block_tail_kernel", "block_head_coop_kernel", "block_tail_coop_kernel", "mlp2_kernel",
     "window_attn_full_kernel", "window_attn_kernel", "block_head_wide_kernel", "block_tail_wide_kernel",
     "conv_tile_kernel (sparse conv)", "gemm_tn_kernel", "attn_bwd_dq_kernel", "attn_bwd_dkv_kernel",
-    "swin_attn_kernel", "rows_linear_kernel", "swin_attn_mfma_kernel"};
+    "swin_attn_kernel", "rows_linear_kernel", "swin_attn_mfma_kernel", "conv_halo_kernel (sparse conv)"};
 static bool g_on = false;
 static double g_hint_flops = -1.0;
 static std::vector<ProfRec> g_recs;
diff --git a/pointcept-keypointdetection_amd/csrc/sparse.hip b/pointcept-keypointdetection_amd/csrc/sparse.hip
--- a/pointcept-keypointdetection_amd/csrc/sparse.hip
+++ b/pointcept-keypointdetection_amd/csrc/sparse.hip
@@ -1,6 +1,7 @@
 #include <stdlib.h>
 #include "common.h"
 #include "hashtable.h"
+#include "halo_plan.h"
 #include "../../include/ptv3_hip.h"
 
 namespace ptv3 {
@@ -232,6 +233,78 @@
   }
 }
 
+constexpr int HALO_HASH = 4096;
+__global__ __launch_bounds__(256) void halo_plan_kernel(const int32_t* __restrict__ nbr,
+                                                        const int32_t* __restrict__ row_order, int64_t n, HaloPlan p) {
+  constexpr int ENT = HALO_T * HALO_TAPS, PER = (ENT + 255) / 256, CELLS = HALO_HASH / 256;
+  __shared__ int32_t s_key[HALO_HASH];
+  __shared__ uint16_t s_slot[HALO_HASH];
+  __shared__ int s_wave[4];
+  const int tid = threadIdx.x, lane = tid & 63, wave = tid >> 6;
+  const int64_t tile = blockIdx.x, row0 = tile * HALO_T;
+  for (int c = tid; c < HALO_HASH; c += 256) s_key[c] = -1;
+  int64_t orow[PER];
+  bool in[PER];
+#pragma unroll
+  for (int u = 0; u < PER; ++u) {
+    const int e = tid + 256 * u;
+    const int64_t r = row0 + e / HALO_TAPS;
+    in[u] = e < ENT && r < n;
+    const int64_t rs = in[u] ? r : 0;
+    orow[u] = row_order ? (int64_t)row_order[rs] : rs;
+  }
+  int32_t v[PER];
+#pragma unroll
+  for (int u = 0; u < PER; ++u) {
+    const int e = tid + 256 * u;
+    v[u] = nbr[orow[u] * HALO_TAPS + e % HALO_TAPS];
+    if (!in[u]) v[u] = -1;
+  }
+  __syncthreads();
+  int cell[PER];
+#pragma unroll
+  for (int u = 0; u < PER; ++u) {
+    cell[u] = -1;
+    if (v[u] < 0) continue;
+    unsigned hsh = ((unsigned)v[u] * 2654435761u) >> 20;
+    for (int probe = 0; probe < HALO_HASH; ++probe) {
+      int32_t prev = *(volatile int32_t*)&s_key[hsh];
+      if (prev == -1) prev = atomicCAS(&s_key[hsh], -1, v[u]);
+      if (prev == -1 || prev == v[u]) { cell[u] = (int)hsh; break; }
+      hsh = (hsh + 1) & (HALO_HASH - 1);
+    }
+  }
+  __syncthreads();
+  int mine = 0;
+#pragma unroll
+  for (int j = 0; j < CELLS; ++j) mine += s_key[tid + 256 * j] >= 0;
+  int incl = mine;
+#pragma unroll
+  for (int o = 1; o < 64; o <<= 1) {
+    const int up = __shfl_up(incl, o, 64);
+    if (lane >= o) incl += up;
+  }
+  if (lane == 63) s_wave[wave] = incl;
+  __syncthreads();
+  int at = incl - mine;
+  for (int wv = 0; wv < wave; ++wv) at += s_wave[wv];
+#pragma unroll
+  for (int j = 0; j < CELLS; ++j) {
+    const int32_t key = s_key[tid + 256 * j];
+    if (key < 0) continue;
+    s_slot[tid + 256 * j] = (uint16_t)at;
+    if (at < HALO_CAP) p.rows[tile * HALO_CAP + at] = key;
+    ++at;
+  }
+  __syncthreads();
+#pragma unroll
+  for (int u = 0; u < PER; ++u) {
+    const int e = tid + 256 * u;
+    if (e < ENT) p.slots[tile * ENT + e] = cell[u] >= 0 ? s_slot[cell[u]] : (uint16_t)HALO_ABSENT;
+  }
+  if (tid == 0) p.count[tile] = s_wave[0] + s_wave[1] + s_wave[2] + s_wave[3];
+}
+
 }
 
 using namespace ptv3;
@@ -362,3 +435,24 @@
   PTV3_LAUNCH_CHECK();
   return PTV3_OK;
 }
+
+extern "C" size_t ptv3_halo_plan_bytes(int64_t m) { return halo_plan_bytes(m); }
+
+extern "C" int ptv3_halo_plan_shape(int* tile_sites, int* cap_rows) {
+  if (tile_sites) *tile_sites = HALO_T;
+  if (cap_rows) *cap_rows = HALO_CAP;
+  return PTV3_OK;
+}
+
+extern "C" int ptv3_halo_plan_build(const int32_t* nbr, const int32_t* row_order, int64_t m, void* plan, size_t bytes,
+                                    void* stream) {
+  PTV3_REQUIRE(m >= 0 && m < ((int64_t)1 << 31), "halo_plan_build: m=%lld out of range", (long long)m);
+  if (m == 0) return PTV3_OK;
+  PTV3_REQUIRE(nbr != nullptr, "halo_plan_build: the 27-tap neighbour table is required");
+  PTV3_REQUIRE(plan && bytes >= halo_plan_bytes(m) && ((uintptr_t)plan & 15) == 0,
+               "halo_plan_build: plan must be 16-byte aligned and hold ptv3_halo_plan_bytes(m) bytes");
+  const HaloPlan p = halo_layout(plan, m);
+  hipLaunchKernelGGL(halo_plan_kernel, dim3((unsigned)p.tiles), dim3(256), 0, (hipStream_t)stream, nbr, row_order, m, p);
+  PTV3_LAUNCH_CHECK();
+  return PTV3_OK;
+}
diff --git a/pointcept-keypointdetection_amd/ptv3_hip/lib.py b/pointcept-keypointdetection_amd/ptv3_hip/lib.py
--- a/pointcept-keypointdetection_amd/ptv3_hip/lib.py
+++ b/pointcept-keypointdetection_amd/ptv3_hip/lib.py
@@ -62,6 +62,11 @@
     "ptv3_gemm": (c_int, [P, P, P, c_int64, c_int, c_int, c_int, P, P, P, P, P, c_int, P, P, P, c_int, P, c_size_t,
                           P]),
     "ptv3_gemm_splits": (c_int, [c_int64, c_int, c_int, c_int, c_int]),
+    "ptv3_halo_plan_bytes": (c_size_t, [c_int64]),
+    "ptv3_halo_plan_shape": (c_int, [P, P]),
+    "ptv3_halo_plan_build": (c_int, [P, P, c_int64, P, c_size_t, P]),
+    "ptv3_conv_halo_policy": (c_int, [c_int64, c_int, c_int, c_int, c_int]),
+    "ptv3_conv_halo": (c_int, [P, P, P, c_int64, c_int, P, P, P, c_size_t, P, P, P, c_int, P, P, P, c_int, P]),
     "ptv3_block_fusable": (c_int, [c_int, c_int, c_int, c_int64]),
     "ptv3_rows_linear_capable": (c_int, [c_int, c_int, c_int, c_int64]),
     "ptv3_rows_linear": (c_int, [P, P, P, P, P, P, P, P, c_int, P, P, P, c_int64, c_int, c_int, c_float, c_int, P]),
diff --git a/pointcept-keypointdetection_amd/ptv3_hip/ops.py b/pointcept-keypointdetection_amd/ptv3_hip/ops.py
--- a/pointcept-keypointdetection_amd/ptv3_hip/ops.py
+++ b/pointcept-keypointdetection_amd/ptv3_hip/ops.py
@@ -348,6 +348,75 @@
     lib.check(lib.ptv3_gemm(_p(x), _p(w), _p(out), m, cin, cout, int(kvol), _p(nbr), _p(row_order), _p(bias),
                             _p(bn_scale), _p(bn_shift), int(act), _p(res), _p(res_index), _p(out2), dt, _p(ws),
                             ws_bytes, _stream()), "ptv3_gemm")
+    return (out, out2) if dual else out
+
+
+def halo_plan_shape():
+    t, cap = ctypes.c_int(0), ctypes.c_int(0)
+    lib.check(lib.ptv3_halo_plan_shape(ctypes.byref(t), ctypes.byref(cap)), "ptv3_halo_plan_shape")
+    return t.value, cap.value
+
+
+def halo_plan(nbr, row_order=None):
+    _chk(nbr, "nbr", torch.int32, 2)
+    _chk(row_order, "row_order", torch.int32, 1)
+    m = nbr.shape[0]
+    if nbr.shape[1] != 27:
+        raise RuntimeError("halo_plan: the neighbour table must have 27 taps")
+    if row_order is not None and row_order.shape[0] != m:
+        raise RuntimeError("halo_plan: row_order length != m")
+    t, cap = halo_plan_shape()
+    tiles = (m + t - 1) // t
+    nbytes = lib.ptv3_halo_plan_bytes(m)
+    plan = torch.empty(nbytes, dtype=torch.uint8, device=nbr.device)
+    lib.check(lib.ptv3_halo_plan_build(_p(nbr), _p(row_order), m, _p(plan), nbytes, _stream()), "ptv3_halo_plan_build")
+    cb = (tiles * 4 + 15) // 16 * 16
+    rb = tiles * cap * 4
+    counts = plan[:tiles * 4].view(torch.int32)
+    rows = plan[cb:cb + rb].view(torch.int32).view(tiles, cap)
+    slots = plan[cb + rb:cb + rb + tiles * t * 27 * 2].view(torch.int16).view(tiles, t, 27)
+    return plan, counts, rows, slots
+
+
+def conv_halo_policy(m, c, dtype):
+    return bool(lib.ptv3_conv_halo_policy(int(m), int(c), int(c), 27, _DT[dtype]))
+
+
+def conv_halo(x, w, nbr, plan, bias=None, row_order=None, bn_scale=None, bn_shift=None, act=ACT_NONE, res=None,
+              res_index=None, dual=False, out=None):
+    _chk(x, "x", (torch.float32, torch.bfloat16), 2)
+    _chk(w, "w", x.dtype)
+    for t, nm in ((bias, "bias"), (bn_scale, "bn_scale"), (bn_shift, "bn_shift")):
+        _chk(t, nm, torch.float32, 1)
+    _chk(nbr, "nbr", torch.int32, 2)
+    _chk(row_order, "row_order", torch.int32, 1)
+    _chk(res, "res", x.dtype, 2)
+    _chk(res_index, "res_index", torch.int32, 1)
+    _chk(plan, "plan", torch.uint8, 1)
+    m, c = nbr.shape[0], x.shape[1]
+    if nbr.shape[1] != 27 or x.shape[0] != m:
+        raise RuntimeError("conv_halo: x must have one row per row of the 27-tap neighbour table")
+    if w.numel() != c * 27 * c:
+        raise RuntimeError(f"conv_halo: weight has {w.numel()} elements, expected {c}x27x{c}")
+    for t in (bias, bn_scale, bn_shift):
+        if t is not None and t.numel() != c:
+            raise RuntimeError("conv_halo: epilogue vector length != c")
+    if res is not None:
+        if res.shape[1] != c or (res_index is None and res.shape[0] != m):
+            raise RuntimeError("conv_halo: residual shape mismatch")
+        if res_index is not None and res_index.shape[0] != m:
+            raise RuntimeError("conv_halo: res_index length != m")
+    if row_order is not None and row_order.shape[0] != m:
+        raise RuntimeError("conv_halo: row_order length != m")
+    if out is None:
+        out = torch.empty((m, c), dtype=x.dtype, device=x.device)
+    _chk(out, "out", x.dtype, 2)
+    if tuple(out.shape) != (m, c):
+        raise RuntimeError("conv_halo: out shape mismatch")
+    out2 = torch.empty_like(out) if dual else None
+    lib.check(lib.ptv3_conv_halo(_p(x), _p(w), _p(out), m, c, _p(nbr), _p(row_order), _p(plan), plan.numel(), _p(bias),
+                                 _p(bn_scale), _p(bn_shift), int(act), _p(res), _p(res_index), _p(out2), _dt(x),
+                                 _stream()), "ptv3_conv_halo")
     return (out, out2) if dual else out
 
 
```

Result: faster. 41.23 Mpoints/s, median of 6 (+3.0%).
